# hammershock/3dgs-avatar-release

Hardware: AMD Instinct MI355X
Metric: render fps (fwd+bwd) @200k Gaussians 1024x1024 SH3 (higher is better)
Workload: dtype f32; 1 GPU; config3: 200k Gaussians, 1024x1024, SH deg 3, forward+backward; shs+scales+rotations inputs, L1 loss (L1 fused into the rasterizer: l1_target); tile_rect=1, l1=fused, long_lists=0, gaussians=200000, width=1024, height=1024, sh_degree=3, frames_per_rank=1857, total_frames=1857, ranks=1, backend=none, parallelism=frames sharded x1

## Files before the change

### 3dgs-avatar-release_amd/csrc/binning.hip

```cpp
#include "common.h"

__global__ __launch_bounds__(256) void first_pair_kernel(const uint32_t* __restrict__ tiles,
                                                         const uint32_t* __restrict__ wave_tiles, float* __restrict__ rec,
                                                         int P, unsigned long long* __restrict__ count,
                                                         unsigned long long* host_count) {
    __shared__ unsigned long long wb[4];
    const int tid = threadIdx.x, lane = tid & 63, wid = tid >> 6;
    const int w0 = 4 * (int)blockIdx.x;
    unsigned long long before = 0;
    for (int w = tid; w < w0; w += 256) before += wave_tiles[w];
#pragma unroll
    for (int d = 32; d >= 1; d >>= 1) before += __shfl_xor(before, d, 64);
    if (lane == 0) wb[wid] = before;
    const int i = blockIdx.x * 256 + tid;
    const uint32_t v = i < P ? tiles[i] : 0u;
    uint32_t x = v;
#pragma unroll
    for (int d = 1; d < 64; d <<= 1) {
        const uint32_t y = __shfl_up(x, d, 64);
        if (lane >= d) x += y;
    }
    __syncthreads();
    const unsigned long long block_base = (wb[0] + wb[1]) + (wb[2] + wb[3]);
    uint32_t woff = 0;
// ... 257 lines not shown
        }
#pragma unroll
        for (int i = 0; i < PER; i++) {
            if (i * 1024 >= ntiles) break;
            mx = max(mx, held[i]);
        }
    } else {
        for (int t = tid; t < ntiles; t += 1024) mx = max(mx, tile_work(ranges, keys, mode, t));
    }
    mx = wave_max(mx);
    if (lane == 0) wmax[wid] = mx;
    __syncthreads();
    mx = 0;
    for (int w = 0; w < 16; w++) mx = max(mx, wmax[w]);
    const float scale = mx ? 1023.0f / (float)mx : 0.f;
    auto bin_of = [&](uint32_t w) { return 1023u - min(1023u, (uint32_t)((float)w * scale)); };
    if (HELD) {
#pragma unroll
        for (int i = 0; i < PER; i++) {
            if (i * 1024 >= ntiles) break;
            if (i * 1024 + tid < ntiles) atomicAdd(&hist[bin_of(held[i])], 1u);
        }
    } else {
        for (int t = tid; t < ntiles; t += 1024) atomicAdd(&hist[bin_of(tile_work(ranges, keys, mode, t))], 1u);
    }
    __syncthreads();
    const uint32_t v = hist[tid];
    const uint32_t x = wave_scan_incl(v);
    if (lane == 63) wsum[wid] = x;
    __syncthreads();
    uint32_t woff = 0;
    for (int w = 0; w < wid; w++) woff += wsum[w];
    hist[tid] = woff + x - v;
    __syncthreads();
    uint32_t wide_from = 0xFFFFFFFFu;
    uint32_t ch = 0;
    uint32_t xmask = 0;
    if (mode == 2) {
        const unsigned long long D = *pc.dev;
        wide_from = max(FWD4_MIN_LIST, (uint32_t)min(D / (unsigned long long)ll.total_div, 0x7FFFFFFFull));
        if (ll.mark == 2 && D <= FWDC_SPARSE_PAIRS) wide_from = min(FWD4_MIN_LIST, ll.ch_min);
        if (ll.stats || ll.mark == 2) {
            uint32_t nlong = 0;
            if (HELD) {
#pragma unroll
                for (int i = 0; i < PER; i++) {
                    if (i * 1024 >= ntiles) break;
                    nlong += (i * 1024 + tid < ntiles && held[i] > wide_from) ? 1u : 0u;
                }
            } else {
                for (int t = tid; t < ntiles; t += 1024) nlong += tile_work(ranges, keys, mode, t) > wide_from ? 1u : 0u;
            }
            nlong = wave_sum(nlong);
            __syncthreads();
            if (lane == 0) wsum[wid] = nlong;
            __syncthreads();
            uint32_t tot = 0;
            for (int w = 0; w < 16; w++) tot += wsum[w];
            if (tid == 0 && ll.stats) {
                __hip_atomic_store(&ll.stats[0], (long long)tot, __ATOMIC_RELAXED, __HIP_MEMORY_SCOPE_SYSTEM);
                __hip_atomic_store(&ll.stats[1], (long long)mx, __ATOMIC_RELAXED, __HIP_MEMORY_SCOPE_SYSTEM);
            }
            xmask = (ll.mark == 2 && ll.xcc_mask) ? (*ll.xcc_mask & 0xFFu) : 0u;
            if (xmask && tot > 0 && tot <= FWDC_MAX_UNITS / 2 && D <= (unsigned long long)pc.cap) {
                ch = ll.ch_min;
                while (D / ch + tot > (unsigned long long)FWDC_MAX_UNITS && ch < 0x40000000u) ch <<= 1;
            }
            __syncthreads();
            if (tid == 0) wmax[0] = 0u;
            if (tid < 16) wsum[tid] = 0u;
            __syncthreads();
        }
        if (!ll.mark) wide_from = 0xFFFFFFFFu;
        if (ll.mark == 2 && ch == 0) wide_from = 0xFFFFFFFFu;
    }
    auto place = [&](const int t, const uint32_t wk) {
        const bool marked = wk > wide_from && (ch == 0u || wk > ch);
        order[atomicAdd(&hist[bin_of(wk)], 1u)] = (uint32_t)t | (marked ? 0x80000000u : 0u);
    };
    if (HELD) {
#pragma unroll
        for (int i = 0; i < PER; i++) {
            if (i * 1024 >= ntiles) break;
            const int t = i * 1024 + tid;
            if (t < ntiles) place(t, held[i]);
        }
    } else {
        for (int t = tid; t < ntiles; t += 1024) place(t, tile_work(ranges, keys, mode, t));
    }
    if (ch) {
        __syncthreads();
        uint32_t* __restrict__ stash = hist;
        uint32_t* __restrict__ nstash = &wmax[1];
        if (tid == 0) *nstash = 0u;
        __syncthreads();
        const uint32_t nx = (uint32_t)__popc(xmask);
        for (int pos = tid; pos < ntiles; pos += 1024) {
            const uint32_t ov = order[pos];
            if (!(ov >> 31)) continue;
            const int t = (int)(ov & 0x7FFFFFFFu);
            const uint32_t nch = (tile_work(ranges, keys, mode, t) + ch - 1u) / ch;
            const uint32_t u0 = atomicAdd(&wmax[0], nch);
            const uint32_t ph = (uint32_t)pos % (2u * nx);
            uint32_t pick = ph < nx ? ph : 2u * nx - 1u - ph, best = 0;
            for (uint32_t x = 0; x < 8; x++) {
                if ((xmask >> x) & 1u) {
                    if (pick == 0u) { best = x; break; }
                    pick--;
                }
            }
            const uint32_t i0 = atomicAdd(&wsum[8 + best], 4u * nch);
            const uint32_t k = atomicAdd(nstash, 1u);
            stash[4 * k] = (uint32_t)t;
            stash[4 * k + 1] = u0;
            stash[4 * k + 2] = i0 | (best << 28);
            stash[4 * k + 3] = nch;
        }
        __syncthreads();
        const uint32_t nk = *nstash;
        for (uint32_t k = (uint32_t)wid; k < nk; k += 16) {
            const uint32_t t = stash[4 * k], u0 = stash[4 * k + 1], ib = stash[4 * k + 2], nch = stash[4 * k + 3];
            uint32_t* __restrict__ items = ll.cw_items + (size_t)(ib >> 28) * (FWDC_MAX_UNITS * 4) + (ib & 0x0FFFFFFFu);
            for (uint32_t c = (uint32_t)lane; c < nch; c += 64) ll.cw_units[u0 + c] = make_uint2(t, c | (nch << 16));
            for (uint32_t i = (uint32_t)lane; i < 4u * nch; i += 64) items[i] = (u0 + (i >> 2)) * 4u + (i & 3u);
        }
    }
    if (ll.cw_hdr) {
        __syncthreads();
        if (tid == 0) {
            ll.cw_hdr[0] = (mode == 2 && ch) ? wmax[0] : 0u;
            ll.cw_hdr[1] = ch;
        }
        if (tid < 8) ll.cw_hdr[4 + tid] = (mode == 2 && ch) ? wsum[8 + tid] : 0u;
    }
}

template <bool HELD>
__global__ __launch_bounds__(1024) void tile_order_kernel(const uint2* __restrict__ ranges,
                                                          const uint32_t* __restrict__ keys, int mode, int ntiles,
                                                          uint32_t* __restrict__ order, const PairCount pc,
                                                          const FillJob fill, const LongLists ll) {
    if (blockIdx.x > 0) {
        if (fill.clean && *fill.clean == MARKS_CLEAN) return;
        const uint4 ones = make_uint4(0xFFFFFFFFu, 0xFFFFFFFFu, 0xFFFFFFFFu, 0xFFFFFFFFu);
        for (size_t k = (size_t)(blockIdx.x - 1) * 1024 + threadIdx.x; k < fill.quads; k += (size_t)(gridDim.x - 1) * 1024)
            if (fill.stream) store_stream(&fill.ptr[k], ones); else fill.ptr[k] = ones;
        return;
    }
    __shared__ uint32_t hist[1024];
    __shared__ uint32_t wmax[16];
    __shared__ uint32_t wsum[16];
    if (mode < 0) return;
    tile_order_body<HELD>(ranges, keys, mode, ntiles, order, pc, ll, hist, wmax, wsum);
}

#define BM_LD 33
#ifndef TW_STOP_AFTER
#define TW_STOP_AFTER 99
#endif
template <bool CW>
__global__ __launch_bounds__(TBK_THREADS) void tile_write_kernel(const uint4* __restrict__ ranklist,
                                                                 const uint32_t* __restrict__ seg_start, int P, int gx,
                                                                 int gy, int nbx, int nblocks, int nseg, int ntiles,
                                                                 const uint32_t* __restrict__ seg_cnt,
                                                                 const uint32_t* __restrict__ tile_tot,
                                                                 uint2* __restrict__ ranges, uint32_t* __restrict__ order,
                                                                 uint32_t* __restrict__ point_list, const PairCount pc,
                                                                 const LongLists ll) {
    __shared__ uint32_t m_id[TBK_BUF];
    __shared__ unsigned short m_rc[TBK_BUF];
    __shared__ uint32_t bitmap[TB_TILES * BM_LD];
    __shared__ uint32_t dst[TB_TILES];
    __shared__ uint32_t wcnt[TBK_WAVES];
    __shared__ unsigned long long sb_scratch[20];
    static_assert(TBK_THREADS == 1024 && TBK_WAVES == 16 && TB_H <= 4 && TB_TILES * BM_LD >= 1024 && TB_TILES >= 32, "the ordering job borrows bitmap / dst");
    if (blockIdx.x == 0) {
        if (CW) {
            if (ntiles <= 32 * 1024) tile_order_body<true>(nullptr, tile_tot, 2, ntiles, order, pc, ll, bitmap, dst, dst + 16);
            else tile_order_body<false>(nullptr, tile_tot, 2, ntiles, order, pc, ll, bitmap, dst, dst + 16);
        } else if (ntiles <= 32 * 1024) {
            tile_order_plain<true>(nullptr, tile_tot, 2, ntiles, order, pc, ll, bitmap, dst, dst + 16);
        } else {
            tile_order_plain<false>(nullptr, tile_tot, 2, ntiles, order, pc, ll, bitmap, dst, dst + 16);
        }
        return;
    }
    const int tid = threadIdx.x, lane = tid & 63, wid = tid >> 6;
    const int b = ((int)blockIdx.x - 1) % nblocks, sg = ((int)blockIdx.x - 1) / nblocks;
    const int r0 = min(P, (int)seg_start[sg] * 256), r1 = min(P, (int)seg_start[sg + 1] * 256);
    const int bx0 = (b % nbx) * TB_W, by0 = (b / nbx) * TB_H;
    const int bx1 = min(gx, bx0 + TB_W), by1 = min(gy, by0 + TB_H);
    const unsigned long long frame_pairs = *pc.dev;
    const bool fits = frame_pairs <= (unsigned long long)pc.cap;
    uint32_t my_dst = 0;
    {
        const int t_blk0 = by0 * gx + bx0;
        uint32_t part = 0;
        for (int t0 = 0; t0 < t_blk0; t0 += 4 * TBK_THREADS) {
            uint32_t v[4];
#pragma unroll
            for (int k = 0; k < 4; k++) v[k] = t0 + k * TBK_THREADS + tid < t_blk0 ? tile_tot[t0 + k * TBK_THREADS + tid] : 0u;
            part += (v[0] + v[1]) + (v[2] + v[3]);
        }
        const int ty = by0 + wid, tx = bx0 + lane;
        const bool row_ok = tid < TB_TILES && ty < by1;
        const int t_row0 = ty * gx + bx0, t = t_row0 + lane;
        const bool tile_ok = row_ok && tx < bx1;
        uint32_t tot = 0, pre = 0, rowsum = 0;
        if (row_ok) {
            for (int k = lane; k < gx; k += 64) rowsum += t_row0 + k < ntiles ? tile_tot[t_row0 + k] : 0u;
            if (tile_ok) {
                tot = tile_tot[t];
                for (int s0 = 0; s0 < sg; s0 += 8) {
                    uint32_t v[8];
#pragma unroll
                    for (int k = 0; k < 8; k++) v[k] = (s0 + k < sg) ? seg_cnt[(size_t)(s0 + k) * ntiles + t] : 0u;
#pragma unroll
                    for (int k = 0; k < 8; k++) pre += v[k];
                }
            }
        }
        part = wave_sum(part);
        rowsum = wave_sum(rowsum);
        uint32_t* s_part = reinterpret_cast<uint32_t*>(sb_scratch);
        if (lane == 0) {
            s_part[wid] = part;
            if (wid < TB_H) s_part[16 + wid] = rowsum;
        }
        __syncthreads();
        if (row_ok) {
            uint32_t before = 0;
            for (int w = 0; w < TBK_WAVES; w++) before += s_part[w];
            for (int r = 0; r < wid; r++) before += s_part[16 + r];
            const uint32_t x = wave_scan_incl(tot);
            const uint32_t first = before + x - tot;
            if (sg == 0 && tile_ok) ranges[t] = fits ? make_uint2(first, first + tot) : make_uint2(0u, 0u);
            my_dst = first + pre;
        }
        __syncthreads();
    }
    if (TW_STOP_AFTER <= 1) return;
    if (!fits || !point_list) return;
    for (int k = tid; k < TB_TILES * BM_LD; k += TBK_THREADS) bitmap[k] = 0u;
    uint4 e[TBK_LPL];
    auto load_trip = [&](const int rb) {
#pragma unroll
        for (int k = 0; k < TBK_LPL; k++) {
            const int r = rb + wid * (64 * TBK_LPL) + k * 64 + lane;
            e[k] = r < r1 ? ranklist[r] : make_uint4(0, 0, 0, 0);
        }
    };
    if (TW_STOP_AFTER <= 2) return;
    load_trip(r0);
    if (tid < TB_TILES) dst[tid] = my_dst;
    const unsigned long long lt_mask = (lane == 0) ? 0ull : (~0ull >> (64 - lane));
    int count = 0;
    const int grp = lane >> 4, gl = lane & 15;

    auto process_batch = [&](const int n) {
        const int nw = (n + 31) >> 5;
        for (int m0 = wid * 4; m0 < n; m0 += TBK_WAVES * 4) {
            const int m = m0 + grp;
            if (m < n) {
                const uint32_t rc = m_rc[m];
                const uint32_t lw = ((rc >> 8) & 63u) + 1u, lh = ((rc >> 14) & 3u) + 1u;
                const uint32_t area = lw * lh, lx = rc & 63u, ly = (rc >> 6) & 3u;
                for (uint32_t j = (uint32_t)gl; j < area; j += 16u) {
                    const uint32_t dy = (j >= lw ? 1u : 0u) + (j >= 2u * lw ? 1u : 0u) + (j >= 3u * lw ? 1u : 0u);
                    const uint32_t lt = (ly + dy) * TB_W + lx + (j - dy * lw);
                    atomicOr(&bitmap[lt * BM_LD + (m >> 5)], 1u << (m & 31));
                }
            }
        }
        __syncthreads();
        for (int lt0 = wid * 4; lt0 < TB_TILES; lt0 += TBK_WAVES * 4) {
            const int lt = lt0 + grp;
            uint32_t bits0 = 0, bits1 = 0;
            if (gl < nw) { bits0 = bitmap[lt * BM_LD + gl]; bitmap[lt * BM_LD + gl] = 0u; }
            if (gl + 16 < nw) { bits1 = bitmap[lt * BM_LD + gl + 16]; bitmap[lt * BM_LD + gl + 16] = 0u; }
            const uint32_t c0 = (uint32_t)__popc(bits0), c1 = (uint32_t)__popc(bits1);
            const uint32_t xs = row_scan_incl(c0 | (c1 << 16));
            const uint32_t x0 = xs & 0xFFFFu, x1 = xs >> 16;
            const uint32_t e0 = (uint32_t)__builtin_amdgcn_readlane((int)xs, 15), e1 = (uint32_t)__builtin_amdgcn_readlane((int)xs, 31);
            const uint32_t e2 = (uint32_t)__builtin_amdgcn_readlane((int)xs, 47), e3 = (uint32_t)__builtin_amdgcn_readlane((int)xs, 63);
            const uint32_t ends = grp == 0 ? e0 : (grp == 1 ? e1 : (grp == 2 ? e2 : e3));
            const uint32_t tot0 = ends & 0xFFFFu, tot1 = ends >> 16;
            const uint32_t d0 = dst[lt];
            uint32_t pos = d0 + x0 - c0;
            while (bits0) {
                const int bp = __ffs((int)bits0) - 1;
                bits0 &= bits0 - 1u;
                point_list[pos++] = m_id[(gl << 5) + bp];
            }
            pos = d0 + tot0 + x1 - c1;
            while (bits1) {
                const int bp = __ffs((int)bits1) - 1;
                bits1 &= bits1 - 1u;
                point_list[pos++] = m_id[((gl + 16) << 5) + bp];
            }
            if (gl == 0) dst[lt] = d0 + tot0 + tot1;
        }
        __syncthreads();
    };

    __syncthreads();
    for (int rb = r0; rb < r1 || count > 0;) {
        if (rb < r1) {
            uint32_t rc[TBK_LPL], id[TBK_LPL];
            unsigned long long bal[TBK_LPL];
            int c[TBK_LPL], csum = 0;
#pragma unroll
            for (int k = 0; k < TBK_LPL; k++) {
                const bool h = block_hit(e[k], bx0, by0, bx1, by1, &rc[k]);
                id[k] = e[k].x;
                bal[k] = __ballot(h);
                c[k] = __popcll(bal[k]);
                csum += c[k];
            }
            if (lane == 0) wcnt[wid] = (uint32_t)csum;
            if (rb + TBK_CHUNK < r1) load_trip(rb + TBK_CHUNK);
            __syncthreads();
            uint32_t woff = 0, tot = 0;
            for (int w = 0; w < TBK_WAVES; w++) {
                const uint32_t cw = wcnt[w];
                woff += w < wid ? cw : 0u;
                tot += cw;
            }
            int slot0 = count + (int)woff;
#pragma unroll
            for (int k = 0; k < TBK_LPL; k++) {
                if ((bal[k] >> lane) & 1ull) {
                    const int slot = slot0 + __popcll(bal[k] & lt_mask);
                    m_id[slot] = id[k];
                    m_rc[slot] = (unsigned short)rc[k];
                }
                slot0 += c[k];
            }
            count += (int)tot;
            rb += TBK_CHUNK;
            __syncthreads();
        }
        const bool last = rb >= r1;
        while (count >= TBK_BATCH || (last && count > 0)) {
            const int n = min(count, TBK_BATCH);
            if (TW_STOP_AFTER > 3) process_batch(n);
            const int rem = count - n;
            uint32_t cid[TBK_LPL];
            unsigned short crc[TBK_LPL];
#pragma unroll
            for (int k = 0; k < TBK_LPL; k++) {
                const int i = tid + k * TBK_THREADS;
                cid[k] = i < rem ? m_id[n + i] : 0u;
                crc[k] = i < rem ? m_rc[n + i] : (unsigned short)0;
            }
            __syncthreads();
#pragma unroll
            for (int k = 0; k < TBK_LPL; k++) {
                const int i = tid + k * TBK_THREADS;
                if (i < rem) { m_id[i] = cid[k]; m_rc[i] = crc[k]; }
            }
            count = rem;
            __syncthreads();
        }
    }
}

int launch_tile_order(const uint32_t* ranges, const uint32_t* keys, int mode, int ntiles, uint32_t* order, PairCount pc,
                      FillJob fill, LongLists ll, int debug, hipStream_t s) {
    const size_t pieces = (fill.quads + 1023) / 1024;
    const int side = fill.ptr ? (int)(pieces < 255 ? pieces : 255) : 0;
    if (ntiles <= 32 * 1024)
        hipLaunchKernelGGL(tile_order_kernel<true>, dim3(1 + side), dim3(1024), 0, s, reinterpret_cast<const uint2*>(ranges),
                           keys, mode, ntiles, order, pc, fill, ll);
    else
        hipLaunchKernelGGL(tile_order_kernel<false>, dim3(1 + side), dim3(1024), 0, s, reinterpret_cast<const uint2*>(ranges),
                           keys, mode, ntiles, order, pc, fill, ll);
    GS_LAUNCH_CHECK("tile_order", debug, s);
    return GS_OK;
}

int launch_tile_lists(const uint4* ranklist, const uint32_t* chunk_pairs, uint32_t* seg_start, int P, int gx, int gy, TileCounts tc, uint32_t* ranges,
                      uint32_t* order, uint32_t* point_list, PairCount pc, LongLists ll, bool totals_zeroed, int debug,
                      hipStream_t s) {
    uint32_t* seg_cnt = tc.seg_cnt;
    const BinGrid G = bin_grid(gx, gy);
    const int nseg = bin_segments(G, P);
    const int ntiles = gx * gy;
    if (!totals_zeroed) {
        const int zrc = gs_zero_async(tc.tile_tot, tc.zero_bytes, "tile_totals.zero", s);
        if (zrc != GS_OK) return zrc;
    }
    {
        int band_rows = TC_CELLS / (gx + 1) - 1;
        if (band_rows < 1) return GS_E_TOO_LARGE;
        if (band_rows > gy) band_rows = gy;
        const int nbands = (gy + band_rows - 1) / band_rows;
        StageScope sc_("tile_count", s);
        hipLaunchKernelGGL(tile_count_kernel, dim3((unsigned)(nbands * nseg)), dim3(TC_THREADS), 0, s, ranklist, chunk_pairs, seg_start, P,
                           gx, gy, band_rows, nbands, nseg, ntiles, seg_cnt, tc.tile_tot, tc.xcc_mask);
        GS_LAUNCH_CHECK("tile_count", debug, s);
    }
    {
        StageScope sc_("tile_write", s);
        if (ll.mark == 2)
            hipLaunchKernelGGL(tile_write_kernel<true>, dim3((unsigned)(1 + G.nblocks * nseg)), dim3(TBK_THREADS), 0, s, ranklist,
                               seg_start, P, gx, gy, G.nbx, G.nblocks, nseg, ntiles, seg_cnt, tc.tile_tot,
                               reinterpret_cast<uint2*>(ranges), order, pc.cap > 0 ? point_list : nullptr, pc, ll);
        else
            hipLaunchKernelGGL(tile_write_kernel<false>, dim3((unsigned)(1 + G.nblocks * nseg)), dim3(TBK_THREADS), 0, s, ranklist,
                               seg_start, P, gx, gy, G.nbx, G.nblocks, nseg, ntiles, seg_cnt, tc.tile_tot,
                               reinterpret_cast<uint2*>(ranges), order, pc.cap > 0 ? point_list : nullptr, pc, ll);
        GS_LAUNCH_CHECK("tile_write", debug, s);
    }
    return GS_OK;
}
```

### 3dgs-avatar-release_amd/csrc/capi.hip

```cpp
#include "common.h"
#include <string.h>
#include <stdlib.h>
#include <atomic>
#include <chrono>
#include <mutex>
#include <vector>

static thread_local int g_last_hip = 0;
static thread_local const char* g_last_stage = "";
void gs_set_error(int hip_err, const char* stage) {
    g_last_hip = hip_err;
    g_last_stage = stage;
}

struct TuneSwitch {
    const char* name;
    int key, def;
    const char* env;
    bool (*ok)(int);
};
static const TuneSwitch k_tune[GS_TUNE_COUNT] = {
    {"xcd_map", GS_TUNE_XCD_MAP, 1, nullptr, nullptr},
    {"depth_sort", GS_TUNE_DEPTH_SORT, 1, nullptr, nullptr},
    {"nt_stores", GS_TUNE_NT_STORES, 1, nullptr, nullptr},
    {"bwd_chunks", GS_TUNE_BWD_CHUNKS, 1, nullptr, nullptr},
    {"fwd4", GS_TUNE_FWD4, 1, "GSPLAT_FWD4", nullptr},
    {"small_tiles", GS_TUNE_SMALL_TILES, BWD_CHUNK_MAX_TILES, nullptr, nullptr},
    {"shared_qlist", GS_TUNE_SHARED_QLIST, 1, nullptr, nullptr},
    {"ones_fast", GS_TUNE_ONES_FAST, 1, nullptr, nullptr},
    {"bwd_order", GS_TUNE_BWD_ORDER, 1, nullptr, nullptr},
    {"fwd_marks", GS_TUNE_FWD_MARKS, 1, nullptr, nullptr},
    {"fwdc_ch", GS_TUNE_FWDC_CH, (int)FWDC_CH_MIN, "GSPLAT_FWDC_CH", [](int v) { return v >= 64 && (v & (v - 1)) == 0; }},
    {"fwdc_div", GS_TUNE_FWDC_DIV, (int)FWD4_TOTAL_DIV, "GSPLAT_FWDC_DIV", [](int v) { return v >= 1; }},
};
struct TuneState {
    std::atomic<int> v[GS_TUNE_COUNT];
    TuneState() {
        for (const TuneSwitch& t : k_tune) {
            int value = t.def;
            if (const char* e = t.env ? getenv(t.env) : nullptr) {
                const int x = atoi(e);
                if (!t.ok || t.ok(x)) value = x;
            }
            v[t.key].store(value);
        }
    }
};
static TuneState& tune_state() {
    static TuneState st;
    return st;
}
int gs_tune_get(int key) {
    return (key >= 0 && key < GS_TUNE_COUNT) ? tune_state().v[key].load(std::memory_order_relaxed) : 0;
}

struct ProfRec { const char* name; hipEvent_t a, b; };
struct ProfState {
    bool on = false;
    bool armed = false;
    int nested = 0;
    char filter[32] = {0};
    std::vector<ProfRec> recs;
    std::vector<hipEvent_t> pool;
    hipEvent_t get() {
        if (!pool.empty()) { hipEvent_t e = pool.back(); pool.pop_back(); return e; }
        hipEvent_t e = nullptr;
        (void)hipEventCreate(&e);
        return e;
    }
};
static ProfState g_prof;
static std::mutex g_prof_mu;
static bool profiling_on() { return g_prof.on; }
void gs_prof_begin(const char* stage, hipStream_t s) {
    if (!g_prof.on) return;
    std::lock_guard<std::mutex> lk(g_prof_mu);
    if (g_prof.armed) { g_prof.nested++; return; }
    g_prof.armed = g_prof.on && (g_prof.filter[0] == 0 || strcmp(g_prof.filter, stage) == 0);
    if (!g_prof.armed) return;
    ProfRec r{stage, g_prof.get(), g_prof.get()};
    (void)hipEventRecord(r.a, s);
    g_prof.recs.push_back(r);
}
void gs_prof_end(hipStream_t s) {
    if (!g_prof.on) return;
    std::lock_guard<std::mutex> lk(g_prof_mu);
    if (!g_prof.armed || g_prof.recs.empty()) return;
    if (g_prof.nested > 0) { g_prof.nested--; return; }
    (void)hipEventRecord(g_prof.recs.back().b, s);
    g_prof.armed = false;
}

static int validate(const GsFwdArgs* a) {
    if (!a) return GS_E_BAD_ARG;
    if (a->P < 0 || a->W <= 0 || a->H <= 0) return GS_E_BAD_ARG;
    if (!a->bg || !a->viewmatrix || !a->projmatrix || !a->campos) return GS_E_BAD_ARG;
    if (a->P > 0 && (!a->means3D || !a->opacities)) return GS_E_BAD_ARG;
    if ((a->shs != nullptr) == (a->colors_precomp != nullptr)) return GS_E_EXCLUSIVE;
    const bool sr = a->scales != nullptr && a->rotations != nullptr;
    if ((a->scales != nullptr) != (a->rotations != nullptr)) return GS_E_EXCLUSIVE;
    if (sr == (a->cov3D_precomp != nullptr)) return GS_E_EXCLUSIVE;
    if (a->shs) {
        if (a->sh_degree < 0 || a->sh_degree > 3) return GS_E_BAD_ARG;
        if (a->M < (a->sh_degree + 1) * (a->sh_degree + 1)) return GS_E_BAD_ARG;
        if (a->M > 16) return GS_E_BAD_ARG;
    }
    if (a->rotations && ((uintptr_t)a->rotations & 15u)) return GS_E_BAD_ARG;
    if ((a->W + TILE - 1) / TILE > 0xFFFF || (a->H + TILE - 1) / TILE > 0xFFFF) return GS_E_TOO_LARGE;
    return GS_OK;
}

static bool stream_is_capturing(void* stream) {
    hipStreamCaptureStatus st = hipStreamCaptureStatusNone;
    const hipError_t e = hipStreamIsCapturing((hipStream_t)stream, &st);
    if (e != hipSuccess) {
        (void)hipGetLastError();
        return e == hipErrorStreamCaptureImplicit || e == hipErrorStreamCaptureUnsupported || e == hipErrorStreamCaptureInvalidated;
    }
    return st != hipStreamCaptureStatusNone;
}
#define GS_CAPTURE_OK_IF(stream, cond)                                           \
    do {                                                                         \
        if (stream_is_capturing(stream) && (!(cond) || profiling_on())) return GS_E_CAPTURE; \
    } while (0)
#define GS_NO_CAPTURE(stream) GS_CAPTURE_OK_IF(stream, false)

__global__ void zero_words_kernel(uint32_t* __restrict__ p, size_t words) {
    for (size_t k = (size_t)blockIdx.x * blockDim.x + threadIdx.x; k < words; k += (size_t)gridDim.x * blockDim.x) p[k] = 0u;
}
int gs_zero_async(void* ptr, size_t bytes, const char* stage, hipStream_t s) {
    const size_t words = bytes / 4;
    if (words == 0) return GS_OK;
    const size_t blocks = (words + 255) / 256;
    hipLaunchKernelGGL(zero_words_kernel, dim3((unsigned)(blocks < 1024 ? blocks : 1024)), dim3(256), 0, s, (uint32_t*)ptr, words);
    const hipError_t e = hipGetLastError();
    if (e != hipSuccess) { gs_set_error((int)e, stage); return GS_E_HIP; }
    return GS_OK;
}

__global__ __launch_bounds__(256) void clock_probe_kernel(unsigned long long* __restrict__ out, int iters, float seed, float* __restrict__ sink) {
    const unsigned long long t0 = __builtin_readcyclecounter(), r0 = __builtin_amdgcn_s_memrealtime();
    float a[8];
#pragma unroll
    for (int i = 0; i < 8; i++) a[i] = seed + (float)i + (float)threadIdx.x * 1e-3f;
    for (int it = 0; it < iters; it++) {
#pragma unroll
        for (int u = 0; u < 4; u++)
#pragma unroll
            for (int i = 0; i < 8; i++) a[i] = __builtin_fmaf(a[i], 1.0001f, 0.5f);
    }
    float sum = 0.f;
#pragma unroll
    for (int i = 0; i < 8; i++) sum += a[i];
    if (sum == 12345.678f) sink[0] = sum;
    if (threadIdx.x == 0) {
        const unsigned long long t1 = __builtin_readcyclecounter(), r1 = __builtin_amdgcn_s_memrealtime();
        atomicAdd(&out[0], t1 - t0);
        atomicAdd(&out[1], r1 - r0);
    }
}

__global__ __launch_bounds__(64) void xcc_probe_kernel(uint32_t* __restrict__ out) {
    if (threadIdx.x == 0) out[blockIdx.x] = xcc_id();
}

template <class Void, class VoidBin, class G, class B, class I, class Own>
static int frame_states(const GsFwdArgs* a, Void* geom, size_t geom_bytes, VoidBin* binning, size_t binning_bytes, Void* img,
                        size_t img_bytes, int64_t D, G* g, B* b, I* im, Own own) {
    int rc = validate(a);
    if (rc != GS_OK) return rc;
    if (!geom || !img || D < 0 || (D > 0 && !binning)) return GS_E_BAD_ARG;
    if ((rc = own()) != GS_OK) return rc;
    *g = geom_state(geom, a->P);
    *im = img_state(img, a->W, a->H, a->long_lists);
    *b = bin_state(D > 0 ? binning : nullptr, D);
    if (geom_bytes < g->total || img_bytes < im->total || (D > 0 && binning_bytes < b->total)) return GS_E_WORKSPACE;
    return GS_OK;
}

template <class T> static T* writable(T* p) { return p; }
template <class T> static T* writable(const T* p) { return const_cast<T*>(p); }
template <bool RO>
static QuadLists quad_lists(const ImgViewT<RO>& im, const BinView& b, int long_lists) {
    QuadLists ql;
    ql.qlist = b.qlist;
    ql.ncon_c = writable(im.ncon_c);
    ql.qcount = writable(im.qcount);
    ql.chunks = gs_tune_get(GS_TUNE_BWD_CHUNKS) ? im.bwd_chunks : 1;
    ql.four_waves = forward_small_image(im.ntiles, long_lists) ? 1 : 0;
    ql.ckpt = ql.chunks > 1 ? writable(im.ckpt) : nullptr;
    ql.ck_start = ql.chunks > 1 ? writable(im.ck_start) : nullptr;
    return ql;
}
template <bool RO>
static void quad_lists_chunked(QuadLists& ql, const ImgView& own, const ImgViewT<RO>& list) {
    ql.chunked = 1;
    ql.cw_hdr = list.cw_hdr;
    ql.cw_units = list.cw_units;
    ql.cw_items = list.cw_items;
    ql.cw_q = own.cw_q;
    ql.cw_flag = own.cw_flag;
    ql.cw_done = own.cw_done;
    ql.cw_rec = own.cw_rec;
}
static int sync_if_debug(const GsFwdArgs* a, const char* stage, hipStream_t s) {
    if (!a->debug) return GS_OK;
    const hipError_t e = hipStreamSynchronize(s);
    if (e != hipSuccess) { gs_set_error((int)e, stage); return GS_E_HIP; }
    return GS_OK;
}

extern "C" {

int gs_xcc_probe(uint32_t* xcc, int32_t n_blocks, void* stream) {
    if (!xcc || n_blocks <= 0) return GS_E_BAD_ARG;
    hipStream_t s = (hipStream_t)stream;
    hipLaunchKernelGGL(xcc_probe_kernel, dim3((unsigned)n_blocks), dim3(64), 0, s, xcc);
    GS_LAUNCH_CHECK("xcc_probe", 0, s);
    return GS_OK;
}

int gs_clock_probe(uint64_t* ticks, int32_t iters, void* stream) {
    if (!ticks || iters <= 0) return GS_E_BAD_ARG;
    GS_NO_CAPTURE(stream);
    hipStream_t s = (hipStream_t)stream;
    int rc = gs_zero_async(ticks, 32, "clock_probe.zero", s);
    if (rc != GS_OK) return rc;
    hipLaunchKernelGGL(clock_probe_kernel, dim3(2048), dim3(256), 0, s, (unsigned long long*)ticks, iters, 1.0f, (float*)(ticks + 2));
    GS_LAUNCH_CHECK("clock_probe", 0, s);
    return GS_OK;
}

int gs_geom_bytes(int32_t P, size_t* out) {
    if (!out || P < 0) return GS_E_BAD_ARG;
    *out = geom_layout(P).total;
    return GS_OK;
}
int gs_image_bytes(int32_t W, int32_t H, size_t* out) {
    if (!out || W <= 0 || H <= 0) return GS_E_BAD_ARG;
    *out = img_layout(W, H).total;
    return GS_OK;
}
int gs_image_bytes_for(const GsFwdArgs* a, size_t* out) {
    if (!a || !out || a->W <= 0 || a->H <= 0) return GS_E_BAD_ARG;
    *out = img_layout(a->W, a->H, a->long_lists).total;
    return GS_OK;
}
int gs_binning_bytes(int64_t D, int32_t W, int32_t H, size_t* out) {
    if (!out || D < 0 || W <= 0 || H <= 0) return GS_E_BAD_ARG;
    if (D > GS_MAX_PAIRS) return GS_E_TOO_LARGE;
    *out = bin_layout(D).total;
    return GS_OK;
}
int gs_backward_scratch_bytes(int64_t D, int32_t P, int32_t W, int32_t H, size_t* out) {
    if (!out || D < 0 || P < 0 || W <= 0 || H <= 0) return GS_E_BAD_ARG;
    const ImgLayout I = img_layout(W, H);
    *out = scratch_total_bytes(D, P, I.gx * I.gy);
    return GS_OK;
}

static int forward_phase1(const GsFwdArgs* a, void* geom, size_t geom_bytes, void* img, size_t img_bytes, int32_t* radii,
                          int64_t* count_host_pinned, unsigned long long* poll, void* stream) {
    GeomView g;
    BinView none;
    ImgView im;
    int rc = frame_states(a, geom, geom_bytes, (void*)nullptr, 0, img, img_bytes, 0, &g, &none, &im,
                          [&]() -> int { return (a->P > 0 && !radii) ? GS_E_BAD_ARG : GS_OK; });
    if (rc != GS_OK) return rc;
    hipStream_t s = (hipStream_t)stream;
    if (a->P == 0) {
        rc = gs_zero_async(g.count, COUNT_ZERO_BYTES, "count.zero", s);
        if (rc != GS_OK) return rc;
    } else {
        ZeroJob zt;
        sort_totals_region(g.hist, a->P, 32, &zt.ptr, &zt.words);
        const ZeroJob zi{im.tile_tot, (int)(im.tile_zero_bytes / 4)};
        { StageScope sc_("preprocess", s);
        rc = launch_preprocess(*a, g.rec, g.depths, g.tiles, g.clamped, g.key0, g.val0, radii, g.wsum, g.wkmin, g.wkmax, zt, zi, s); }
        if (rc != GS_OK) return rc;
        if (gs_tune_get(GS_TUNE_DEPTH_SORT)) {
            StageScope sc_("depth_sort", s);
            const DepthSortState ds{g.ds_tmp, g.ds_tmp2, g.ds_cnt, g.ds_pre, g.ds_tot, g.ds_loc, g.ds_grp, g.ds_range, g.ds_nb, g.ds_blocks};
            const PairNumbering pn{g.tiles, g.wsum, g.rec, g.count, poll, g.chunk_pairs, (a->P + 255) / 256};
            const RankOut ro{g.rec, g.tiles, g.val0, g.ranklist, g.chunk_pairs};
            rc = launch_depth_sort(g.key0, g.wkmin, g.wkmax, g.nwaves, a->P, ds, pn, ro, a->debug, s);
            if (rc != GS_OK) return rc;
        } else {
            { StageScope sc_("pair_scan", s);
            rc = launch_first_pair(g.tiles, g.wsum, g.rec, g.count, poll, a->P, a->debug, s); }
            if (rc != GS_OK) return rc;
            { StageScope sc_("depth_sort", s);
            rc = launch_sort_pairs(g.key0, g.val0, g.key1, g.val1, g.hist, a->P, 32, true, a->debug, s); }
            if (rc != GS_OK) return rc;
            { StageScope sc_("rank_list", s);
            rc = launch_rank_list(g.val0, g.rec, g.tiles, g.ranklist, g.chunk_pairs, a->P, a->debug, s); }
            if (rc != GS_OK) return rc;
        }
    }
    if (count_host_pinned && (!poll || a->P == 0)) {
        hipError_t e = hipMemcpyAsync(count_host_pinned, g.count, 8, hipMemcpyDeviceToHost, s);
        if (e != hipSuccess) { gs_set_error((int)e, "count.copy"); return GS_E_HIP; }
    }
    return GS_OK;
}

int gs_forward_preprocess(const GsFwdArgs* a, void* geom, size_t geom_bytes, void* img, size_t img_bytes,
                          int32_t* radii, int64_t* count_host_pinned, void* stream) {
    GS_CAPTURE_OK_IF(stream, a && !a->debug && count_host_pinned == nullptr);
    return forward_phase1(a, geom, geom_bytes, img, img_bytes, radii, count_host_pinned, nullptr, stream);
}

static int forward_phase2(const GsFwdArgs* a, void* geom, size_t geom_bytes, void* binning, size_t binning_bytes, void* img,
                          size_t img_bytes, int64_t cap, float* out_color, void* stream, bool totals_zeroed) {
    GeomView g;
    BinView b;
    ImgView im;
    int rc = frame_states(a, geom, geom_bytes, binning, binning_bytes, img, img_bytes, cap, &g, &b, &im, [&]() -> int {
        if (!out_color) return GS_E_BAD_ARG;
        if (a->l1_target && !a->l1_loss) return GS_E_BAD_ARG;
        return cap > GS_MAX_PAIRS ? GS_E_TOO_LARGE : GS_OK;
    });
    if (rc != GS_OK) return rc;
    hipStream_t s = (hipStream_t)stream;
    const PairCount pc{g.count + COUNT_PAIRS, (uint32_t)cap};
    const bool chunked = forward_chunked(im.ntiles, a->long_lists);
    if (a->P > 0) {
        rc = launch_tile_lists(g.ranklist, g.chunk_pairs, g.seg_start, a->P, im.gx, im.gy,
                               TileCounts{im.seg_cnt, im.tile_tot, im.tile_zero_bytes, im.cw_xcc_mask}, im.ranges, im.order,
                               b.point_list, pc,
                               LongLists{chunked ? 2 : (forward_small_image(im.ntiles, a->long_lists) ? 1 : 0), (long long*)a->frame_stats,
                                         im.cw_hdr, im.cw_units, (uint32_t)gs_tune_get(GS_TUNE_FWDC_CH), im.cw_items, im.cw_xcc_mask,
                                         chunked ? (uint32_t)gs_tune_get(GS_TUNE_FWDC_DIV) : (uint32_t)FWD4_TOTAL_DIV},
                               totals_zeroed, a->debug, s);
        if (rc != GS_OK) return rc;
    } else {
        rc = gs_zero_async(im.ranges, (size_t)im.ntiles * 8, "ranges.zero", s);
        if (rc != GS_OK) return rc;
        StageScope sc_("ranges_order", s);
        rc = launch_tile_order(im.ranges, nullptr, 0, im.ntiles, im.order, pc, FillJob{nullptr, 0},
                               LongLists{0, nullptr, im.cw_hdr, nullptr}, a->debug, s);
        if (rc != GS_OK) return rc;
    }
    QuadLists ql = quad_lists(im, b, a->long_lists);
    if (chunked) quad_lists_chunked(ql, im, im);
    if (cap > 0) {
        ql.marks = (gs_tune_get(GS_TUNE_FWD_MARKS) && !a->forward_only) ? b.marks : nullptr;
        ql.mark_quads = (size_t)cap;
        ql.marks_flag = b.marks_flag;
    }
    ql.l1_target = a->l1_target;
    ql.l1_part = im.l1_part;
    ql.l1_loss = a->l1_loss;
    { StageScope sc_("render_fwd", s);
    rc = launch_render_forward(g.rec, a->P > 0 ? b.point_list : nullptr, im.ranges, im.order, a->bg, a->W, a->H, out_color,
                               im.final_T, im.n_contrib, ql, s); }
    if (rc != GS_OK) return rc;
    return sync_if_debug(a, "render_forward", s);
}

int gs_forward_render(const GsFwdArgs* a, void* geom, size_t geom_bytes, void* binning, size_t binning_bytes,
                      void* img, size_t img_bytes, int64_t D, float* out_color, void* stream) {
    GS_CAPTURE_OK_IF(stream, a && !a->debug && a->frame_stats == nullptr);
    return forward_phase2(a, geom, geom_bytes, binning, binning_bytes, img, img_bytes, D, out_color, stream, false);
}

int gs_forward(const GsFwdArgs* a, void* geom, size_t geom_bytes, void* binning, size_t binning_bytes, int64_t capacity,
               void* img, size_t img_bytes, int32_t* radii, int64_t* count_host_pinned, float* out_color,
               int64_t* num_rendered, void* stream) {
    if (!count_host_pinned || !num_rendered || capacity < 0) return GS_E_BAD_ARG;
    GS_NO_CAPTURE(stream);
    volatile int64_t* word = count_host_pinned;
    const int64_t pending = -1;
    static std::atomic<bool> poll_works{true};
    const bool poll = a && a->P > 0 && poll_works.load(std::memory_order_relaxed);
    if (poll) *word = pending;
    int rc = forward_phase1(a, geom, geom_bytes, img, img_bytes, radii, count_host_pinned,
                            poll ? (unsigned long long*)count_host_pinned : nullptr, stream);
    if (rc != GS_OK) return rc;
    const bool speculate = capacity > 0 && binning && binning_bytes >= bin_layout(capacity).total && capacity <= GS_MAX_PAIRS;
    if (speculate) {
        rc = forward_phase2(a, geom, geom_bytes, binning, binning_bytes, img, img_bytes, capacity, out_color, stream, true);
        if (rc != GS_OK) return rc;
    }
    bool have = false;
    if (poll) {
        const auto t0 = std::chrono::steady_clock::now();
        for (long spin = 0;; spin++) {
            if (*word != pending) { have = true; break; }
            if ((spin & 1023) == 1023 && std::chrono::steady_clock::now() - t0 > std::chrono::milliseconds(200)) break;
        }
    }
    if (!have) {
        hipError_t e = hipStreamSynchronize((hipStream_t)stream);
        if (e != hipSuccess) { gs_set_error((int)e, "count.sync"); return GS_E_HIP; }
        if (poll && *word == pending) {
            poll_works.store(false, std::memory_order_relaxed);
            int64_t c = 0;
            e = hipMemcpy(&c, geom_state(geom, a->P).count + COUNT_PAIRS, 8, hipMemcpyDeviceToHost);
            if (e != hipSuccess) { gs_set_error((int)e, "count.copy"); return GS_E_HIP; }
            *word = c;
        }
    }
    const int64_t D = *word;
    *num_rendered = D;
    if (D > (int64_t)GS_MAX_PAIRS) return GS_E_TOO_LARGE;
    if (!speculate || D > capacity) return GS_E_WORKSPACE;
    return GS_OK;
}

int gs_forward_shared(const GsFwdArgs* a, const void* geom_src, const void* img_src, void* geom, size_t geom_bytes,
                      void* binning, size_t binning_bytes, void* img, size_t img_bytes, int64_t D, float* out_color,
                      void* stream) {
    GS_CAPTURE_OK_IF(stream, a && !a->debug && a->P > 0);
    GeomView g;
    BinView b;
    ImgView im;
    int rc = frame_states(a, geom, geom_bytes, binning, binning_bytes, img, img_bytes, D, &g, &b, &im,
                          [&]() -> int { return (!geom_src || !img_src || !out_color) ? GS_E_BAD_ARG : GS_OK; });
    if (rc != GS_OK) return rc;
    const GeomViewRO first_g = geom_state(geom_src, a->P);
    const ImgViewRO first_im = img_state(img_src, a->W, a->H, a->long_lists);
    hipStream_t s = (hipStream_t)stream;
    const bool chunked = forward_chunked(im.ntiles, a->long_lists);
    QuadLists ql = quad_lists(im, b, a->long_lists);
    unsigned long long* not_ones = nullptr;
    if (a->P > 0) {
        StageScope sc_("recolor", s);
        if (gs_tune_get(GS_TUNE_ONES_FAST) && gs_tune_get(GS_TUNE_SHARED_QLIST) && a->colors_precomp && D > 0)
            not_ones = not_ones_word(first_g);
        const SecondOnes so{first_im.final_T, first_im.n_contrib, first_im.ncon_c, first_im.qcount, first_im.ckpt, first_im.ck_start,
                            out_color, im.final_T, im.n_contrib, im.ncon_c, im.qcount, ql.ckpt, ql.ck_start, a->bg, a->W, a->H,
                            im.gx, im.ntiles, ql.chunks};
        rc = launch_recolor(*a, first_g.rec, first_g.tiles, g.rec, g.tiles, g.clamped, not_ones,
                            CopyJob{first_im.ranges, im.ranges, im.ntiles * 2}, CopyJob{first_im.order, im.order, im.ntiles},
                            ZeroJob{im.cw_flag, im.cw_clear_words}, not_ones ? &so : nullptr, s);
        if (rc != GS_OK) return rc;
    } else {
        hipError_t e = hipMemcpyAsync(im.ranges, first_im.ranges, (size_t)im.ntiles * 8, hipMemcpyDeviceToDevice, s);
        if (e == hipSuccess) e = hipMemcpyAsync(im.order, first_im.order, (size_t)im.ntiles * 4, hipMemcpyDeviceToDevice, s);
        if (e != hipSuccess) { gs_set_error((int)e, "shared.copy"); return GS_E_HIP; }
    }
    if (gs_tune_get(GS_TUNE_SHARED_QLIST)) {
        ql.src_qcount = first_im.qcount;
        ql.src_n_contrib = first_im.n_contrib;
        ql.not_ones = not_ones;
    }
    if (chunked && a->P > 0) {
        quad_lists_chunked(ql, im, first_im);
        if (ql.src_qcount) {
            ql.src_cw_flag = first_im.cw_flag;
            ql.src_cw_rec = first_im.cw_rec;
            ql.src_final_T = first_im.final_T;
        }
    }
    ql.all_ones = im.all_ones;
    { StageScope sc_("render_fwd", s);
    rc = launch_render_forward(g.rec, b.point_list, im.ranges, im.order, a->bg, a->W, a->H, out_color, im.final_T, im.n_contrib, ql, s); }
    if (rc != GS_OK) return rc;
    return sync_if_debug(a, "render_forward", s);
}

int gs_opacity_image(const GsFwdArgs* a, const void* img, size_t img_bytes, float* opacity, void* stream) {
    GS_CAPTURE_OK_IF(stream, true);
    int rc = validate(a);
    if (rc != GS_OK) return rc;
    if (!img || !opacity) return GS_E_BAD_ARG;
    const ImgViewRO im = img_state(img, a->W, a->H, a->long_lists);
    if (img_bytes < im.total) return GS_E_WORKSPACE;
    return launch_opacity_image(im.final_T, a->bg, a->W, a->H, opacity, (hipStream_t)stream);
}

static int backward_impl(const GsFwdArgs* a, const int32_t* radii, const void* geom, size_t geom_bytes, void* binning,
                         size_t binning_bytes, const void* img, size_t img_bytes, int64_t D, const float* out_color,
                         const float* dL_dpix, const float* dL_dopacity_img, void* scratch, size_t scratch_bytes,
                         const GsGrads* gr, void* stream, const GsSecondImage* second = nullptr) {
    GS_CAPTURE_OK_IF(stream, a && !a->debug);
    GeomViewRO g;
    BinView b;
    ImgViewRO im;
    int rc = frame_states(a, geom, geom_bytes, binning, binning_bytes, img, img_bytes, D, &g, &b, &im, [&]() -> int {
        if (!out_color || (!dL_dpix && !a->l1_target) || !gr || (a->P > 0 && !scratch)) return GS_E_BAD_ARG;
        if (a->P > 0 && (!radii || !gr->dL_dmeans3D || !gr->dL_dmeans2D || !gr->dL_dcolors || !gr->dL_dopacity || !gr->dL_dcov3D))
            return GS_E_BAD_ARG;
        if (a->P > 0 && a->shs && !gr->dL_dsh) return GS_E_BAD_ARG;
        if (a->P > 0 && a->scales && (!gr->dL_dscales || !gr->dL_drotations)) return GS_E_BAD_ARG;
        if (gr->dL_drotations && ((uintptr_t)gr->dL_drotations & 15u)) return GS_E_BAD_ARG;
        return GS_OK;
    });
    if (rc != GS_OK) return rc;
    if (a->P > 0 && scratch_bytes < scratch_total_bytes(D, a->P, im.ntiles)) return GS_E_WORKSPACE;
    if (a->P == 0) return GS_OK;
    hipStream_t s = (hipStream_t)stream;
    float* const sums = (float*)((char*)scratch + scratch_rows_bytes(D));
    if (D > 0) {
        const QuadLists ql = quad_lists(im, b, a->long_lists);
        SecondImage si{nullptr, nullptr, nullptr, nullptr, nullptr};
        if (second) {
            const ImgViewRO im2 = img_state(second->img, a->W, a->H, second->long_lists);
            if (second->img_bytes < im2.total || im2.bwd_chunks != im.bwd_chunks) return GS_E_BAD_ARG;
            si = SecondImage{second->colors, second->out_color, second->dL_dpix, ql.chunks > 1 ? im2.ckpt : nullptr, im2.all_ones};
        }
        uint32_t* const q8 = reinterpret_cast<uint32_t*>(b.marks);
        uint32_t* const own_order = (uint32_t*)((char*)sums + scratch_sums_bytes(a->P));
        const bool order_here = gs_tune_get(GS_TUNE_BWD_ORDER) != 0;
        { StageScope sc_("tile_order", s);
        rc = launch_tile_order(im.ranges, ql.qcount, order_here ? 1 : -1, im.ntiles, own_order, PairCount{nullptr, 0},
                               FillJob{b.marks, (size_t)D, gs_tune_get(GS_TUNE_NT_STORES) & 1, b.marks_flag},
                               LongLists{0, nullptr}, a->debug, s); }
        if (rc != GS_OK) return rc;
        { StageScope sc_("render_bwd", s);
        rc = launch_render_backward(g.rec, im.ranges, order_here ? own_order : im.order, a->W, a->H, ql, out_color, dL_dpix,
                                    dL_dopacity_img, im.final_T, a->bg, (float*)scratch, q8, second ? &si : nullptr,
                                    L1Grad{a->l1_target, a->l1_grad}, s); }
        if (rc != GS_OK) return rc;
        rc = sync_if_debug(a, "render_backward", s);
        if (rc != GS_OK) return rc;
    }
    StageScope sc_("gaussian_bwd", s);
    return launch_gaussian_backward(*a, radii, g.rec, g.tiles, g.clamped, reinterpret_cast<const uint32_t*>(b.marks),
                                    (const float*)scratch, sums, b.marks_flag, *gr, s);
}

int gs_backward(const GsFwdArgs* a, const int32_t* radii, const void* geom, size_t geom_bytes, void* binning,
                size_t binning_bytes, const void* img, size_t img_bytes, int64_t D, const float* out_color,
                const float* dL_dpix, void* scratch, size_t scratch_bytes, const GsGrads* gr, void* stream) {
    return backward_impl(a, radii, geom, geom_bytes, binning, binning_bytes, img, img_bytes, D, out_color, dL_dpix, nullptr,
                         scratch, scratch_bytes, gr, stream);
}

int gs_backward_with_opacity(const GsFwdArgs* a, const int32_t* radii, const void* geom, size_t geom_bytes,
                             void* binning, size_t binning_bytes, const void* img, size_t img_bytes, int64_t D,
                             const float* out_color, const float* dL_dpix, const float* dL_dopacity_img, void* scratch,
                             size_t scratch_bytes, const GsGrads* gr, void* stream) {
    if (!dL_dopacity_img) return GS_E_BAD_ARG;
    return backward_impl(a, radii, geom, geom_bytes, binning, binning_bytes, img, img_bytes, D, out_color, dL_dpix,
                         dL_dopacity_img, scratch, scratch_bytes, gr, stream);
}

int gs_backward_with_second(const GsFwdArgs* a, const int32_t* radii, const void* geom, size_t geom_bytes,
                            void* binning, size_t binning_bytes, const void* img, size_t img_bytes, int64_t D,
                            const float* out_color, const float* dL_dpix, const GsSecondImage* second, void* scratch,
                            size_t scratch_bytes, const GsGrads* grads, void* stream) {
    if (!second || !second->colors || !second->out_color || !second->dL_dpix || !second->img) return GS_E_BAD_ARG;
    return backward_impl(a, radii, geom, geom_bytes, binning, binning_bytes, img, img_bytes, D, out_color, dL_dpix, nullptr,
                         scratch, scratch_bytes, grads, stream, second);
}

int gs_mark_visible(int32_t P, const float* means3D, const float* viewmatrix, const float* projmatrix,
                    uint8_t* present, void* stream) {
    GS_CAPTURE_OK_IF(stream, true);
    (void)projmatrix;
    if (P < 0 || !viewmatrix || (P > 0 && (!means3D || !present))) return GS_E_BAD_ARG;
    if (P == 0) return GS_OK;
    return launch_mark_visible(P, means3D, viewmatrix, present, (hipStream_t)stream);
}

int knn_workspace_bytes(int32_t P, size_t* out) {
    if (!out || P < 0) return GS_E_BAD_ARG;
    *out = knn_ws_bytes(P);
    return GS_OK;
}
int knn_dist2(int32_t P, const float* points, float* mean_d2, void* workspace, size_t workspace_bytes, void* stream) {
    GS_NO_CAPTURE(stream);
    if (P < 0 || (P > 0 && (!points || !mean_d2 || !workspace))) return GS_E_BAD_ARG;
    if (P == 0) return GS_OK;
    return launch_knn(P, points, mean_d2, workspace, workspace_bytes, (hipStream_t)stream);
}

int gs_build_covariance(int32_t N, const float* scaling, float scaling_modifier, const float* rotation, int32_t rotation_is_matrix,
                        float* cov6, void* stream) {
    GS_CAPTURE_OK_IF(stream, true);
    if (N < 0 || (N > 0 && (!scaling || !rotation || !cov6))) return GS_E_BAD_ARG;
    if (!rotation_is_matrix && ((uintptr_t)rotation & 15u)) return GS_E_BAD_ARG;
    if (N == 0) return GS_OK;
    return launch_build_cov(N, scaling, scaling_modifier, rotation, rotation_is_matrix ? 1 : 0, cov6, (hipStream_t)stream);
}
int gs_build_covariance_backward(int32_t N, const float* scaling, float scaling_modifier, const float* rotation,
                                 int32_t rotation_is_matrix, const float* dL_dcov6, float* dL_dscaling, float* dL_drotation,
                                 void* stream) {
    GS_CAPTURE_OK_IF(stream, true);
    if (N < 0 || (N > 0 && (!scaling || !rotation || !dL_dcov6 || !dL_dscaling || !dL_drotation))) return GS_E_BAD_ARG;
    if (!rotation_is_matrix && (((uintptr_t)rotation | (uintptr_t)dL_drotation) & 15u)) return GS_E_BAD_ARG;
    if (N == 0) return GS_OK;
    return launch_build_cov_bwd(N, scaling, scaling_modifier, rotation, rotation_is_matrix ? 1 : 0, dL_dcov6, dL_dscaling,
                                dL_drotation, (hipStream_t)stream);
}
int gs_sh2rgb(int32_t N, int32_t sh_degree, int32_t M, const float* shs, const float* xyz, const float* campos,
              const float* fwd_rotation, const float* view_noise_host, float* colors, uint8_t* clamped, void* stream) {
    GS_CAPTURE_OK_IF(stream, view_noise_host == nullptr);
    if (N < 0 || sh_degree < 0 || sh_degree > 3 || M < (sh_degree + 1) * (sh_degree + 1) || M > 16) return GS_E_BAD_ARG;
    if (N > 0 && (!shs || !xyz || !campos || !colors || !clamped)) return GS_E_BAD_ARG;
    if (N == 0) return GS_OK;
    return launch_sh2rgb(N, sh_degree, M, shs, xyz, campos, fwd_rotation, view_noise_host, colors, clamped, (hipStream_t)stream);
}
int gs_sh2rgb_backward(int32_t N, int32_t sh_degree, int32_t M, const float* shs, const float* xyz, const float* campos,
                       const float* fwd_rotation, const float* view_noise_host, const uint8_t* clamped,
                       const float* dL_dcolors, float* dL_dshs, float* dL_dxyz, void* stream) {
    GS_CAPTURE_OK_IF(stream, view_noise_host == nullptr);
    if (N < 0 || sh_degree < 0 || sh_degree > 3 || M < (sh_degree + 1) * (sh_degree + 1) || M > 16) return GS_E_BAD_ARG;
    if (N > 0 && (!shs || !xyz || !campos || !clamped || !dL_dcolors || !dL_dshs || !dL_dxyz)) return GS_E_BAD_ARG;
    if (N == 0) return GS_OK;
    return launch_sh2rgb_bwd(N, sh_degree, M, shs, xyz, campos, fwd_rotation, view_noise_host, clamped, dL_dcolors, dL_dshs,
                             dL_dxyz, (hipStream_t)stream);
}

int gs_l1_loss_workspace_bytes(int64_t n, size_t* out) {
    if (!out || n < 0) return GS_E_BAD_ARG;
    *out = l1_ws_bytes(n);
    return GS_OK;
}
int gs_l1_loss(int64_t n, const float* x, const float* y, float* loss, float* dL_dx, void* workspace, size_t workspace_bytes,
               void* stream) {
    GS_CAPTURE_OK_IF(stream, true);
    if (n <= 0 || !x || !y || !loss || !dL_dx || !workspace) return GS_E_BAD_ARG;
    if (((uintptr_t)x | (uintptr_t)y | (uintptr_t)dL_dx) & 15u) return GS_E_BAD_ARG;
    if (workspace_bytes < l1_ws_bytes(n)) return GS_E_WORKSPACE;
    return launch_l1_loss(x, y, n, loss, dL_dx, (float*)workspace, (hipStream_t)stream);
}

int gs_bce_loss(int64_t n, const float* x, const float* y, float* loss, float* dL_dx, void* workspace, size_t workspace_bytes,
                void* stream) {
    GS_CAPTURE_OK_IF(stream, true);
    if (n <= 0 || !x || !y || !loss || !dL_dx || !workspace) return GS_E_BAD_ARG;
    if (workspace_bytes < l1_ws_bytes(n)) return GS_E_WORKSPACE;
    return launch_bce_loss(x, y, n, loss, dL_dx, (float*)workspace, (hipStream_t)stream);
}

int gs_ssim_workspace_bytes(int32_t C, int32_t H, int32_t W, size_t* out) {
    if (!out || C <= 0 || H <= 0 || W <= 0) return GS_E_BAD_ARG;
    *out = ssim_ws_bytes(C, H, W);
    return GS_OK;
}
int gs_ssim_forward(int32_t C, int32_t H, int32_t W, const float* img1, const float* img2, float* ssim_out, float* dm_dmu1,
                    float* dm_dsigma1_sq, float* dm_dsigma12, void* workspace, size_t workspace_bytes, void* stream) {
    GS_CAPTURE_OK_IF(stream, true);
    if (C <= 0 || H <= 0 || W <= 0 || !img1 || !img2 || !ssim_out || !workspace) return GS_E_BAD_ARG;
    if ((dm_dmu1 != nullptr) != (dm_dsigma1_sq != nullptr) || (dm_dmu1 != nullptr) != (dm_dsigma12 != nullptr)) return GS_E_BAD_ARG;
    if (workspace_bytes < ssim_ws_bytes(C, H, W)) return GS_E_WORKSPACE;
    return launch_ssim_forward(C, H, W, img1, img2, ssim_out, dm_dmu1, dm_dsigma1_sq, dm_dsigma12, (float*)workspace,
                               (hipStream_t)stream);
}
int gs_ssim_backward(int32_t C, int32_t H, int32_t W, const float* img1, const float* img2, const float* dm_dmu1,
                     const float* dm_dsigma1_sq, const float* dm_dsigma12, const float* dL_dssim, float* dL_dimg1,
                     void* stream) {
    GS_CAPTURE_OK_IF(stream, true);
    if (C <= 0 || H <= 0 || W <= 0 || !img1 || !img2 || !dm_dmu1 || !dm_dsigma1_sq || !dm_dsigma12 || !dL_dssim || !dL_dimg1)
        return GS_E_BAD_ARG;
    return launch_ssim_backward(C, H, W, img1, img2, dm_dmu1, dm_dsigma1_sq, dm_dsigma12, dL_dssim, dL_dimg1,
                                (hipStream_t)stream);
}

int gs_densify_stats(int32_t N, const int32_t* radii, const float* viewspace_grad, float* max_radii2D,
                     float* xyz_gradient_accum, float* denom, void* stream) {
    GS_CAPTURE_OK_IF(stream, true);
    if (N < 0 || (N > 0 && (!radii || !viewspace_grad || !max_radii2D || !xyz_gradient_accum || !denom))) return GS_E_BAD_ARG;
    if (N == 0) return GS_OK;
    return launch_densify_stats(N, radii, viewspace_grad, max_radii2D, xyz_gradient_accum, denom, (hipStream_t)stream);
}
int gs_adam_step(int32_t n_tensors, const GsAdamTensor* tensors, double beta1, double beta2, double eps, int64_t step,
                 void* stream) {
    GS_NO_CAPTURE(stream);
    if (n_tensors < 0 || n_tensors > GS_ADAM_MAX_TENSORS || (n_tensors > 0 && !tensors) || step < 1) return GS_E_BAD_ARG;
    for (int k = 0; k < n_tensors; k++) {
        const GsAdamTensor& t = tensors[k];
// ... 658 lines not shown
```

### 3dgs-avatar-release_amd/csrc/common.h

```cpp
#pragma once
#include <hip/hip_runtime.h>
#include <stdint.h>
#include <stddef.h>
#include <type_traits>
#include "../../include/gsplat_mi355.h"

#define TILE 16
#define WAVE 64
#define REC_F 12
#define GS_MAX_PAIRS 0x3FFFFFFFll

static inline size_t align_up(size_t x, size_t a) { return (x + a - 1) / a * a; }

#define SORT_ITEMS 4096
#define SORT_SMALL_N (1 << 20)
#define SORT_TOTALS_REPL 16
static inline size_t sort_table_words(size_t n) {
    const size_t items = n <= (size_t)SORT_SMALL_N ? 1024 : SORT_ITEMS;
    return (size_t)256 * ((n + items - 1) / items + 4 * SORT_TOTALS_REPL);
}
#define SCAN_ITEMS 2048

#ifndef DS_ITEMS
#define DS_ITEMS 2048
#endif
#ifndef DS_PER_BUCKET
#define DS_PER_BUCKET 64
#endif
static inline int ds_buckets(int P) {
    int nb = (P / DS_PER_BUCKET + 63) / 64 * 64;
    return nb < 256 ? 256 : (nb > 4096 ? 4096 : nb);
}

#define TB_MAX_SEG 64
enum { COUNT_PAIRS = 0, COUNT_NOT_ONES = 2, COUNT_ZERO_BYTES = 24 };
struct GeomLayout {
    size_t rec, depths, tiles, clamped, key0, key1, val0, val1, ranklist, chunk_pairs, wsum, wkmin, wkmax, hist, count,
        ds_tmp, ds_tmp2, ds_cnt, ds_pre, ds_tot, ds_loc, ds_grp, ds_range, seg_start, total;
    int nblk_sort, nwaves, ds_nb, ds_blocks;
};
static inline GeomLayout geom_layout(int P) {
    GeomLayout L;
    size_t o = 0;
    size_t n = (size_t)(P > 0 ? P : 1);
    auto take = [&](size_t bytes) { size_t at = o; o = align_up(o + bytes, 256); return at; };
    L.nblk_sort = (int)((n + SORT_ITEMS - 1) / SORT_ITEMS);
    L.nwaves = (int)((n + 255) / 256) * 4;
    L.rec = take(n * REC_F * 4);
    L.depths = take(n * 4);
    L.tiles = take(n * 4);
    L.clamped = take(n * 4);
    L.key0 = take(n * 4);
    L.key1 = take(n * 4);
    L.val0 = take(n * 4);
    L.val1 = take(n * 4);
    L.ranklist = take(n * 16);
    L.chunk_pairs = take(((n + 255) / 256) * 4);
    L.wsum = take((size_t)L.nwaves * 4);
    L.wkmin = take((size_t)L.nwaves * 4);
    L.wkmax = take((size_t)L.nwaves * 4);
    L.hist = take(sort_table_words(n) * 4);
    L.count = take(64);
    L.ds_nb = ds_buckets(P);
    L.ds_blocks = (int)((n + DS_ITEMS - 1) / DS_ITEMS);
    L.ds_tmp = take(n * 8);
    L.ds_tmp2 = take(n * 8);
    L.ds_cnt = take((size_t)L.ds_blocks * (L.ds_nb + 1) * 4);
    L.ds_pre = take((size_t)L.ds_blocks * (L.ds_nb + 1) * 4);
    L.ds_tot = take((size_t)(L.ds_nb + 1) * 4);
    L.ds_loc = take((size_t)(L.ds_nb + 1) * 4);
    L.ds_grp = take((size_t)((L.ds_nb + 1 + 63) / 64) * 4);
    L.ds_range = take(16);
    L.seg_start = take((size_t)(TB_MAX_SEG + 2) * 4);
    L.total = o;
    return L;
}

struct BinLayout {
    size_t point_list, qlist, marks, marks_flag, total;
};
static inline BinLayout bin_layout(int64_t D) {
    BinLayout L;
    size_t o = 0;
    size_t n = (size_t)(D > 0 ? D : 1);
    auto take = [&](size_t bytes) { size_t at = o; o = align_up(o + bytes, 256); return at; };
    L.point_list = take(n * 4);
    L.qlist = take(n * 16);
    L.marks = take(n * 16);
    L.marks_flag = take(4);
    L.total = o;
    return L;
}

#define TB_W 64
#ifndef TB_H
#define TB_H 4
#endif
#define TB_TILES (TB_W * TB_H)
struct BinGrid { int nbx, nby, nblocks, nseg_max; };
static inline BinGrid bin_grid(int gx, int gy) {
    BinGrid G;
    G.nbx = (gx + TB_W - 1) / TB_W;
    G.nby = (gy + TB_H - 1) / TB_H;
    G.nblocks = G.nbx * G.nby;
#ifndef TB_TARGET_WGS
#define TB_TARGET_WGS 512
#endif
    int s = (TB_TARGET_WGS + G.nblocks - 1) / G.nblocks;
    G.nseg_max = s < 1 ? 1 : (s > TB_MAX_SEG ? TB_MAX_SEG : s);
    return G;
}
static inline int bin_segments(const BinGrid& G, int P) {
    int s = (P + 1023) / 1024;
    if (s < 1) s = 1;
    return s < G.nseg_max ? s : G.nseg_max;
}

enum { GS_TUNE_XCD_MAP = 0, GS_TUNE_DEPTH_SORT = 1, GS_TUNE_NT_STORES = 2, GS_TUNE_BWD_CHUNKS = 3, GS_TUNE_FWD4 = 4, GS_TUNE_SMALL_TILES = 5, GS_TUNE_SHARED_QLIST = 6, GS_TUNE_ONES_FAST = 7, GS_TUNE_BWD_ORDER = 8, GS_TUNE_FWD_MARKS = 9, GS_TUNE_FWDC_CH = 10, GS_TUNE_FWDC_DIV = 11, GS_TUNE_COUNT = 12 };
int gs_tune_get(int key);

#define BWD_CH 128
#define BWD_KMAX 16
#define BWD_CHUNK_MAX_TILES 2048
#define FWD4_MAX_TILES 2048
#define FWD4_MIN_LIST 512u
#ifndef FWD4_TOTAL_DIV
#define FWD4_TOTAL_DIV 320ull
#endif

#define FWDC_CH_MIN 256u
#define FWDC_SPARSE_PAIRS 524288ull
#define FWDC_MAX_UNITS 4096
#define FWDC_MAX_TILES (FWDC_MAX_UNITS / 2)
#define FWDC_Q_WORDS (8 * FWDC_MAX_UNITS * 4)
#define FWDC_Q_BYTES ((size_t)FWDC_Q_WORDS * 4 + 64)
#ifdef FWDC_PROF
#define FWDC_SLOTS 9
#else
#define FWDC_SLOTS 8
#endif
#define FWDC_DEAD 0x80000000u
#define FWDC_SPIN_MAX (1 << 16)
struct ImgLayout {
    size_t ranges, n_contrib, final_T, ncon_c, tile_nmax, order, seg_cnt, tile_tot, all_ones, cw_flag, cw_done, cw_q, tile_zero_bytes, l1_part, ckpt, ck_start, cw_hdr, cw_units, cw_items, cw_rec, total;
    int gx, gy, bwd_chunks;
};
static inline bool few_long_lists_mode(int ntiles, int long_lists) {
    return ntiles <= gs_tune_get(GS_TUNE_SMALL_TILES) || long_lists != 0;
}
static inline ImgLayout img_layout(int W, int H, int long_lists = 0) {
    ImgLayout L;
    size_t o = 0;
    auto take = [&](size_t bytes) { size_t at = o; o = align_up(o + bytes, 256); return at; };
    L.gx = (W + TILE - 1) / TILE;
    L.gy = (H + TILE - 1) / TILE;
    const size_t nt = (size_t)L.gx * L.gy;
    L.ranges = take(nt * 8);
    L.n_contrib = take((size_t)W * H * 4);
    L.final_T = take((size_t)W * H * 4);
    L.ncon_c = take((size_t)W * H * 4);
    L.tile_nmax = take(nt * 16);
    L.order = take(nt * 4);
    L.seg_cnt = take(nt * 4 * (size_t)bin_grid(L.gx, L.gy).nseg_max);
    L.tile_tot = take(nt * 4);
    L.all_ones = take(4);
    L.tile_zero_bytes = L.all_ones + 4 - L.tile_tot;
    const bool fl = few_long_lists_mode((int)nt, long_lists);
    const bool cw = fl && gs_tune_get(GS_TUNE_FWD4) == 2;
    L.cw_flag = L.cw_done = L.cw_q = 0;
    if (cw) {
        L.cw_flag = take((size_t)FWDC_MAX_UNITS * 4 * 4);
        L.cw_done = take(nt * 16);
        L.cw_q = take(FWDC_Q_BYTES);
        L.tile_zero_bytes = L.cw_q + FWDC_Q_BYTES - L.tile_tot;
    }
    L.l1_part = take(nt * 16);
    L.bwd_chunks = fl ? BWD_KMAX : 1;
    L.ckpt = take(nt * 4 * (size_t)(L.bwd_chunks - 1) * 64 * 16);
    L.ck_start = take(nt * 4 * (size_t)L.bwd_chunks * 4);
    L.cw_hdr = L.cw_units = L.cw_items = L.cw_rec = 0;
    if (cw) {
        L.cw_hdr = take(64);
        L.cw_units = take((size_t)FWDC_MAX_UNITS * 8);
        L.cw_items = take((size_t)FWDC_Q_WORDS * 4);
        L.cw_rec = take((size_t)FWDC_MAX_UNITS * 4 * FWDC_SLOTS * 64 * 4);
    }
    L.total = o;
    return L;
}

template <bool RO>
struct StateCarve {
    typename std::conditional<RO, const char, char>::type* base;
    StateCarve(typename std::conditional<RO, const void, void>::type* state) : base(static_cast<decltype(base)>(state)) {}
    template <class T>
    void operator()(T*& field, size_t offset, bool present = true) const {
        field = (base && present) ? reinterpret_cast<T*>(base + offset) : nullptr;
    }
};
template <bool RO>
struct GeomViewT {
    template <class T> using ptr = typename std::conditional<RO, const T, T>::type*;
    ptr<float> rec, depths;
    ptr<uint32_t> tiles, clamped, key0, key1, val0, val1;
    ptr<uint4> ranklist;
    ptr<uint32_t> chunk_pairs, wsum, wkmin, wkmax, hist;
    ptr<unsigned long long> count;
    ptr<unsigned long long> ds_tmp, ds_tmp2;
    ptr<uint32_t> ds_cnt, ds_pre, ds_tot, ds_loc, ds_grp, ds_range, seg_start;
    size_t total;
    int nwaves, ds_nb, ds_blocks;
};
template <bool RO>
struct BinViewT {
    template <class T> using ptr = typename std::conditional<RO, const T, T>::type*;
    ptr<uint32_t> point_list, qlist;
    ptr<uint4> marks;
    ptr<uint32_t> marks_flag;
    size_t total;
};
template <bool RO>
struct ImgViewT {
    template <class T> using ptr = typename std::conditional<RO, const T, T>::type*;
    ptr<uint32_t> ranges, n_contrib;
    ptr<float> final_T;
    ptr<uint32_t> ncon_c, qcount , order, seg_cnt, tile_tot, all_ones;
    ptr<uint32_t> cw_flag, cw_done, cw_q, cw_xcc_mask ;
    ptr<float> l1_part;
    ptr<float4> ckpt;
    ptr<uint32_t> ck_start, cw_hdr;
    ptr<uint2> cw_units;
    ptr<uint32_t> cw_items;
    ptr<float> cw_rec;
    size_t tile_zero_bytes;
    int cw_clear_words;
    size_t total;
    int gx, gy, ntiles, bwd_chunks;
};
typedef GeomViewT<false> GeomView;
typedef GeomViewT<true> GeomViewRO;
typedef BinViewT<false> BinView;
typedef BinViewT<true> BinViewRO;
typedef ImgViewT<false> ImgView;
typedef ImgViewT<true> ImgViewRO;

template <class Void >
static inline GeomViewT<std::is_const<Void>::value> geom_state(Void* base, int P) {
    constexpr bool RO = std::is_const<Void>::value;
    const GeomLayout L = geom_layout(P);
    const StateCarve<RO> at{base};
    GeomViewT<RO> v;
    at(v.rec, L.rec); at(v.depths, L.depths); at(v.tiles, L.tiles); at(v.clamped, L.clamped);
    at(v.key0, L.key0); at(v.key1, L.key1); at(v.val0, L.val0); at(v.val1, L.val1);
    at(v.ranklist, L.ranklist); at(v.chunk_pairs, L.chunk_pairs);
    at(v.wsum, L.wsum); at(v.wkmin, L.wkmin); at(v.wkmax, L.wkmax); at(v.hist, L.hist); at(v.count, L.count);
    at(v.ds_tmp, L.ds_tmp); at(v.ds_tmp2, L.ds_tmp2); at(v.ds_cnt, L.ds_cnt); at(v.ds_pre, L.ds_pre);
    at(v.ds_tot, L.ds_tot); at(v.ds_loc, L.ds_loc); at(v.ds_grp, L.ds_grp); at(v.ds_range, L.ds_range);
    at(v.seg_start, L.seg_start);
    v.total = L.total; v.nwaves = L.nwaves; v.ds_nb = L.ds_nb; v.ds_blocks = L.ds_blocks;
    return v;
}
template <class Void >
static inline BinViewT<std::is_const<Void>::value> bin_state(Void* base, int64_t D) {
    constexpr bool RO = std::is_const<Void>::value;
    const BinLayout L = bin_layout(D);
    const StateCarve<RO> at{base};
    BinViewT<RO> v;
    at(v.point_list, L.point_list); at(v.qlist, L.qlist); at(v.marks, L.marks); at(v.marks_flag, L.marks_flag);
    v.total = L.total;
    return v;
}
template <class Void >
static inline ImgViewT<std::is_const<Void>::value> img_state(Void* base, int W, int H, int long_lists) {
    constexpr bool RO = std::is_const<Void>::value;
    const ImgLayout L = img_layout(W, H, long_lists);
    const StateCarve<RO> at{base};
    const bool cw = L.cw_rec != 0;
    ImgViewT<RO> v;
    at(v.ranges, L.ranges); at(v.n_contrib, L.n_contrib); at(v.final_T, L.final_T); at(v.ncon_c, L.ncon_c);
    at(v.qcount, L.tile_nmax); at(v.order, L.order); at(v.seg_cnt, L.seg_cnt); at(v.tile_tot, L.tile_tot);
    at(v.all_ones, L.all_ones);
    at(v.cw_flag, L.cw_flag, cw); at(v.cw_done, L.cw_done, cw); at(v.cw_q, L.cw_q, cw);
    at(v.cw_xcc_mask, L.cw_q + (size_t)FWDC_Q_WORDS * 4, cw);
    at(v.l1_part, L.l1_part); at(v.ckpt, L.ckpt); at(v.ck_start, L.ck_start);
    at(v.cw_hdr, L.cw_hdr, cw); at(v.cw_units, L.cw_units, cw); at(v.cw_items, L.cw_items, cw); at(v.cw_rec, L.cw_rec, cw);
    v.tile_zero_bytes = L.tile_zero_bytes;
    v.cw_clear_words = cw ? (int)((L.cw_q + FWDC_Q_BYTES - L.cw_flag) / 4) : 0;
    v.total = L.total; v.gx = L.gx; v.gy = L.gy; v.ntiles = L.gx * L.gy; v.bwd_chunks = L.bwd_chunks;
    return v;
}
static inline unsigned long long* not_ones_word(const GeomViewRO& first) {
    return const_cast<unsigned long long*>(first.count) + COUNT_NOT_ONES;
}

static inline int radix_passes(int bits) { return (bits + 7) / 8; }

void gs_set_error(int hip_err, const char* stage);
#define GS_LAUNCH_CHECK(stage, dbg, stream)                                            \
    do {                                                                               \
        hipError_t e__ = hipGetLastError();                                            \
        if (e__ == hipSuccess && (dbg)) e__ = hipStreamSynchronize((hipStream_t)(stream)); \
        if (e__ != hipSuccess) { gs_set_error((int)e__, stage); return GS_E_HIP; }     \
    } while (0)

int gs_zero_async(void* ptr, size_t bytes, const char* stage, hipStream_t s);
void gs_prof_begin(const char* stage, hipStream_t s);
void gs_prof_end(hipStream_t s);
struct ZeroJob { uint32_t* ptr; int words; };
template <int CTRL, int ROW_MASK>
__device__ __forceinline__ uint32_t dpp_or_zero(uint32_t v) {
    return (uint32_t)__builtin_amdgcn_update_dpp(0, (int)v, CTRL, ROW_MASK, 0xF, false);
}
__device__ __forceinline__ uint32_t wave_scan_incl(uint32_t x) {
    x += dpp_or_zero<0x111, 0xF>(x);
    x += dpp_or_zero<0x112, 0xF>(x);
    x += dpp_or_zero<0x114, 0xF>(x);
    x += dpp_or_zero<0x118, 0xF>(x);
    x += dpp_or_zero<0x142, 0xA>(x);
    x += dpp_or_zero<0x143, 0xC>(x);
    return x;
}
__device__ __forceinline__ uint32_t row_scan_incl(uint32_t x) {
    x += dpp_or_zero<0x111, 0xF>(x);
    x += dpp_or_zero<0x112, 0xF>(x);
    x += dpp_or_zero<0x114, 0xF>(x);
    x += dpp_or_zero<0x118, 0xF>(x);
    return x;
}
__device__ __forceinline__ unsigned long long wave_scan_incl(unsigned long long x) {
#define GS_SCAN64_STEP(CTRL, MASK)                                                                           \
    x += (unsigned long long)dpp_or_zero<CTRL, MASK>((uint32_t)x) |                                          \
         ((unsigned long long)dpp_or_zero<CTRL, MASK>((uint32_t)(x >> 32)) << 32);
    GS_SCAN64_STEP(0x111, 0xF) GS_SCAN64_STEP(0x112, 0xF) GS_SCAN64_STEP(0x114, 0xF) GS_SCAN64_STEP(0x118, 0xF)
    GS_SCAN64_STEP(0x142, 0xA) GS_SCAN64_STEP(0x143, 0xC)
#undef GS_SCAN64_STEP
    return x;
}

__device__ __forceinline__ uint32_t wave_sum(uint32_t x) { return (uint32_t)__builtin_amdgcn_readlane((int)wave_scan_incl(x), 63); }
__device__ __forceinline__ unsigned long long wave_sum(unsigned long long x) {
    x = wave_scan_incl(x);
    return (unsigned long long)(uint32_t)__builtin_amdgcn_readlane((int)(uint32_t)x, 63) |
           ((unsigned long long)(uint32_t)__builtin_amdgcn_readlane((int)(uint32_t)(x >> 32), 63) << 32);
}
__device__ __forceinline__ uint32_t wave_max(uint32_t x) {
    x = max(x, dpp_or_zero<0x111, 0xF>(x));
    x = max(x, dpp_or_zero<0x112, 0xF>(x));
    x = max(x, dpp_or_zero<0x114, 0xF>(x));
    x = max(x, dpp_or_zero<0x118, 0xF>(x));
    x = max(x, dpp_or_zero<0x142, 0xA>(x));
    x = max(x, dpp_or_zero<0x143, 0xC>(x));
    return (uint32_t)__builtin_amdgcn_readlane((int)x, 63);
}
__device__ __forceinline__ uint32_t wave_min(uint32_t x) { return ~wave_max(~x); }
__device__ __forceinline__ float wave_sum(float x) {
#define GS_FSUM_STEP(CTRL, MASK) x += __builtin_bit_cast(float, __builtin_amdgcn_update_dpp(0, __builtin_bit_cast(int, x), CTRL, MASK, 0xF, false));
    GS_FSUM_STEP(0x111, 0xF) GS_FSUM_STEP(0x112, 0xF) GS_FSUM_STEP(0x114, 0xF) GS_FSUM_STEP(0x118, 0xF)
    GS_FSUM_STEP(0x142, 0xA) GS_FSUM_STEP(0x143, 0xC)
#undef GS_FSUM_STEP
    return __builtin_bit_cast(float, __builtin_amdgcn_readlane(__builtin_bit_cast(int, x), 63));
}

#ifndef SEG_RANK_W
#define SEG_RANK_W 4096u
#endif
__device__ __forceinline__ int segment_of(unsigned long long before, unsigned long long scale, int nseg) {
    const unsigned long long hi = __umul64hi(before, scale), lo = before * scale;
    return (int)min((unsigned long long)(nseg - 1), (hi << 32) | (lo >> 32));
}
__device__ __forceinline__ void segment_starts(const uint32_t* __restrict__ chunk_pairs, int P, int nseg, uint32_t* seg_start ,
                                               unsigned long long* scratch ) {
    const int tid = threadIdx.x, lane = tid & 63, wid = tid >> 6;
    const int nthreads = (int)blockDim.x, nwaves = nthreads >> 6;
    const int nchunks = (P + 255) / 256;
    const int per = (nchunks + nthreads - 1) / nthreads;
    const int c0 = tid * per;
    auto work = [&](int c) { return chunk_pairs[c] + SEG_RANK_W; };
    uint32_t w[4] = {0u, 0u, 0u, 0u};
    const uint32_t w_prev = (c0 > 0 && c0 < nchunks) ? work(c0 - 1) : 0u;
    unsigned long long mine = 0;
    for (int k0 = 0; k0 < per; k0 += 4) {
#pragma unroll
        for (int k = 0; k < 4; k++) w[k] = (k0 + k < per && c0 + k0 + k < nchunks) ? work(c0 + k0 + k) : 0u;
#pragma unroll
        for (int k = 0; k < 4; k++) mine += w[k];
    }
    const unsigned long long x = wave_scan_incl(mine);
    __syncthreads();
    if (lane == 63) scratch[wid] = x;
    __syncthreads();
    unsigned long long woff = 0, total = 0;
    for (int wv = 0; wv < nwaves; wv++) {
        const unsigned long long c = scratch[wv];
        woff += wv < wid ? c : 0ull;
        total += c;
    }
    const unsigned long long scale = (unsigned long long)((double)nseg * 4294967296.0 / (double)total);
    unsigned long long before = woff + x - mine;
    int prev_seg = -1;
    if (c0 > 0 && c0 < nchunks) prev_seg = segment_of(before - w_prev, scale, nseg);
    for (int k0 = 0; k0 < per; k0 += 4) {
        if (per > 4) {
#pragma unroll
            for (int k = 0; k < 4; k++) w[k] = (k0 + k < per && c0 + k0 + k < nchunks) ? work(c0 + k0 + k) : 0u;
        }
#pragma unroll
        for (int k = 0; k < 4; k++) {
            const int c = c0 + k0 + k;
            if (k0 + k < per && c < nchunks) {
                const int sgc = segment_of(before, scale, nseg);
                for (int sg = prev_seg + 1; sg <= sgc; sg++) seg_start[sg] = (uint32_t)c;
                prev_seg = sgc;
                before += w[k];
                if (c == nchunks - 1)
                    for (int sg = prev_seg + 1; sg <= nseg; sg++) seg_start[sg] = (uint32_t)nchunks;
            }
        }
    }
}

__device__ __forceinline__ uint32_t xcc_id() {
    uint32_t v;
    asm volatile("s_getreg_b32 %0, hwreg(HW_REG_XCC_ID, 0, 4)" : "=s"(v));
    return v & 7u;
}
__device__ __forceinline__ void zero_job(const ZeroJob z) {
    for (int k = blockIdx.x * blockDim.x + threadIdx.x; k < z.words; k += gridDim.x * blockDim.x) z.ptr[k] = 0u;
}

struct PairCount { const unsigned long long* dev; uint32_t cap; };
__device__ __forceinline__ uint32_t pair_count(const PairCount pc) {
    const unsigned long long d = *pc.dev;
    return d <= (unsigned long long)pc.cap ? (uint32_t)d : 0u;
}

__device__ __forceinline__ void render_block_map(int b, int xmap, int* slot, int* q) {
    if (xmap) {
        *slot = ((b >> 5) << 3) + (b & 7);
// ... 21 lines not shown
struct RankOut { const float* rec; const uint32_t* tiles; uint32_t* sorted_idx; uint4* ranklist; uint32_t* chunk_pairs; };
int launch_depth_sort(const uint32_t* keys, const uint32_t* wave_kmin, const uint32_t* wave_kmax, int nwaves, int P,
                      DepthSortState st, PairNumbering pn, RankOut ro, int debug, hipStream_t s);
struct CopyJob { const uint32_t* src; uint32_t* dst; int words; };
struct SecondOnes {
    const float* src_final_T; const uint32_t* src_n_contrib; const uint32_t* src_ncon_c; const uint32_t* src_qcount;
    const float4* src_ckpt; const uint32_t* src_ck_start;
    float* out_color; float* final_T; uint32_t* n_contrib; uint32_t* ncon_c; uint32_t* qcount; float4* ckpt; uint32_t* ck_start;
    const float* bg; int W, H, gx, ntiles, chunks;
};
__device__ __forceinline__ void second_ones_body(const SecondOnes& A, const int block, const int pixel_blocks) {
    if (block < pixel_blocks) {
        const size_t HW = (size_t)A.H * A.W, pid = (size_t)block * 256 + threadIdx.x;
        if (pid < HW) {
            const float Tf = A.src_final_T[pid];
            A.final_T[pid] = Tf;
            A.n_contrib[pid] = A.src_n_contrib[pid];
            A.ncon_c[pid] = A.src_ncon_c[pid];
            A.out_color[pid] = (1.0f - Tf) + Tf * A.bg[0];
            A.out_color[HW + pid] = (1.0f - Tf) + Tf * A.bg[1];
            A.out_color[2 * HW + pid] = (1.0f - Tf) + Tf * A.bg[2];
        }
        return;
    }
    const int quad = (block - pixel_blocks) * 4 + ((int)threadIdx.x >> 6), tile = quad >> 2, lane = threadIdx.x & 63;
    if (tile >= A.ntiles) return;
    if (lane == 0) A.qcount[quad] = A.src_qcount[quad];
    if (A.chunks > 1) {
        if (lane < A.chunks) A.ck_start[(size_t)quad * A.chunks + lane] = A.src_ck_start[(size_t)quad * A.chunks + lane];
        for (int c = 1; c < A.chunks; c++) {
            if (A.src_ck_start[(size_t)quad * A.chunks + c] == 0xFFFFFFFFu) break;
            const size_t ci = ((size_t)quad * (size_t)(A.chunks - 1) + (size_t)(c - 1)) * 64 + lane;
            const float Tc = A.src_ckpt[ci].x;
            A.ckpt[ci] = make_float4(Tc, 1.0f - Tc, 1.0f - Tc, 1.0f - Tc);
        }
    }
}
int launch_recolor(const GsFwdArgs& a, const float* rec_src, const uint32_t* tiles_src, float* rec_dst,
                   uint32_t* tiles_dst, uint32_t* clamped_dst, unsigned long long* not_ones, CopyJob c0, CopyJob c1,
                   ZeroJob z0, const SecondOnes* ones, hipStream_t s);
int launch_mark_visible(int P, const float* means3D, const float* view, uint8_t* present, hipStream_t s);

int launch_sort_pairs(uint32_t* k0, uint32_t* v0, uint32_t* k1, uint32_t* v1, uint32_t* hist, int64_t n, int bits,
                      bool totals_zeroed, int debug, hipStream_t s, const unsigned long long* n_dev = nullptr);
static inline void sort_totals_region(uint32_t* hist, int64_t n, int bits, uint32_t** ptr, int* words) {
    const size_t nn = (size_t)(n > 0 ? n : 1);
    const size_t items = nn <= (size_t)SORT_SMALL_N ? 1024 : SORT_ITEMS;
    *ptr = hist + (size_t)256 * ((nn + items - 1) / items);
    *words = ((bits + 7) / 8) * SORT_TOTALS_REPL * 256;
}


int launch_first_pair(const uint32_t* tiles, const uint32_t* wave_tiles, float* rec, unsigned long long* count,
                      unsigned long long* host_count, int P, int debug, hipStream_t s);
int launch_rank_list(const uint32_t* sorted_idx, const float* rec, const uint32_t* tiles, uint4* ranklist,
                     uint32_t* chunk_pairs, int P, int debug, hipStream_t s);
struct TileCounts { uint32_t *seg_cnt, *tile_tot; size_t zero_bytes; uint32_t* xcc_mask = nullptr; };
struct LongLists { int mark; long long* stats; uint32_t* cw_hdr = nullptr; uint2* cw_units = nullptr; uint32_t ch_min = FWDC_CH_MIN;
                   uint32_t* cw_items = nullptr; const uint32_t* xcc_mask = nullptr;
                   uint32_t total_div = (uint32_t)FWD4_TOTAL_DIV; };
int launch_tile_lists(const uint4* ranklist, const uint32_t* chunk_pairs, uint32_t* seg_start, int P, int gx, int gy, TileCounts tc, uint32_t* ranges,
                      uint32_t* order, uint32_t* point_list, PairCount pc, LongLists ll, bool totals_zeroed, int debug,
                      hipStream_t s);

int launch_densify_stats(int N, const int32_t* radii, const float* viewspace_grad, float* max_radii2D,
                         float* xyz_gradient_accum, float* denom, hipStream_t s);
int launch_adam(int n, const GsAdamTensor* tensors, double beta1, double beta2, double eps, int64_t step, hipStream_t s);
size_t grad_norm_workspace_bytes(int n, const GsGradTensor* tensors);
int launch_grad_norm(int n, const GsGradTensor* tensors, float max_norm, float* out, float* workspace, hipStream_t s);
int launch_grad_scale(int n, const GsGradTensor* tensors, const float* clip_coef, hipStream_t s);
int launch_adam_ex(int n, const GsAdamTensorEx* tensors, double beta1, double beta2, double eps, int64_t step,
                   const float* clip_coef, hipStream_t s);
size_t densify_workspace_bytes(int N);
int launch_densify_plan(const GsDensifyPlan& p, void* workspace, int32_t* count_host, hipStream_t s);
int launch_densify_apply(int N, int N_new, const void* workspace, int n, const GsDensifyTensor* tensors,
                         const float* scaling, const float* rotation, const float* noise, hipStream_t s);
int launch_reset_opacity(int N, const float* in, float* out, float* exp_avg, float* exp_avg_sq, hipStream_t s);
size_t aiap_workspace_bytes(int N, int K);
int launch_aiap_forward(int N, int K, const long long* idx, int n_sets, const GsAiapSet* sets, void* workspace, hipStream_t s);
int launch_aiap_backward(int N, int K, const long long* idx, int n_sets, const GsAiapSet* sets, const void* workspace,
                         hipStream_t s);

struct HgTable {
    int L, F;
    float scale[GS_HASHGRID_MAX_LEVELS];
    uint32_t res[GS_HASHGRID_MAX_LEVELS], size[GS_HASHGRID_MAX_LEVELS], off[GS_HASHGRID_MAX_LEVELS + 1];
};
int hashgrid_table(const GsHashGrid* g, HgTable* t);
size_t hashgrid_workspace_bytes(const HgTable& t, int N);
int launch_hashgrid_forward(const HgTable& t, int N, const float* x, const float* params, float* out, hipStream_t s);
int launch_hashgrid_backward(const HgTable& t, int N, const float* x, const float* params, const float* dL_dout,
                             float* dL_dx, float* dL_dparams, void* workspace, hipStream_t s);
size_t skinning_workspace_bytes(int N);
int launch_skin_weights_forward(int N, int kind, const float* logits, float* weights, hipStream_t s);
int launch_skin_weights_backward(int N, int kind, const float* logits, const float* dL_dweights, float* dL_dlogits,
                                 hipStream_t s);
int launch_skinning_forward(int N, int kind, const float* w, const float* tfs, const float* xyz, const float* rot,
                            float* xyz_out, float* rot_out, float* T_fwd, hipStream_t s);
int launch_skinning_backward(int N, int kind, const float* w, const float* tfs, const float* xyz, const float* rot,
                             const float* dxyz_out, const float* drot_out, float* dw, float* dtfs, float* dxyz, float* drot,
                             void* workspace, hipStream_t s);
size_t skin_loss_workspace_bytes(int n);
int launch_mesh_sample(int n, int V, int F, const float* verts, const int* faces, const float* cdf, const float* vweights,
                       const float* aabb_min, const float* aabb_inv_extent, const float* draws, float* p_norm, float* target,
                       int* face, float* bary, float* points, hipStream_t s);
int launch_skin_loss_forward(int n, int kind, const float* logits, const float* target, float* loss, void* workspace,
                             hipStream_t s);
int launch_skin_loss_backward(int n, int kind, const float* logits, const float* target, const float* dL_dloss,
                              float* dL_dlogits, hipStream_t s);
size_t pose_workspace_bytes(int V);
int launch_pose_forward(const GsPoseArgs* a, float* rots, float* Jtrs, float* bone, float* loss, float* state, void* workspace,
                        hipStream_t s);
int launch_pose_backward(const GsPoseArgs* a, const float* state, const float* g_rots, const float* g_Jtrs, const float* g_bone,
                         const float* g_loss, float* dbetas, float* droot, float* dbody, float* dhand, float* dtrans,
                         hipStream_t s);
size_t pose_encoder_grad_floats(int d);
int launch_pose_encoder_forward(const GsPoseEncArgs* a, float* out, float* state, hipStream_t s);
int launch_pose_encoder_backward(const GsPoseEncArgs* a, const float* state, const float* g_out, float* dparams, float* drots,
                                 float* dJtrs, hipStream_t s);
size_t nonrigid_workspace_bytes(int N, int D);
int launch_nonrigid_apply_forward(int N, int D, int smode, int rmode, const float* deltas, const float* xyz, const float* scaling,
                                  const float* rot, float* xyz_o, float* scal_o, float* rot_o, float* feat, float* losses,
                                  void* workspace, hipStream_t s);
int launch_nonrigid_apply_backward(int N, int D, int smode, int rmode, const float* deltas, const float* scaling, const float* rot,
                                   const float* g_xyz, const float* g_scal, const float* g_rot, const float* g_feat,
                                   const float* g_nrx, const float* g_nrs, const float* g_nrr, float* ddeltas, float* dscal,
                                   float* drot, hipStream_t s);
struct TxGrads {
    float* before[GS_TEXTURE_MAX_BEFORE];
    float* after[GS_TEXTURE_MAX_AFTER];
};
size_t texture_workspace_bytes(int N, int D, int latent_dim);
int launch_texture_input_forward(const GsTextureArgs* a, float* inp, hipStream_t s);
int launch_texture_input_backward(const GsTextureArgs* a, const float* g, const TxGrads& grads, float* dxyz, float* dlatent,
                                  void* workspace, hipStream_t s);
size_t mlp_workspace_bytes(const GsMlpArgs* a, int backward);
int launch_mlp_forward(const GsMlpArgs* a, float* y, float* acts, void* workspace, hipStream_t s);
int launch_mlp_backward(const GsMlpArgs* a, const float* acts, const float* g, void* workspace, hipStream_t s);
int launch_knn_points(int Nq, const float* queries, int Nr, const float* ref, int K, float* out_d, long long* out_i,
                      void* ws, size_t ws_bytes, hipStream_t s);

int launch_build_cov(int N, const float* scales, float mod, const float* rot, int is_matrix, float* cov6, hipStream_t s);
int launch_build_cov_bwd(int N, const float* scales, float mod, const float* rot, int is_matrix, const float* dL_dcov6,
                         float* dL_dscales, float* dL_drot, hipStream_t s);
int launch_sh2rgb(int N, int deg, int M, const float* shs, const float* xyz, const float* campos, const float* R_fwd,
                  const float* noise_host, float* colors, uint8_t* clamped, hipStream_t s);
int launch_sh2rgb_bwd(int N, int deg, int M, const float* shs, const float* xyz, const float* campos, const float* R_fwd,
                      const float* noise_host, const uint8_t* clamped, const float* dL_dcolors, float* dL_dshs, float* dL_dxyz,
                      hipStream_t s);

size_t l1_ws_bytes(int64_t n);
int launch_l1_loss(const float* x, const float* y, int64_t n, float* loss, float* grad, float* partial, hipStream_t s);
int launch_loss_final(const float* partial, int nparts, float inv_n, float* loss, hipStream_t s);
int launch_bce_loss(const float* x, const float* y, int64_t n, float* loss, float* grad, float* partial, hipStream_t s);
size_t ssim_ws_bytes(int C, int H, int W);
int launch_ssim_forward(int C, int H, int W, const float* img1, const float* img2, float* ssim_out, float* dm_dmu1,
                        float* dm_ds1, float* dm_ds12, float* partial, hipStream_t s);
int launch_ssim_backward(int C, int H, int W, const float* img1, const float* img2, const float* dm_dmu1,
                         const float* dm_ds1, const float* dm_ds12, const float* dL_dssim, float* dL_dimg1,
                         hipStream_t s);

#define MARKS_CLEAN 0x600DF111u
struct FillJob { uint4* ptr; size_t quads; int stream = 0; const uint32_t* clean = nullptr;  };

typedef uint32_t gs_u32x4 __attribute__((ext_vector_type(4)));
__device__ __forceinline__ void store_stream(uint4* p, uint4 v) {
    gs_u32x4 x = {v.x, v.y, v.z, v.w};
    __builtin_nontemporal_store(x, reinterpret_cast<gs_u32x4*>(p));
}
int launch_tile_order(const uint32_t* ranges, const uint32_t* keys, int mode, int ntiles, uint32_t* order, PairCount pc,
                      FillJob fill, LongLists ll, int debug, hipStream_t s);
struct QuadLists {
    uint32_t* qlist;
    uint32_t* ncon_c;
    uint32_t* qcount;
    int four_waves = 0;
    int chunked = 0;
    const uint32_t* cw_hdr = nullptr;
    const uint2* cw_units = nullptr;
    const uint32_t* cw_items = nullptr;
    uint32_t* cw_q = nullptr;
    uint32_t* cw_flag = nullptr;
    uint32_t* cw_done = nullptr;
    float* cw_rec = nullptr;
    const uint32_t* src_cw_flag = nullptr;
    const float* src_cw_rec = nullptr;
    const float* src_final_T = nullptr;
    const uint32_t* src_qcount = nullptr;
    const uint32_t* src_n_contrib = nullptr;
    const unsigned long long* not_ones = nullptr;
    float4* ckpt = nullptr;
    uint32_t* ck_start = nullptr;
    int chunks = 1;
    uint4* marks = nullptr;
    size_t mark_quads = 0;
    uint32_t* marks_flag = nullptr;
    uint32_t* all_ones = nullptr;
    const float* l1_target = nullptr;
    float* l1_part = nullptr;
    float* l1_loss = nullptr;
};
int launch_render_forward(const float* rec, const uint32_t* point_list, const uint32_t* ranges, const uint32_t* order,
                          const float* bg, int W, int H, float* out_color, float* final_T, uint32_t* n_contrib,
                          const QuadLists& ql, hipStream_t s);
struct SecondImage {
    const float* colors;
    const float* out_color;
    const float* dL_dpix;
    const float4* ckpt;
    const uint32_t* all_ones;
};
struct L1Grad { const float* target; const float* grad; };
int launch_render_backward(const float* rec, const uint32_t* ranges, const uint32_t* order, int W, int H,
                           const QuadLists& ql, const float* out_color, const float* dL_dpix, const float* dL_dopa,
                           const float* final_T, const float* bg, float* qrows, uint32_t* q8, const SecondImage* second,
                           L1Grad l1, hipStream_t s);
int launch_opacity_image(const float* final_T, const float* bg, int W, int H, float* out, hipStream_t s);
int launch_gaussian_backward(const GsFwdArgs& a, const int32_t* radii, const float* rec, const uint32_t* tiles,
                             const uint32_t* clamped, const uint32_t* q8, const float* qrows, float* sums,
                             uint32_t* marks_flag, const GsGrads& g, hipStream_t s);
#define ROW_UNWRITTEN 0xFFFFFFFFu
__host__ __device__ __forceinline__ uint32_t gradient_row(uint32_t first_pair, uint32_t w, uint32_t tx, uint32_t ty, uint32_t q) {
    return first_pair * 4u + (2u * ty + (q >> 1)) * (2u * w) + 2u * tx + (q & 1u);
}
static inline size_t scratch_rows_bytes(int64_t D) { return align_up((size_t)(D > 0 ? D : 1) * 4 * 32, 256); }
static inline size_t scratch_sums_bytes(int P) { return align_up((size_t)(P > 0 ? P : 1) * REC_F * 4, 256); }
static inline size_t scratch_total_bytes(int64_t D, int P, int ntiles) {
    return scratch_rows_bytes(D) + scratch_sums_bytes(P) + align_up((size_t)ntiles * 4, 256);
}

int launch_pair_stats(const float* rec, const uint32_t* point_list, const uint32_t* ranges, const uint32_t* n_contrib, int W, int H,
                      unsigned long long* out, hipStream_t s);
int launch_knn(int P, const float* points, float* out, void* ws, size_t ws_bytes, hipStream_t s);
size_t knn_ws_bytes(int P);
```

### 3dgs-avatar-release_amd/csrc/loss.hip

```cpp
#include "common.h"
#include <math.h>

#define L1_THREADS 256
#define L1_MAX_BLOCKS 1024

__device__ __forceinline__ float sgn_over_n(float d, float inv_n) { return d > 0.f ? inv_n : (d < 0.f ? -inv_n : 0.f); }

__global__ __launch_bounds__(L1_THREADS) void l1_partial_kernel(const float* __restrict__ x, const float* __restrict__ y,
                                                                int64_t n, float inv_n, float* __restrict__ grad,
                                                                float* __restrict__ partial) {
    __shared__ float ws[L1_THREADS / 64];
    const int tid = threadIdx.x, lane = tid & 63, wid = tid >> 6;
    float acc = 0.f;
    const int64_t n4 = n >> 2;
    const float4* x4 = reinterpret_cast<const float4*>(x);
    const float4* y4 = reinterpret_cast<const float4*>(y);
    float4* g4 = reinterpret_cast<float4*>(grad);
    const int64_t stride = (int64_t)gridDim.x * L1_THREADS;
    for (int64_t i = (int64_t)blockIdx.x * L1_THREADS + tid; i < n4; i += stride) {
        const float4 a = x4[i], b = y4[i];
        const float d0 = a.x - b.x, d1 = a.y - b.y, d2 = a.z - b.z, d3 = a.w - b.w;
        acc += (fabsf(d0) + fabsf(d1)) + (fabsf(d2) + fabsf(d3));
        g4[i] = make_float4(sgn_over_n(d0, inv_n), sgn_over_n(d1, inv_n), sgn_over_n(d2, inv_n), sgn_over_n(d3, inv_n));
    }
    if (blockIdx.x == 0 && tid < (int)(n & 3)) {
        const int64_t i = (n4 << 2) + tid;
        const float d = x[i] - y[i];
        acc += fabsf(d);
        grad[i] = sgn_over_n(d, inv_n);
    }
    acc = wave_sum(acc);
    if (lane == 0) ws[wid] = acc;
    __syncthreads();
    if (tid == 0) partial[blockIdx.x] = (ws[0] + ws[1]) + (ws[2] + ws[3]);
}

__global__ __launch_bounds__(L1_THREADS) void l1_final_kernel(const float* __restrict__ partial, int nparts, float inv_n,
                                                              float* __restrict__ loss) {
    __shared__ float ws[L1_THREADS / 64];
    const int tid = threadIdx.x, lane = tid & 63, wid = tid >> 6;
    float acc = 0.f;
    for (int i = tid; i < nparts; i += L1_THREADS) acc += partial[i];
    acc = wave_sum(acc);
    if (lane == 0) ws[wid] = acc;
    __syncthreads();
    if (tid == 0) loss[0] = ((ws[0] + ws[1]) + (ws[2] + ws[3])) * inv_n;
}

__global__ __launch_bounds__(L1_THREADS) void bce_partial_kernel(const float* __restrict__ x, const float* __restrict__ y,
                                                                 int64_t n, float inv_n, float* __restrict__ grad,
                                                                 float* __restrict__ partial) {
    __shared__ float ws[L1_THREADS / 64];
    const int tid = threadIdx.x, lane = tid & 63, wid = tid >> 6;
    float acc = 0.f;
    const int64_t stride = (int64_t)gridDim.x * L1_THREADS;
    for (int64_t i = (int64_t)blockIdx.x * L1_THREADS + tid; i < n; i += stride) {
        const float xv = x[i], t = y[i];
        const float p = fminf(fmaxf(xv, 1.0e-3f), 1.0f - 1.0e-3f);
        acc -= t * logf(p) + (1.0f - t) * logf(1.0f - p);
        const bool inside = xv >= 1.0e-3f && xv <= 1.0f - 1.0e-3f;
        grad[i] = inside ? (p - t) / (p * (1.0f - p)) * inv_n : 0.f;
    }
    acc = wave_sum(acc);
    if (lane == 0) ws[wid] = acc;
    __syncthreads();
    if (tid == 0) partial[blockIdx.x] = (ws[0] + ws[1]) + (ws[2] + ws[3]);
}

static int l1_blocks(int64_t n) {
    const int64_t want = ((n >> 2) + L1_THREADS - 1) / L1_THREADS;
    return (int)(want < 1 ? 1 : (want > L1_MAX_BLOCKS ? L1_MAX_BLOCKS : want));
}

size_t l1_ws_bytes(int64_t n) { return (size_t)l1_blocks(n) * sizeof(float); }

int launch_bce_loss(const float* x, const float* y, int64_t n, float* loss, float* grad, float* partial, hipStream_t s) {
    const int blocks = l1_blocks(n);
    const float inv_n = 1.0f / (float)n;
    StageScope st("bce_loss", s);
    hipLaunchKernelGGL(bce_partial_kernel, dim3(blocks), dim3(L1_THREADS), 0, s, x, y, n, inv_n, grad, partial);
    GS_LAUNCH_CHECK("bce_loss.partial", 0, s);
    hipLaunchKernelGGL(l1_final_kernel, dim3(1), dim3(L1_THREADS), 0, s, partial, blocks, inv_n, loss);
    GS_LAUNCH_CHECK("bce_loss.final", 0, s);
    return GS_OK;
}

__global__ __launch_bounds__(1024) void loss_final_wide_kernel(const float* __restrict__ partial, int nparts, float inv_n,
                                                               float* __restrict__ loss) {
    __shared__ float ws[16];
    const int tid = threadIdx.x, lane = tid & 63, wid = tid >> 6;
    float acc = 0.f;
    for (int i0 = tid; i0 < nparts; i0 += 8 * 1024) {
        float v[8];
#pragma unroll
        for (int u = 0; u < 8; u++) v[u] = (i0 + u * 1024 < nparts) ? partial[i0 + u * 1024] : 0.f;
#pragma unroll
        for (int u = 0; u < 8; u++) acc += v[u];
    }
    acc = wave_sum(acc);
    if (lane == 0) ws[wid] = acc;
    __syncthreads();
    if (tid == 0) {
        float t = 0.f;
        for (int w = 0; w < 16; w++) t += ws[w];
        loss[0] = t * inv_n;
    }
}

int launch_loss_final(const float* partial, int nparts, float inv_n, float* loss, hipStream_t s) {
    hipLaunchKernelGGL(loss_final_wide_kernel, dim3(1), dim3(1024), 0, s, partial, nparts, inv_n, loss);
    GS_LAUNCH_CHECK("loss_final", 0, s);
    return GS_OK;
}

int launch_l1_loss(const float* x, const float* y, int64_t n, float* loss, float* grad, float* partial, hipStream_t s) {
    const int blocks = l1_blocks(n);
    const float inv_n = 1.0f / (float)n;
    StageScope st("l1_loss", s);
    hipLaunchKernelGGL(l1_partial_kernel, dim3(blocks), dim3(L1_THREADS), 0, s, x, y, n, inv_n, grad, partial);
    GS_LAUNCH_CHECK("l1_loss.partial", 0, s);
    hipLaunchKernelGGL(l1_final_kernel, dim3(1), dim3(L1_THREADS), 0, s, partial, blocks, inv_n, loss);
    GS_LAUNCH_CHECK("l1_loss.final", 0, s);
    return GS_OK;
}

#define SS_T 32
#define SS_NT 256
#define SS_R 5
#define SS_H (SS_T + 2 * SS_R)
#define SS_C1 0.0001f
#define SS_C2 0.0009f

struct SsimWindow { float w[11]; };

__global__ __launch_bounds__(SS_NT) void ssim_fwd_kernel(int H, int W, const float* __restrict__ img1,
                                                         const float* __restrict__ img2, SsimWindow win,
                                                         float* __restrict__ dm_dmu1, float* __restrict__ dm_ds1,
                                                         float* __restrict__ dm_ds12, float* __restrict__ partial) {
    __shared__ float hx[5][SS_H][SS_T + 1];
    float (*t1)[SS_H + 1] = reinterpret_cast<float (*)[SS_H + 1]>(&hx[0][0][0]);
    float (*t2)[SS_H + 1] = reinterpret_cast<float (*)[SS_H + 1]>(&hx[0][0][0] + SS_H * (SS_H + 1));
    static_assert(2 * SS_H * (SS_H + 1) <= 5 * SS_H * (SS_T + 1), "halo tiles fit in hx");
    __shared__ float ws[SS_NT / 64];
    const int tid = threadIdx.x, tx = tid % SS_T, ty = tid / SS_T;
    const int x0 = blockIdx.x * SS_T, y0 = blockIdx.y * SS_T;
    const size_t plane = (size_t)blockIdx.z * H * W;
    {
        constexpr int TRIPS = (SS_H + SS_NT / 64 - 1) / (SS_NT / 64);
        const int c = tid & 63;
        float v1[TRIPS], v2[TRIPS];
#pragma unroll
        for (int u = 0; u < TRIPS; u++) {
            const int r = (tid >> 6) + u * (SS_NT / 64);
            const int y = y0 + r - SS_R, x = x0 + c - SS_R;
            const bool in = r < SS_H && c < SS_H && y >= 0 && y < H && x >= 0 && x < W;
            v1[u] = in ? img1[plane + (size_t)y * W + x] : 0.f;
            v2[u] = in ? img2[plane + (size_t)y * W + x] : 0.f;
        }
#pragma unroll
        for (int u = 0; u < TRIPS; u++) {
            const int r = (tid >> 6) + u * (SS_NT / 64);
            if (r < SS_H && c < SS_H) { t1[r][c] = v1[u]; t2[r][c] = v2[u]; }
        }
    }
    __syncthreads();
    {
        const int r = tid >> 2, c0 = (tid & 3) * 8;
        float a[18], b[18], aa[18], bb[18], ab[18];
        if (r < SS_H) {
#pragma unroll
            for (int j = 0; j < 18; j++) {
                a[j] = t1[r][c0 + j];
                b[j] = t2[r][c0 + j];
                aa[j] = a[j] * a[j];
                bb[j] = b[j] * b[j];
                ab[j] = a[j] * b[j];
            }
        }
        __syncthreads();
        if (r < SS_H) {
#pragma unroll
            for (int o = 0; o < 8; o++) {
                float m1 = 0.f, m2 = 0.f, e11 = 0.f, e22 = 0.f, e12 = 0.f;
#pragma unroll
                for (int k = 0; k < 11; k++) {
                    const float w = win.w[k];
                    m1 += w * a[o + k];
                    m2 += w * b[o + k];
                    e11 += w * aa[o + k];
                    e22 += w * bb[o + k];
                    e12 += w * ab[o + k];
                }
                hx[0][r][c0 + o] = m1; hx[1][r][c0 + o] = m2; hx[2][r][c0 + o] = e11; hx[3][r][c0 + o] = e22;
                hx[4][r][c0 + o] = e12;
            }
        }
    }
    __syncthreads();
    float val = 0.f;
    {
        const int oy0 = ty * 4;
        float acc[5][4];
#pragma unroll
        for (int m = 0; m < 5; m++) {
            float v[14];
#pragma unroll
            for (int j = 0; j < 14; j++) v[j] = hx[m][oy0 + j][tx];
#pragma unroll
            for (int o = 0; o < 4; o++) {
                float sum = 0.f;
#pragma unroll
                for (int k = 0; k < 11; k++) sum += win.w[k] * v[o + k];
                acc[m][o] = sum;
            }
        }
#pragma unroll
        for (int o = 0; o < 4; o++) {
            const float mu1 = acc[0][o], mu2 = acc[1][o], e11 = acc[2][o], e22 = acc[3][o], e12 = acc[4][o];
            const int x = x0 + tx, y = y0 + oy0 + o;
            if (x < W && y < H) {
                const float mu1_sq = mu1 * mu1, mu2_sq = mu2 * mu2, mu12 = mu1 * mu2;
                const float s1 = e11 - mu1_sq, s2 = e22 - mu2_sq, s12 = e12 - mu12;
                const float A = 2.f * mu12 + SS_C1, B = 2.f * s12 + SS_C2;
                const float C = mu1_sq + mu2_sq + SS_C1, D = s1 + s2 + SS_C2;
                const float inv_cd = 1.0f / (C * D);
                const float v = A * B * inv_cd;
                val += v;
                if (dm_dmu1) {
                    const float d_s1 = -v / D;
                    const float d_s12 = 2.f * A * inv_cd;
                    const float d_mu1 = 2.f * mu2 * B * inv_cd - 2.f * mu1 * v / C - 2.f * mu1 * d_s1 - mu2 * d_s12;
                    const size_t oo = plane + (size_t)y * W + x;
                    dm_dmu1[oo] = d_mu1;
                    dm_ds1[oo] = d_s1;
                    dm_ds12[oo] = d_s12;
                }
            }
        }
    }
    val = wave_sum(val);
    if ((tid & 63) == 0) ws[tid >> 6] = val;
    __syncthreads();
    if (tid == 0) partial[((size_t)blockIdx.z * gridDim.y + blockIdx.y) * gridDim.x + blockIdx.x] = (ws[0] + ws[1]) + (ws[2] + ws[3]);
}

__global__ __launch_bounds__(256) void ssim_final_kernel(const float* __restrict__ partial, int nparts, float inv_n,
                                                         float* __restrict__ out) {
    __shared__ float ws[4];
    const int tid = threadIdx.x, lane = tid & 63, wid = tid >> 6;
    float acc = 0.f;
    for (int i = tid; i < nparts; i += 256) acc += partial[i];
    acc = wave_sum(acc);
    if (lane == 0) ws[wid] = acc;
    __syncthreads();
    if (tid == 0) out[0] = ((ws[0] + ws[1]) + (ws[2] + ws[3])) * inv_n;
}

__global__ __launch_bounds__(SS_NT) void ssim_bwd_kernel(int H, int W, const float* __restrict__ img1,
                                                         const float* __restrict__ img2, SsimWindow win,
// ... 122 lines not shown
```

### 3dgs-avatar-release_amd/csrc/render_fwd.hip

```cpp
#include "common.h"
#include "blend.h"
#include <type_traits>

struct FwdArgs {
    const float4* __restrict__ rec;
    const uint32_t* __restrict__ point_list;
    const uint2* __restrict__ ranges;
    const uint32_t* __restrict__ order;
    const float* __restrict__ bg;
    int W, H, gx, ntiles, xmap;
    float* __restrict__ out_color;
    float* __restrict__ final_T;
    uint32_t* __restrict__ n_contrib;
    uint32_t* __restrict__ qlist;
    uint32_t* __restrict__ ncon_c;
    uint32_t* __restrict__ qcount;
    float4* __restrict__ ckpt;
    uint32_t* __restrict__ ck_start;
    int chunks;
    const uint32_t* __restrict__ src_qcount;
    const uint32_t* __restrict__ src_n_contrib;
    const unsigned long long* __restrict__ not_ones;
    uint4* __restrict__ marks;
    size_t mark_quads;
// ... 737 lines not shown
#ifdef FWD4_PROF
        pf_batches++;
        pf_steps += (lead + (uint32_t)cnt + 3u) / 4u;
#endif
        const char* sp = reinterpret_cast<const char*>(srec) + e * 48;
        const uint32_t kstep0 = kbase - lead;
        const int nstaged = (int)lead + cnt;
        uint32_t idx1 = kstep0 + (uint32_t)e + 1u;
        auto step = [&](const float4 a, const float2 b, const float4 c) {
            const float dx = a.x - pxf, dy = a.y - pyf;
            const float power2 = __builtin_fmaf(a.z * dx, dx, __builtin_fmaf(a.w, dx, b.x * dy) * dy);
            const float G = __builtin_amdgcn_exp2f(power2);
            const float al = fminf(0.99f, b.y * G);
            const float a2 = (power2 <= 0.0f && al >= (1.0f / 255.0f)) ? al : 0.f;
            const float x = 1.f - a2;
            const float xs = __uint_as_float((__float_as_uint(qperm<QP_PREV>(x)) & ~e0_mask) | (0x3F800000u & e0_mask));
            float tb = Tc;
#pragma unroll
            for (int r = 0; r < 3; r++) tb = mul_qprev(tb, xs);
            const float ta = tb * x;
            const bool pass = ta >= 0.0001f;
            const float w = pass ? a2 * tb : 0.f;
            C0 += c.x * w;
            C1 += c.y * w;
            C2 += c.z * w;
            last_k = (w > 0.f) ? idx1 : last_k;
            idx1 += 4u;
            uint32_t cand = pass ? __float_as_uint(ta) : 0x7F800000u;
            cand = min(cand, qperm<QP_X1>(cand));
            cand = min(cand, qperm<QP_X2>(cand));
            Tf = cand != 0x7F800000u ? __uint_as_float(cand) : Tf;
            Tc = qperm<QP_LAST>(ta);
        };
        auto ld_a = [&](int o) { return *reinterpret_cast<const float4*>(sp + o); };
        auto ld_b = [&](int o) { return *reinterpret_cast<const float2*>(sp + o + 16); };
        auto ld_c = [&](int o) {
            const float4 c = *reinterpret_cast<const float4*>(sp + o + 32);
            asm volatile("" ::"v"(c.w));
            return c;
        };
        float4 a0 = ld_a(0), c0 = ld_c(0);
        float2 b0 = ld_b(0);
        int j = 0;
        for (; j + 4 < nstaged; j += 8) {
            if (ck_due(kstep0 + (uint32_t)j)) checkpoint(kstep0 + (uint32_t)j);
            const float4 a1 = ld_a(192), c1 = ld_c(192);
            const float2 b1 = ld_b(192);
            step(a0, b0, c0);
            if (ck_due(kstep0 + (uint32_t)j + 4u)) checkpoint(kstep0 + (uint32_t)j + 4u);
            a0 = ld_a(384); c0 = ld_c(384); b0 = ld_b(384);
            sp += 384;
            step(a1, b1, c1);
        }
        if (j < nstaged) {
            if (ck_due(kstep0 + (uint32_t)j)) checkpoint(kstep0 + (uint32_t)j);
            step(a0, b0, c0);
        }
        PF_ADD(pf_loop);
        {
            uint32_t lk = max(last_k, qperm<QP_X1>(last_k));
            lk = max(lk, qperm<QP_X2>(lk));
            last_k = lk;
            if (lk > kbase) last = __float_as_uint(srec[(lk - 1u - kstep0) * 3 + 2].w);
        }
        const bool alive = __ballot(Tc >= 0.0001f) != 0ull;
        if (lane == 0) s_flag[wv] = alive ? 1u : 0u;
        lds_barrier();
        live = (s_flag[0] | s_flag[1] | s_flag[2] | s_flag[3]) != 0u;
        PF_ADD(pf_tail);
    }
#ifdef FWD4_PROF
    if (tid == 0 && blockIdx.x < 8)
        printf("fwd4prof block %d tile %d q %d: list %d batches %u steps %u | cycles total %llu stage %llu loop %llu tail %llu\n", (int)blockIdx.x, tile, q, n,
               pf_batches, pf_steps, (unsigned long long)(__builtin_readcyclecounter() - pf_t0), pf_stage, pf_loop, pf_tail);
#endif
    {
        const uint32_t wm = wave_max_u32(last_k);
        if (lane == 0) s_lastk[wv] = wm;
        lds_barrier();
        if (tid == 0) qcount[quad] = max(max(s_lastk[0], s_lastk[1]), max(s_lastk[2], s_lastk[3]));
        if (chunks > 1 && tid > nck && tid < chunks) ck_start[quad * (size_t)chunks + tid] = 0xFFFFFFFFu;
    }
    float s0 = C0 + qperm<QP_X1>(C0), s1 = C1 + qperm<QP_X1>(C1), s2 = C2 + qperm<QP_X1>(C2);
    s0 += qperm<QP_X2>(s0);
    s1 += qperm<QP_X2>(s1);
    s2 += qperm<QP_X2>(s2);
    float l1 = 0.f;
    if (inside && e0) {
        const size_t HW = (size_t)H * W;
        const size_t pid = (size_t)py * W + px;
        final_T[pid] = Tf;
        n_contrib[pid] = FQ ? A.src_n_contrib[pid] : last;
        ncon_c[pid] = last_k;
        const float o0 = s0 + Tf * bg[0], o1 = s1 + Tf * bg[1], o2 = s2 + Tf * bg[2];
        out_color[pid] = o0;
        out_color[HW + pid] = o1;
        out_color[2 * HW + pid] = o2;
        l1 = (fabsf(o0 - gt0) + fabsf(o1 - gt1)) + fabsf(o2 - gt2);
    }
    if (A.l1_target) {
        l1 = wave_sum(l1);
        lds_barrier();
        if (lane == 0) s_lastk[wv] = __float_as_uint(l1);
        lds_barrier();
        if (tid == 0)
            A.l1_part[quad] = (__uint_as_float(s_lastk[0]) + __uint_as_float(s_lastk[1])) + (__uint_as_float(s_lastk[2]) + __uint_as_float(s_lastk[3]));
    }
}

template <bool FQ>
__global__ __launch_bounds__(FWD4_BATCH) void render_fwd_small_kernel(const FwdArgs A) {
    __shared__ float4 srec[(FWD4_BATCH + 12) * 3];
    __shared__ uint32_t s_cnt[4], s_flag[4], s_lastk[4];
    int slot, q;
    if (blockIdx.x == 0 && threadIdx.x == 0 && A.all_ones) *A.all_ones = (A.not_ones && *A.not_ones == 0ull) ? 1u : 0u;
    render_block_map((int)blockIdx.x, A.xmap, &slot, &q);
    if (slot < A.ntiles && !(FQ && A.not_ones && *A.not_ones == 0ull)) {
        const uint32_t ov = A.order[slot];
        if (ov >> 31) {
            render_quadrant_4<FQ>(A, (int)(ov & 0x7FFFFFFFu), q, srec, s_cnt, s_flag, s_lastk);
        } else if (threadIdx.x < 64) {
            render_quadrant_1<FQ>(A, (int)ov, q, srec);
        }
    }
    forward_side_fill(A);
}

int launch_render_forward(const float* rec, const uint32_t* point_list, const uint32_t* ranges, const uint32_t* order,
                          const float* bg, int W, int H, float* out_color, float* final_T, uint32_t* n_contrib,
                          const QuadLists& ql, hipStream_t s) {
    const int gx = (W + TILE - 1) / TILE, gy = (H + TILE - 1) / TILE;
    const int xmap = gs_tune_get(GS_TUNE_XCD_MAP);
    const FwdArgs A{reinterpret_cast<const float4*>(rec), point_list, reinterpret_cast<const uint2*>(ranges), order, bg, W, H, gx,
                    gx * gy, xmap, out_color, final_T, n_contrib, ql.qlist, ql.ncon_c, ql.qcount, ql.ckpt, ql.ck_start,
                    ql.ckpt ? ql.chunks : 1, ql.src_qcount, ql.src_n_contrib, ql.not_ones, ql.marks, ql.mark_quads, ql.marks_flag, ql.all_ones,
                    ql.l1_target, ql.l1_part,
                    ql.chunked ? FWDC_MAX_UNITS * 4 : 0, ql.cw_hdr, ql.cw_units, ql.cw_items, ql.cw_q, ql.cw_flag, ql.cw_done, ql.cw_rec, ql.src_cw_flag,
                    ql.src_cw_rec, ql.src_final_T};
    const dim3 grid(render_grid_blocks(gx * gy, xmap) + A.cw_blocks);
    const bool fq = ql.src_qcount != nullptr;
    if (ql.four_waves) {
        if (fq) hipLaunchKernelGGL(render_fwd_small_kernel<true>, grid, dim3(FWD4_BATCH), 0, s, A);
        else hipLaunchKernelGGL(render_fwd_small_kernel<false>, grid, dim3(FWD4_BATCH), 0, s, A);
    } else {
        if (A.cw_blocks) {
            if (fq) hipLaunchKernelGGL(render_fwd_cw_kernel<true>, grid, dim3(64), 0, s, A);
            else hipLaunchKernelGGL(render_fwd_cw_kernel<false>, grid, dim3(64), 0, s, A);
        } else {
            if (fq) hipLaunchKernelGGL(render_fwd_kernel<true>, grid, dim3(64), 0, s, A);
            else hipLaunchKernelGGL(render_fwd_kernel<false>, grid, dim3(64), 0, s, A);
        }
    }
    GS_LAUNCH_CHECK("render_forward", 0, s);
    if (ql.l1_target)
        return launch_loss_final(ql.l1_part, gx * gy * 4, 1.0f / (3.0f * (float)W * (float)H), ql.l1_loss, s);
    return GS_OK;
}

__global__ __launch_bounds__(256) void opacity_image_kernel(const float* __restrict__ final_T, const float* __restrict__ bg,
                                                            int n, float* __restrict__ out) {
    const int i = blockIdx.x * blockDim.x + threadIdx.x;
    if (i >= n) return;
    const float Tf = final_T[i];
    out[i] = (1.0f - Tf) + Tf * bg[0];
}

int launch_opacity_image(const float* final_T, const float* bg, int W, int H, float* out, hipStream_t s) {
    const int n = W * H;
    hipLaunchKernelGGL(opacity_image_kernel, dim3((n + 255) / 256), dim3(256), 0, s, final_T, bg, n, out);
    GS_LAUNCH_CHECK("opacity_image", 0, s);
    return GS_OK;
}
```

### 3dgs-avatar-release_amd/diff_gaussian_rasterization/__init__.py

```python
import ctypes
import os
import threading
import weakref
from typing import NamedTuple

import torch
import torch.nn as nn

from gsplat_mi355 import _lib

__all__ = ["GaussianRasterizationSettings", "GaussianRasterizer", "rasterize_gaussians"]


class GaussianRasterizationSettings(NamedTuple):
    image_height: int
    image_width: int
    tanfovx: float
    tanfovy: float
    bg: torch.Tensor
    scale_modifier: float
    viewmatrix: torch.Tensor
    projmatrix: torch.Tensor
    sh_degree: int
    campos: torch.Tensor
    prefiltered: bool
    debug: bool


_tls = threading.local()
_SHARE = os.environ.get("GSPLAT_SHARE_GEOMETRY", "1") != "0"
_SPECULATE = os.environ.get("GSPLAT_SPECULATE", "1") != "0"


class _GeomEntry(object):
    __slots__ = ("key", "geom", "binning", "img", "num_rendered", "capacity", "radii", "color_ref", "means2D_id",
                 "allow_second", "second", "long_lists", "__weakref__")

    def __init__(self, key, geom, binning, img, num_rendered, capacity, radii):
        self.key, self.geom, self.binning, self.img, self.radii = key, geom, binning, img, radii
        self.num_rendered, self.capacity = num_rendered, capacity
        self.color_ref, self.means2D_id, self.allow_second, self.second, self.long_lists = None, None, False, None, 0

    def release(self):
        self.key = self.geom = self.binning = self.img = self.radii = None


class _GeomCache(object):

    def __init__(self):
        self.offer = {}
        self.hits = 0

    @staticmethod
    def _sig(t):
        if t is None or t.numel() == 0:
            return None
        return (id(t), t.data_ptr(), t._version, tuple(t.shape), tuple(t.stride()))

    def key(self, settings, means3D, opacities, scales, rotations, cov3D, stream_handle=None, capturing=False):
        tensors = (means3D, opacities, scales, rotations, cov3D, settings.viewmatrix, settings.projmatrix, settings.campos)
        return dict(scalars=(int(settings.image_height), int(settings.image_width), float(settings.tanfovx),
                             float(settings.tanfovy), float(settings.scale_modifier), int(means3D.shape[0]), _TILE_RECT,
                             _lib.stream_handle(means3D.device) if stream_handle is None
                             else int(stream_handle),
                             bool(capturing)),
                    sigs=[self._sig(t) for t in tensors],
                    objs=[t for t in tensors if t is not None and t.numel() > 0])

    def take(self, dev, key):
        ref = self.offer.pop(dev.index, None)
        e = ref() if ref is not None else None
        if e is None or e.key is None:
            return None
        if e.key["scalars"] != key["scalars"] or e.key["sigs"] != key["sigs"]:
            return None
        self.hits += 1
        return e

    def put(self, dev, entry):
        self.offer[dev.index] = weakref.ref(entry)

    def clear(self):
        self.offer.clear()


_geom_cache = _GeomCache()


def release_shared_geometry():
    _geom_cache.clear()


_sizes = {}
_lib.tuning_listeners.append(_sizes.clear)


def _size(fn_name, *args):
    k = (fn_name,) + args
    v = _sizes.get(k)
    if v is None:
        if len(_sizes) > 4096:
            _sizes.clear()
        v = _sizes[k] = _lib.nbytes(getattr(_lib.load(), fn_name), *args)
    return v


_last_count = {}


def _capacity_for(count):
    want = count + count // 8
    step = 1 << max(want.bit_length() - 5, 0)
    return (want + step - 1) // step * step


_is_capturing = None


def _stream_capturing():
    global _is_capturing
    if _is_capturing is None:
        _is_capturing = getattr(torch._C, "_cuda_isCurrentStreamCapturing", None) or torch.cuda.is_current_stream_capturing
    return bool(_is_capturing())


_captured = []


def captured_forwards(clear=False):
    out = list(_captured)
    if clear:
        del _captured[:]
    return out


_CAPTURE_SLACK = float(os.environ.get("GSPLAT_CAPTURE_SLACK", "0.25"))


def _pinned_count(device):
    cache = getattr(_tls, "pinned", None)
    if cache is None:
        cache = _tls.pinned = {}
    key = device.index
    if key not in cache:
        cache[key] = torch.zeros(1, dtype=torch.int64).pin_memory()
    return cache[key]


def _f32c(t, name):
    if t is None or t.numel() == 0:
        return None
    if not t.is_cuda:
        raise RuntimeError("diff_gaussian_rasterization: `%s` must be a GPU tensor (this build has no CPU path)" % name)
    if t.dtype != torch.float32:
        raise RuntimeError("diff_gaussian_rasterization: `%s` must be float32" % name)
    return t.contiguous()


_TILE_RECT = int(os.environ.get("GSPLAT_TILE_RECT", "1"))


_LONG_LISTS = os.environ.get("GSPLAT_LONG_LISTS", "0")
_frame_stats = {}


def _stats_words(key):
    st = _frame_stats.get(key)
    if st is None:
        st = _frame_stats[key] = torch.zeros(2, dtype=torch.int64).pin_memory()
    return st


def _make_args(settings, means3D, sh, colors_precomp, opacities, scales, rotations, cov3Ds_precomp, keep, long_lists=None):
    a = _lib.GsFwdArgs()
    P = int(means3D.shape[0])
    a.P = P
    a.sh_degree = int(settings.sh_degree)
    a.M = int(sh.shape[1]) if sh is not None else 0
    a.W, a.H = int(settings.image_width), int(settings.image_height)
    dev = means3D.device
    bg = _f32c(settings.bg.to(dev), "bg")
    view = _f32c(settings.viewmatrix.to(dev), "viewmatrix")
    proj = _f32c(settings.projmatrix.to(dev), "projmatrix")
    campos = _f32c(settings.campos.to(dev), "campos")
    keep.extend([bg, view, proj, campos])
    a.bg, a.viewmatrix, a.projmatrix, a.campos = bg.data_ptr(), view.data_ptr(), proj.data_ptr(), campos.data_ptr()
    a.means3D = _lib.ptr(means3D)
    a.shs = _lib.ptr(sh)
    a.colors_precomp = _lib.ptr(colors_precomp)
    a.opacities = _lib.ptr(opacities)
    a.scales = _lib.ptr(scales)
    a.rotations = _lib.ptr(rotations)
    a.cov3D_precomp = _lib.ptr(cov3Ds_precomp)
    a.scale_modifier = float(settings.scale_modifier)
    a.tanfovx, a.tanfovy = float(settings.tanfovx), float(settings.tanfovy)
    a.prefiltered = int(bool(settings.prefiltered))
    a.debug = int(bool(settings.debug))
    a.tile_rect = _TILE_RECT
    st = _stats_words((dev.index, a.W, a.H))
    if long_lists is None:
        long_lists = 1 if (_LONG_LISTS == "1" or (_LONG_LISTS == "auto" and int(st[0]) > 0)) else 0
        a.frame_stats = st.data_ptr()
    a.long_lists = int(long_lists)
    return a


def _dump_snapshot(path, raster_settings, tensors):
    try:
        cpu = [t.detach().cpu().clone() if isinstance(t, torch.Tensor) else t for t in tensors]
        settings = {k: (v.detach().cpu() if isinstance(v, torch.Tensor) else v) for k, v in raster_settings._asdict().items()}
        torch.save({"settings": settings, "tensors": cpu}, path)
    except Exception:
        pass


def rasterize_gaussians(means3D, means2D, sh, colors_precomp, opacities, scales, rotations, cov3Ds_precomp,
                        raster_settings, with_opacity=False, l1_target=None):
    if l1_target is not None:
        l1_target = _f32c(l1_target, "l1_target")
        if tuple(l1_target.shape) != (3, int(raster_settings.image_height), int(raster_settings.image_width)):
            raise ValueError("diff_gaussian_rasterization: l1_target must be a (3, H, W) image")
    dep = None
    if (_FUSE_SECOND and _SHARE and not with_opacity and torch.is_grad_enabled() and colors_precomp is not None
            and colors_precomp.numel() and not colors_precomp.requires_grad and (sh is None or sh.numel() == 0)):
        dep = _second_render_dependency(means3D, means2D, opacities, scales, rotations, cov3Ds_precomp, raster_settings)
    if not torch.is_grad_enabled():
        color, radii, opacity, l1 = _RasterizeGaussians.forward(_InferenceCtx(), means3D, means2D, sh, colors_precomp, opacities,
                                                                scales, rotations, cov3Ds_precomp, raster_settings,
                                                                bool(with_opacity), None, l1_target)
    else:
        color, radii, opacity, l1 = _RasterizeGaussians.apply(means3D, means2D, sh, colors_precomp, opacities, scales,
                                                               rotations, cov3Ds_precomp, raster_settings, bool(with_opacity),
                                                               dep, l1_target)
    out = (color, radii, opacity) if with_opacity else (color, radii)
    return out + (l1,) if l1_target is not None else out


_FUSE_SECOND = os.environ.get("GSPLAT_FUSE_SECOND_BACKWARD", "1") != "0"


def _second_render_dependency(means3D, means2D, opacities, scales, rotations, cov3Ds_precomp, settings):
    if not means3D.is_cuda:
        return None
    ref = _geom_cache.offer.get(means3D.device.index)
    e = ref() if ref is not None else None
    if e is None or e.key is None or not e.allow_second or e.color_ref is None or e.means2D_id != id(means2D):
        return None
    img1 = e.color_ref()
    if img1 is None or not img1.requires_grad:
        return None
    def c(t):
        return t if (t is None or t.numel() == 0 or (t.dtype == torch.float32 and t.is_contiguous())) else None
    if any(c(t) is None and t is not None and t.numel() for t in (means3D, opacities, scales, rotations, cov3Ds_precomp)):
        return None
    key = _geom_cache.key(settings, means3D, opacities, scales, rotations, cov3Ds_precomp)
    if e.key["scalars"] != key["scalars"] or e.key["sigs"] != key["sigs"]:
        return None
    return img1


class _InferenceCtx(object):
    needs_input_grad = (False,) * 12

    def set_materialize_grads(self, value):
        pass

    def save_for_backward(self, *tensors):
        pass

    def mark_non_differentiable(self, *tensors):
        pass


class _RasterizeGaussians(torch.autograd.Function):
    @staticmethod
    def forward(ctx, means3D, means2D, sh, colors_precomp, opacities, scales, rotations, cov3Ds_precomp,
                raster_settings, with_opacity=False, dep=None, l1_target=None):
        if not raster_settings.debug:
            return _RasterizeGaussians._forward(ctx, means3D, means2D, sh, colors_precomp, opacities, scales, rotations,
                                                cov3Ds_precomp, raster_settings, with_opacity, dep, l1_target)
        args = (means3D, means2D, sh, colors_precomp, opacities, scales, rotations, cov3Ds_precomp)
        try:
            return _RasterizeGaussians._forward(ctx, means3D, means2D, sh, colors_precomp, opacities, scales, rotations,
                                                cov3Ds_precomp, raster_settings, with_opacity, dep, l1_target)
        except Exception:
            _dump_snapshot("snapshot_fw.dump", raster_settings, args)
            print("\nAn error occured in forward. Please forward snapshot_fw.dump for debugging.")
            raise

    @staticmethod
    def _forward(ctx, means3D, means2D, sh, colors_precomp, opacities, scales, rotations, cov3Ds_precomp,
                 raster_settings, with_opacity=False, dep=None, l1_target=None):
        ctx.with_opacity = bool(with_opacity)
        ctx.l1_target = None
        l1 = None
        ctx.defer_to = None
        means2D_in = means2D
        ctx.set_materialize_grads(False)
        L = _lib.load()
        means3D = _f32c(means3D, "means3D")
        if means3D is None:
            raise RuntimeError("diff_gaussian_rasterization: means3D is empty")
        sh = _f32c(sh, "shs")
        colors_precomp = _f32c(colors_precomp, "colors_precomp")
        opacities = _f32c(opacities, "opacities")
        scales = _f32c(scales, "scales")
        rotations = _f32c(rotations, "rotations")
        if rotations is not None:
            rotations = _lib.contiguous_aligned(rotations)
        cov3Ds_precomp = _f32c(cov3Ds_precomp, "cov3D_precomp")
        dev = means3D.device
        P = int(means3D.shape[0])
        W, H = int(raster_settings.image_width), int(raster_settings.image_height)
        keep = []
        with _lib.on_device(dev):
            a = _make_args(raster_settings, means3D, sh, colors_precomp, opacities, scales, rotations, cov3Ds_precomp,
                           keep)
            stream_h = _lib.stream_handle(dev)
            sptr = ctypes.c_void_p(stream_h)
            capturing = _stream_capturing()
            if capturing:
                a.frame_stats = None
            if l1_target is not None:
                ctx.l1_target = l1_target
                l1 = torch.empty((), dtype=torch.float32, device=dev)
                a.l1_target, a.l1_loss = l1_target.data_ptr(), l1.data_ptr()
            inference = isinstance(ctx, _InferenceCtx)
            if inference:
                a.forward_only = 1
            share = _SHARE and not inference and any(ctx.needs_input_grad)
            gkey = (_geom_cache.key(raster_settings, means3D, opacities, scales, rotations, cov3Ds_precomp, stream_h,
                                    capturing)
                    if share else None)
            hit = _geom_cache.take(dev, gkey) if (share and l1_target is None) else None
            if not share or l1_target is not None:
                _geom_cache.offer.pop(dev.index, None)
            ctx.geom_entry = None
            if hit is not None:
                a.long_lists = int(hit.long_lists)
            geom_bytes = _size("gs_geom_bytes", P)
            ik = ("img", W, H, int(a.long_lists))
            img_bytes = _sizes.get(ik)
            if img_bytes is None:
                img_bytes = _sizes[ik] = _lib.nbytes(L.gs_image_bytes_for, ctypes.byref(a))
            geom = torch.empty(geom_bytes, dtype=torch.uint8, device=dev)
            img = torch.empty(img_bytes, dtype=torch.uint8, device=dev)
            radii = torch.empty(P, dtype=torch.int32, device=dev)
            if hit is not None:
                num_rendered, capacity = hit.num_rendered, hit.capacity
                binning = hit.binning
                if (dep is not None and hit.allow_second and hit.color_ref is not None and hit.color_ref() is dep
                        and hit.long_lists == int(a.long_lists)):
                    ctx.defer_to = hit
                bin_bytes = binning.numel()
                radii.copy_(hit.radii)
                color = torch.empty(3, H, W, dtype=torch.float32, device=dev)
                check_qlist = binning.clone() if (raster_settings.debug and bin_bytes) else None
                _lib.check(L.gs_forward_shared(ctypes.byref(a), hit.geom.data_ptr(), hit.img.data_ptr(),
                                               geom.data_ptr(), geom_bytes, binning.data_ptr(), bin_bytes, img.data_ptr(),
                                               img_bytes, capacity, color.data_ptr(), sptr))
                if check_qlist is not None and not torch.equal(check_qlist, binning):
                    raise RuntimeError("diff_gaussian_rasterization: the shared-geometry render changed the binning "
                                       "state it shares with the previous call")
                return _RasterizeGaussians._finish(ctx, raster_settings, num_rendered, capacity, means3D, sh, colors_precomp,
                                                   opacities, scales, rotations, cov3Ds_precomp, radii, geom, binning,
                                                   img, color, dev, a, sptr, keep)
            color = torch.empty(3, H, W, dtype=torch.float32, device=dev)
            if capturing:
                ck = (dev.index, P, W, H)
                if ck not in _last_count:
                    raise RuntimeError("diff_gaussian_rasterization: run one eager frame of this shape (P=%d, %dx%d) before "
                                       "capturing it into a graph: the binning state of a captured frame has a fixed "
                                       "capacity, sized from the last eager frame's pair count" % (P, W, H))
                guess = _last_count[ck]
                capacity = _capacity_for(max(int(guess * (1.0 + _CAPTURE_SLACK)), 1024))
                bin_bytes = _size("gs_binning_bytes", capacity, W, H)
                binning = torch.empty(bin_bytes, dtype=torch.uint8, device=dev)
                _lib.check(L.gs_forward_preprocess(ctypes.byref(a), geom.data_ptr(), geom_bytes, img.data_ptr(), img_bytes,
                                                   radii.data_ptr(), None, sptr))
                _lib.check(L.gs_forward_render(ctypes.byref(a), geom.data_ptr(), geom_bytes, binning.data_ptr(), bin_bytes,
                                               img.data_ptr(), img_bytes, capacity, color.data_ptr(), sptr))
                cptr = ctypes.c_void_p()
                _lib.check(L.gs_geom_field(geom.data_ptr(), P, _lib.GS_GEOM_COUNT, ctypes.byref(cptr)))
                off = int(cptr.value) - geom.data_ptr()
                _captured.append((geom[off:off + 8].view(torch.int64), capacity))
                num_rendered = capacity
                if share:
                    ctx.geom_entry = _GeomEntry(gkey, geom, binning, img, num_rendered, capacity, radii)
                    ctx.geom_entry.color_ref = weakref.ref(color)
                    ctx.geom_entry.means2D_id = id(means2D_in)
                    ctx.geom_entry.allow_second = not ctx.with_opacity
                    ctx.geom_entry.long_lists = int(a.long_lists)
                    _geom_cache.put(dev, ctx.geom_entry)
                return _RasterizeGaussians._finish(ctx, raster_settings, num_rendered, capacity, means3D, sh, colors_precomp,
                                                   opacities, scales, rotations, cov3Ds_precomp, radii, geom, binning, img,
                                                   color, dev, a, sptr, keep, l1)
            count = _pinned_count(dev)
            guess = _last_count.get((dev.index, P, W, H), 0)
            capacity = _capacity_for(guess) if (guess and _SPECULATE) else 0
            bin_bytes = _size("gs_binning_bytes", capacity, W, H) if capacity else 0
            binning = torch.empty(bin_bytes, dtype=torch.uint8, device=dev) if capacity else None
            nr = ctypes.c_int64(0)
            rc = L.gs_forward(ctypes.byref(a), geom.data_ptr(), geom_bytes, _lib.ptr(binning), bin_bytes, capacity,
                              img.data_ptr(), img_bytes, radii.data_ptr(), count.data_ptr(), color.data_ptr(),
                              ctypes.byref(nr), sptr)
            num_rendered = int(nr.value)
            if rc == _lib.GS_E_WORKSPACE:
                capacity = num_rendered
                bin_bytes = _size("gs_binning_bytes", capacity, W, H)
                binning = torch.empty(bin_bytes, dtype=torch.uint8, device=dev)
                rc = L.gs_forward_render(ctypes.byref(a), geom.data_ptr(), geom_bytes, binning.data_ptr(), bin_bytes,
                                         img.data_ptr(), img_bytes, capacity, color.data_ptr(), sptr)
            _lib.check(rc)
            if len(_last_count) > 256:
                _last_count.clear()
            _last_count[(dev.index, P, W, H)] = num_rendered
            if share:
                ctx.geom_entry = _GeomEntry(gkey, geom, binning, img, num_rendered, capacity, radii)
                ctx.geom_entry.color_ref = weakref.ref(color)
                ctx.geom_entry.means2D_id = id(means2D_in)
                ctx.geom_entry.allow_second = not ctx.with_opacity
                ctx.geom_entry.long_lists = int(a.long_lists)
                _geom_cache.put(dev, ctx.geom_entry)
            return _RasterizeGaussians._finish(ctx, raster_settings, num_rendered, capacity, means3D, sh, colors_precomp,
                                               opacities, scales, rotations, cov3Ds_precomp, radii, geom, binning, img, color,
                                               dev, a, sptr, keep, l1)

    @staticmethod
    def _finish(ctx, raster_settings, num_rendered, capacity, means3D, sh, colors_precomp, opacities, scales, rotations,
                cov3Ds_precomp, radii, geom, binning, img, color, dev, a, sptr, keep=None, l1=None):
        opacity = None
        if ctx.with_opacity:
            L = _lib.load()
            H, W = int(raster_settings.image_height), int(raster_settings.image_width)
            opacity = torch.empty(1, H, W, dtype=torch.float32, device=dev)
            _lib.check(L.gs_opacity_image(ctypes.byref(a), img.data_ptr(), img.numel(), opacity.data_ptr(), sptr))
        ctx.raster_settings = raster_settings
        ctx.long_lists = int(a.long_lists)
        ctx.fwd_args = (a, keep)
        ctx.num_rendered = num_rendered
        ctx.capacity = capacity
        ctx.present = (sh is not None, colors_precomp is not None, scales is not None, cov3Ds_precomp is not None)
        empty = torch.empty(0, device=dev)
        ctx.save_for_backward(means3D, sh if sh is not None else empty,
                              colors_precomp if colors_precomp is not None else empty, opacities,
                              scales if scales is not None else empty, rotations if rotations is not None else empty,
                              cov3Ds_precomp if cov3Ds_precomp is not None else empty, radii, geom, binning, img, color)
        ctx.mark_non_differentiable(radii)
        return color, radii, opacity, l1

    @staticmethod
    def backward(ctx, grad_out_color, _grad_radii, grad_out_opacity=None, grad_l1=None):
        if not ctx.raster_settings.debug:
            return _RasterizeGaussians._backward(ctx, grad_out_color, _grad_radii, grad_out_opacity, grad_l1)
        try:
            return _RasterizeGaussians._backward(ctx, grad_out_color, _grad_radii, grad_out_opacity, grad_l1)
        except Exception:
            _dump_snapshot("snapshot_bw.dump", ctx.raster_settings, tuple(ctx.saved_tensors[:8]) + (grad_out_color,))
            print("\nAn error occured in backward. Writing snapshot_bw.dump for debugging.\n")
            raise

    @staticmethod
    def _backward(ctx, grad_out_color, _grad_radii, grad_out_opacity=None, grad_l1=None):
        L = _lib.load()
        tgt = getattr(ctx, "defer_to", None)
        if tgt is not None and tgt.geom is not None and grad_out_color is not None:
            saved = ctx.saved_tensors
            tgt.second = dict(colors=saved[2], out_color=saved[11], grad=_f32c(grad_out_color, "grad_out_color"), img=saved[10],
                              long_lists=ctx.long_lists)
            return (None,) * 12
        entry = getattr(ctx, "geom_entry", None)
        second = None
        if entry is not None:
            second, entry.second = entry.second, None
            entry.release()
            ctx.geom_entry = None
        (means3D, sh, colors_precomp, opacities, scales, rotations, cov3Ds_precomp, radii, geom, binning, img,
         color) = ctx.saved_tensors
        has_sh, has_col, has_sr, has_cov = ctx.present
        settings = ctx.raster_settings
        dev = means3D.device
        P = int(means3D.shape[0])
        W, H = int(settings.image_width), int(settings.image_height)
        D = ctx.capacity
        use_l1 = ctx.l1_target is not None and grad_l1 is not None
        if grad_out_color is None and not use_l1:
            grad_out_color = torch.zeros(3, H, W, dtype=torch.float32, device=dev)
        g = _f32c(grad_out_color, "grad_out_color") if grad_out_color is not None else None
        g_l1 = _f32c(grad_l1, "grad_l1") if use_l1 else None
        g_op = _f32c(grad_out_opacity, "grad_out_opacity") if (ctx.with_opacity and grad_out_opacity is not None) else None
        with _lib.on_device(dev):
            a, _keep = ctx.fwd_args
            if (a.means3D != means3D.data_ptr() or a.opacities != opacities.data_ptr()
                    or (has_sh and a.shs != sh.data_ptr()) or (has_sr and a.scales != scales.data_ptr())):
                _keep = []
                a = _make_args(settings, means3D, sh if has_sh else None, colors_precomp if has_col else None, opacities,
                               scales if has_sr else None, rotations if has_sr else None,
                               cov3Ds_precomp if has_cov else None, _keep, long_lists=ctx.long_lists)
            a.l1_target = ctx.l1_target.data_ptr() if use_l1 else None
            a.l1_loss = None
            a.l1_grad = g_l1.data_ptr() if use_l1 else None
            gp = g.data_ptr() if g is not None else None
            sptr = _lib.stream_ptr(dev)
            scratch_bytes = _size("gs_backward_scratch_bytes", D, P, W, H)
            scratch = torch.empty(scratch_bytes, dtype=torch.uint8, device=dev)
            M = int(sh.shape[1]) if has_sh else 0
            f = dict(dtype=torch.float32, device=dev)
            d_means3D = torch.empty(P, 3, **f)
            d_means2D = torch.empty(P, 3, **f)
            d_colors = torch.empty(P, 3, **f)
            d_opacity = torch.empty(P, 1, **f)
            d_cov3D = torch.empty(P, 6, **f)
            d_sh = torch.empty(P, M, 3, **f) if has_sh else None
            d_scales = torch.empty(P, 3, **f) if has_sr else None
            d_rot = torch.empty(P, 4, **f) if has_sr else None
            gr = _lib.GsGrads(_lib.ptr(d_means3D), _lib.ptr(d_means2D), _lib.ptr(d_sh), _lib.ptr(d_colors),
                              _lib.ptr(d_opacity), _lib.ptr(d_scales), _lib.ptr(d_rot), _lib.ptr(d_cov3D))
            if second is not None and g_op is None:
                si = _lib.GsSecondImage(second["colors"].data_ptr(), second["out_color"].data_ptr(), second["grad"].data_ptr(),
                                        second["img"].data_ptr(), second["img"].numel(), int(second["long_lists"]))
                _lib.check(L.gs_backward_with_second(ctypes.byref(a), radii.data_ptr(), geom.data_ptr(), geom.numel(),
                                                     binning.data_ptr(), binning.numel(), img.data_ptr(), img.numel(), D,
                                                     color.data_ptr(), gp, ctypes.byref(si), scratch.data_ptr(),
                                                     scratch_bytes, ctypes.byref(gr), sptr))
            elif g_op is None:
                _lib.check(L.gs_backward(ctypes.byref(a), radii.data_ptr(), geom.data_ptr(), geom.numel(),
                                         binning.data_ptr(), binning.numel(), img.data_ptr(), img.numel(), D,
                                         color.data_ptr(), gp, scratch.data_ptr(), scratch_bytes,
                                         ctypes.byref(gr), sptr))
            else:
                _lib.check(L.gs_backward_with_opacity(ctypes.byref(a), radii.data_ptr(), geom.data_ptr(), geom.numel(),
                                                      binning.data_ptr(), binning.numel(), img.data_ptr(), img.numel(), D,
                                                      color.data_ptr(), gp, g_op.data_ptr(), scratch.data_ptr(),
                                                      scratch_bytes, ctypes.byref(gr), sptr))
        return (d_means3D, d_means2D, d_sh, d_colors if has_col else None, d_opacity, d_scales, d_rot,
                d_cov3D if has_cov else None, None, None, None, None)


class GaussianRasterizer(nn.Module):
    def __init__(self, raster_settings):
        super().__init__()
        self.raster_settings = raster_settings

    def markVisible(self, positions):
        L = _lib.load()
        rs = self.raster_settings
        with torch.no_grad():
            pos = _f32c(positions, "positions")
            P = int(pos.shape[0])
            out = torch.zeros(P, dtype=torch.uint8, device=pos.device)
            view = _f32c(rs.viewmatrix.to(pos.device), "viewmatrix")
            proj = _f32c(rs.projmatrix.to(pos.device), "projmatrix")
            with _lib.on_device(pos.device):
                sptr = _lib.stream_ptr(pos.device)
                _lib.check(L.gs_mark_visible(P, pos.data_ptr(), view.data_ptr(), proj.data_ptr(), _lib.ptr(out), sptr))
        return out.bool()

    def forward(self, means3D, means2D, opacities, shs=None, colors_precomp=None, scales=None, rotations=None,
                cov3D_precomp=None, with_opacity=False, l1_target=None):
        raster_settings = self.raster_settings
        if (shs is None and colors_precomp is None) or (shs is not None and colors_precomp is not None):
            raise Exception('Please provide excatly one of either SHs or precomputed colors!')
        if ((scales is None or rotations is None) and cov3D_precomp is None) or \
                ((scales is not None or rotations is not None) and cov3D_precomp is not None):
            raise Exception('Please provide exactly one of either scale/rotation pair or precomputed 3D covariance!')
        if shs is None:
            shs = torch.Tensor([])
        if colors_precomp is None:
            colors_precomp = torch.Tensor([])
        if scales is None:
            scales = torch.Tensor([])
        if rotations is None:
            rotations = torch.Tensor([])
        if cov3D_precomp is None:
            cov3D_precomp = torch.Tensor([])
        return rasterize_gaussians(means3D, means2D, shs, colors_precomp, opacities, scales, rotations, cov3D_precomp,
                                   raster_settings, with_opacity=with_opacity, l1_target=l1_target)
```

### 3dgs-avatar-release_amd/gsplat_mi355/_lib.py

```python
import ctypes
import os
import threading
from ctypes import POINTER, c_char_p, c_double, c_float, c_int, c_int32, c_int64, c_size_t, c_uint8, c_void_p

_HERE = os.path.dirname(os.path.abspath(__file__))
LIB_PATH = os.environ.get("GSPLAT_LIB_PATH") or os.path.join(os.path.dirname(_HERE), "lib", "libgsplat_mi355.so")


class GsFwdArgs(ctypes.Structure):
    _fields_ = [
        ("P", c_int32), ("sh_degree", c_int32), ("M", c_int32), ("W", c_int32), ("H", c_int32),
        ("bg", c_void_p), ("means3D", c_void_p), ("shs", c_void_p), ("colors_precomp", c_void_p),
        ("opacities", c_void_p), ("scales", c_void_p), ("rotations", c_void_p), ("cov3D_precomp", c_void_p),
        ("viewmatrix", c_void_p), ("projmatrix", c_void_p), ("campos", c_void_p),
        ("scale_modifier", c_float), ("tanfovx", c_float), ("tanfovy", c_float),
        ("prefiltered", c_int32), ("debug", c_int32), ("tile_rect", c_int32), ("long_lists", c_int32),
        ("frame_stats", c_void_p), ("l1_target", c_void_p), ("l1_loss", c_void_p), ("l1_grad", c_void_p),
        ("forward_only", c_int32),
    ]


class GsSecondImage(ctypes.Structure):
    _fields_ = [("colors", c_void_p), ("out_color", c_void_p), ("dL_dpix", c_void_p), ("img", c_void_p),
                ("img_bytes", c_size_t), ("long_lists", c_int32)]


class GsGrads(ctypes.Structure):
    _fields_ = [(n, c_void_p) for n in ("dL_dmeans3D", "dL_dmeans2D", "dL_dsh", "dL_dcolors", "dL_dopacity",
                                        "dL_dscales", "dL_drotations", "dL_dcov3D")]


EXPORTS = ["gs_geom_bytes", "gs_image_bytes", "gs_binning_bytes", "gs_backward_scratch_bytes",
           "gs_forward_preprocess", "gs_forward_render", "gs_forward", "gs_forward_shared", "gs_backward", "gs_mark_visible", "knn_workspace_bytes",
           "knn_dist2", "gs_geom_field", "gs_binning_field", "gs_image_field", "gs_status_string",
           "gs_last_hip_error", "gs_last_stage", "gs_build_info", "gs_profile_enable", "gs_profile_filter", "gs_profile_collect",
           "gs_l1_loss_workspace_bytes", "gs_l1_loss", "gs_bce_loss", "gs_ssim_workspace_bytes", "gs_ssim_forward", "gs_ssim_backward",
           "gs_build_covariance", "gs_build_covariance_backward", "gs_sh2rgb", "gs_sh2rgb_backward", "knn_points", "gs_densify_stats", "gs_adam_step",
           "gs_opacity_image", "gs_backward_with_opacity", "gs_tuning", "gs_profile_reserve", "gs_image_bytes_for", "gs_backward_with_second", "gs_clock_probe", "gs_pair_stats", "gs_xcc_probe",
           "gs_densify_workspace_bytes", "gs_densify_plan", "gs_densify_apply", "gs_reset_opacity",
           "gs_aiap_workspace_bytes", "gs_aiap_forward", "gs_aiap_backward",
           "gs_hashgrid_levels", "gs_hashgrid_workspace_bytes", "gs_hashgrid_forward", "gs_hashgrid_backward",
           "gs_skin_weights_forward", "gs_skin_weights_backward", "gs_skinning_workspace_bytes", "gs_skinning_forward",
           "gs_skinning_backward",
           "gs_mesh_sample", "gs_skin_loss_workspace_bytes", "gs_skin_loss_forward", "gs_skin_loss_backward",
           "gs_pose_workspace_bytes", "gs_pose_forward", "gs_pose_backward",
           "gs_pose_encoder_grad_floats", "gs_pose_encoder_forward", "gs_pose_encoder_backward",
           "gs_nonrigid_workspace_bytes", "gs_nonrigid_apply_forward", "gs_nonrigid_apply_backward",
           "gs_texture_workspace_bytes", "gs_texture_input_forward", "gs_texture_input_backward",
           "gs_mlp_workspace_bytes", "gs_mlp_forward", "gs_mlp_backward",
           "gs_grad_norm_workspace_bytes", "gs_grad_norm", "gs_grad_scale", "gs_adam_step_ex"]

GS_E_WORKSPACE = -5
GS_E_CAPTURE = -6
GS_ADAM_MAX_TENSORS = 16
GS_GEOM_DEPTHS, GS_GEOM_TILES, GS_GEOM_REC, GS_GEOM_CLAMPED, GS_GEOM_SORTED_IDX, GS_GEOM_COUNT, GS_GEOM_FIELDS = range(7)
GS_BIN_POINT_LIST, GS_BIN_QLIST, GS_BIN_FIELDS = range(3)
(GS_IMG_RANGES, GS_IMG_N_CONTRIB, GS_IMG_FINAL_T, GS_IMG_QCOUNT, GS_IMG_NCON_C, GS_IMG_ORDER, GS_IMG_CW_HDR, GS_IMG_CW_UNITS,
 GS_IMG_CW_FLAG, GS_IMG_CW_REC, GS_IMG_FIELDS) = range(11)


class GsAdamTensor(ctypes.Structure):
    _fields_ = [("param", c_void_p), ("grad", c_void_p), ("exp_avg", c_void_p), ("exp_avg_sq", c_void_p),
                ("n", c_int64), ("lr", c_float)]


GS_OPTIM_MAX_TENSORS, GS_GRAD_NORM_BATCH, GS_ADAM_EX_BATCH, GS_ADAM_STEP_BATCH = 4096, 192, 48, 384


class GsGradTensor(ctypes.Structure):
    _fields_ = [("grad", c_void_p), ("n", c_int64)]


class GsAdamTensorEx(ctypes.Structure):
    _fields_ = [("param", c_void_p), ("grad", c_void_p), ("exp_avg", c_void_p), ("exp_avg_sq", c_void_p),
                ("n", c_int64), ("lr", c_float), ("weight_decay", c_float), ("step", c_void_p), ("lr_dev", c_void_p)]


GS_DENSIFY_MAX_TENSORS = 24
GS_DENSIFY_COPY, GS_DENSIFY_ZERO_IF_NEW, GS_DENSIFY_ZERO, GS_DENSIFY_CHILD_POSITION, GS_DENSIFY_CHILD_SCALING = 0, 1, 2, 3, 4
GS_DENSIFY_F_KEEP, GS_DENSIFY_F_CLONE, GS_DENSIFY_F_SPLIT, GS_DENSIFY_F_PRUNE = 1, 2, 4, 8
GS_DENSIFY_F_CHILD_PRUNE, GS_DENSIFY_F_CLONE_KEPT, GS_DENSIFY_F_CHILDREN_KEPT = 16, 32, 64


class GsDensifyPlan(ctypes.Structure):
    _fields_ = [("N", c_int32), ("scaling", c_void_p), ("opacity", c_void_p), ("grad_accum", c_void_p), ("denom", c_void_p),
                ("prune_mask", c_void_p), ("grad_threshold", c_float), ("split_scale", c_float), ("min_opacity", c_float),
                ("max_world_scale", c_float), ("max_screen_size", c_float), ("prune_size", c_int32)]


class GsDensifyTensor(ctypes.Structure):
    _fields_ = [("src", c_void_p), ("dst", c_void_p), ("width", c_int32), ("kind", c_int32)]


class GsAiapSet(ctypes.Structure):
    _fields_ = [("xc", c_void_p), ("xd", c_void_p), ("D", c_int32), ("loss", c_void_p), ("dL_dloss", c_void_p),
                ("dL_dxc", c_void_p), ("dL_dxd", c_void_p)]


GS_HASHGRID_MAX_LEVELS = 32


GS_SKIN_BONES = 24
GS_SKIN_HIERARCHICAL, GS_SKIN_SOFTMAX, GS_SKIN_WEIGHTS = 0, 1, 2


GS_POSE_BONES, GS_POSE_MAX_BETAS, GS_POSE_STATE_FLOATS = 24, 16, 512


class GsPoseArgs(ctypes.Structure):
    _fields_ = [("V", c_int32), ("NB", c_int32), ("parents", c_int32 * GS_POSE_BONES)] + [
        (n, c_void_p) for n in ("v_template", "shapedirs", "J_template", "J_shapedirs", "betas", "root_orient", "pose_body",
                                "pose_hand", "trans", "rots_gt")]


GS_POSE_ENC_JOINTS, GS_POSE_ENC_MAX_DIM, GS_POSE_ENC_STATE_FLOATS = 24, 16, 1392
GS_NONRIGID_MAX_D = 2048
GS_NR_SCALE_LOGIT, GS_NR_SCALE_EXP, GS_NR_SCALE_ZERO = 0, 1, 2
GS_NR_ROT_ADD, GS_NR_ROT_MULT = 0, 1


class GsPoseEncArgs(ctypes.Structure):
    _fields_ = [("d", c_int32), ("parents", c_int32 * GS_POSE_ENC_JOINTS)] + [
        (n, c_void_p) for n in ("rots", "Jtrs", "W0", "b0")] + [
        (n, c_void_p * GS_POSE_ENC_JOINTS) for n in ("W1", "b1", "W2", "b2")]


GS_TEXTURE_MAX_D, GS_TEXTURE_MAX_BEFORE, GS_TEXTURE_MAX_AFTER = 512, 6, 2


class GsTextureArgs(ctypes.Structure):
    _fields_ = [("N", c_int32), ("D", c_int32), ("sh_degree", c_int32), ("n_before", c_int32), ("n_after", c_int32),
                ("before_w", c_int32 * GS_TEXTURE_MAX_BEFORE), ("after_w", c_int32 * GS_TEXTURE_MAX_AFTER),
                ("latent_dim", c_int32), ("rot_stride", c_int32), ("rot_row", c_int32), ("use_noise", c_int32),
                ("noise", c_float * 9), ("before", c_void_p * GS_TEXTURE_MAX_BEFORE), ("after", c_void_p * GS_TEXTURE_MAX_AFTER),
                ("xyz", c_void_p), ("campos", c_void_p), ("fwd_transform", c_void_p), ("latent", c_void_p)]


GS_MLP_MAX_WIDTH, GS_MLP_MAX_HIDDEN, GS_MLP_MAX_LAYERS, GS_MLP_MAX_IN, GS_MLP_MAX_COND, GS_MLP_MAX_OUT = 128, 6, 7, 512, 512, 64
GS_MLP_TILE_ROWS, GS_MLP_PARTIAL_MIN_ROWS, GS_MLP_MAX_PARTIALS = 128, 256, 128


class GsMlpArgs(ctypes.Structure):
    _fields_ = [(n, c_int32) for n in ("N", "dim_in", "dim_cond", "width", "n_hidden", "dim_out")] + [
        ("slope", c_float), ("x", c_void_p), ("cond", c_void_p)] + [
        (n, c_void_p * GS_MLP_MAX_LAYERS) for n in ("W", "b", "dW", "db")] + [("dx", c_void_p), ("dcond", c_void_p)]


class GsHashGrid(ctypes.Structure):
    _fields_ = [("n_levels", c_int32), ("n_features_per_level", c_int32), ("log2_hashmap_size", c_int32),
                ("base_resolution", c_int32), ("per_level_scale", c_float)]


_lock = threading.Lock()
_lib = None


def load():
    global _lib
    if _lib is not None:
        return _lib
    with _lock:
        if _lib is not None:
            return _lib
        import torch
        if not os.path.exists(LIB_PATH):
            raise RuntimeError("libgsplat_mi355.so not found at %s: build it with "
                               "`python 3dgs-avatar-release_amd/build.py` (there is no CPU fallback)" % LIB_PATH)
        L = ctypes.CDLL(LIB_PATH)
        L.gs_geom_bytes.argtypes = [c_int32, POINTER(c_size_t)]
        L.gs_image_bytes.argtypes = [c_int32, c_int32, POINTER(c_size_t)]
        L.gs_image_bytes_for.argtypes = [POINTER(GsFwdArgs), POINTER(c_size_t)]
# ... 227 lines not shown
```

### include/gsplat_mi355.h

```cpp
#ifndef GSPLAT_MI355_H
#define GSPLAT_MI355_H

#include <stddef.h>
#include <stdint.h>

#ifdef __cplusplus
extern "C" {
#endif

#define GS_OK 0
#define GS_E_BAD_ARG (-1)
#define GS_E_EXCLUSIVE (-2)
#define GS_E_TOO_LARGE (-3)
#define GS_E_HIP (-4)
#define GS_E_WORKSPACE (-5)
#define GS_E_CAPTURE (-6)


typedef struct GsFwdArgs {
    int32_t P;
    int32_t sh_degree;
    int32_t M;
    int32_t W, H;
    const float* bg;
    const float* means3D;
    const float* shs;
    const float* colors_precomp;
    const float* opacities;
    const float* scales;
    const float* rotations;
    const float* cov3D_precomp;
    const float* viewmatrix;
    const float* projmatrix;
    const float* campos;
    float scale_modifier, tanfovx, tanfovy;
    int32_t prefiltered;
    int32_t debug;
    int32_t tile_rect;
    int32_t long_lists;
    int64_t* frame_stats;
    const float* l1_target;
    float* l1_loss;
    const float* l1_grad;
    int32_t forward_only;
} GsFwdArgs;

typedef struct GsGrads {
    float* dL_dmeans3D;
    float* dL_dmeans2D;
    float* dL_dsh;
    float* dL_dcolors;
    float* dL_dopacity;
    float* dL_dscales;
    float* dL_drotations;
    float* dL_dcov3D;
} GsGrads;

int gs_geom_bytes(int32_t P, size_t* out);
int gs_image_bytes(int32_t W, int32_t H, size_t* out);
int gs_binning_bytes(int64_t num_rendered, int32_t W, int32_t H, size_t* out);
int gs_backward_scratch_bytes(int64_t num_rendered, int32_t P, int32_t W, int32_t H, size_t* out);

int gs_forward_preprocess(const GsFwdArgs* a, void* geom, size_t geom_bytes, void* img, size_t img_bytes,
                          int32_t* radii, int64_t* count_host_pinned, void* stream);

int gs_forward_render(const GsFwdArgs* a, void* geom, size_t geom_bytes, void* binning, size_t binning_bytes,
                      void* img, size_t img_bytes, int64_t num_rendered, float* out_color, void* stream);

int gs_forward(const GsFwdArgs* a, void* geom, size_t geom_bytes, void* binning, size_t binning_bytes, int64_t capacity,
               void* img, size_t img_bytes, int32_t* radii, int64_t* count_host_pinned, float* out_color,
               int64_t* num_rendered, void* stream);

int gs_forward_shared(const GsFwdArgs* a, const void* geom_src, const void* img_src, void* geom, size_t geom_bytes,
                      void* binning, size_t binning_bytes, void* img, size_t img_bytes, int64_t num_rendered,
                      float* out_color, void* stream);

int gs_backward(const GsFwdArgs* a, const int32_t* radii, const void* geom, size_t geom_bytes, void* binning,
                size_t binning_bytes, const void* img, size_t img_bytes, int64_t num_rendered,
                const float* out_color, const float* dL_dpix, void* scratch, size_t scratch_bytes,
                const GsGrads* grads, void* stream);

int gs_opacity_image(const GsFwdArgs* a, const void* img, size_t img_bytes, float* opacity, void* stream);
int gs_backward_with_opacity(const GsFwdArgs* a, const int32_t* radii, const void* geom, size_t geom_bytes,
                             void* binning, size_t binning_bytes, const void* img, size_t img_bytes,
                             int64_t num_rendered, const float* out_color, const float* dL_dpix,
                             const float* dL_dopacity_img, void* scratch, size_t scratch_bytes, const GsGrads* grads,
                             void* stream);

typedef struct GsSecondImage {
    const float* colors;
    const float* out_color;
    const float* dL_dpix;
    const void* img;
    size_t img_bytes;
    int32_t long_lists;
} GsSecondImage;
int gs_backward_with_second(const GsFwdArgs* a, const int32_t* radii, const void* geom, size_t geom_bytes,
                            void* binning, size_t binning_bytes, const void* img, size_t img_bytes, int64_t D,
                            const float* out_color, const float* dL_dpix, const GsSecondImage* second, void* scratch,
                            size_t scratch_bytes, const GsGrads* grads, void* stream);

int gs_mark_visible(int32_t P, const float* means3D, const float* viewmatrix, const float* projmatrix,
                    uint8_t* present, void* stream);

int knn_workspace_bytes(int32_t P, size_t* out);
int knn_dist2(int32_t P, const float* points, float* mean_d2, void* workspace, size_t workspace_bytes, void* stream);

int gs_build_covariance(int32_t N, const float* scaling, float scaling_modifier, const float* rotation,
                        int32_t rotation_is_matrix, float* cov6, void* stream);
int gs_build_covariance_backward(int32_t N, const float* scaling, float scaling_modifier, const float* rotation,
                                 int32_t rotation_is_matrix, const float* dL_dcov6, float* dL_dscaling,
                                 float* dL_drotation, void* stream);
int gs_sh2rgb(int32_t N, int32_t sh_degree, int32_t M, const float* shs, const float* xyz, const float* campos,
              const float* fwd_rotation, const float* view_noise_host, float* colors, uint8_t* clamped, void* stream);
int gs_sh2rgb_backward(int32_t N, int32_t sh_degree, int32_t M, const float* shs, const float* xyz, const float* campos,
                       const float* fwd_rotation, const float* view_noise_host, const uint8_t* clamped,
                       const float* dL_dcolors, float* dL_dshs, float* dL_dxyz, void* stream);

int gs_l1_loss_workspace_bytes(int64_t n, size_t* out);
int gs_l1_loss(int64_t n, const float* x, const float* y, float* loss, float* dL_dx, void* workspace,
               size_t workspace_bytes, void* stream);

int gs_bce_loss(int64_t n, const float* x, const float* y, float* loss, float* dL_dx, void* workspace,
                size_t workspace_bytes, void* stream);

int gs_ssim_workspace_bytes(int32_t C, int32_t H, int32_t W, size_t* out);
int gs_ssim_forward(int32_t C, int32_t H, int32_t W, const float* img1, const float* img2, float* ssim_out,
                    float* dm_dmu1, float* dm_dsigma1_sq, float* dm_dsigma12, void* workspace, size_t workspace_bytes,
                    void* stream);
int gs_ssim_backward(int32_t C, int32_t H, int32_t W, const float* img1, const float* img2, const float* dm_dmu1,
                     const float* dm_dsigma1_sq, const float* dm_dsigma12, const float* dL_dssim, float* dL_dimg1,
                     void* stream);

int knn_points(int32_t Nq, const float* queries, int32_t Nr, const float* ref, int32_t K, float* dists, int64_t* idx,
               void* workspace, size_t workspace_bytes, void* stream);

#define GS_ADAM_MAX_TENSORS 16
typedef struct GsAdamTensor {
    float* param;
    const float* grad;
    float* exp_avg;
    float* exp_avg_sq;
    int64_t n;
    float lr;
} GsAdamTensor;
int gs_densify_stats(int32_t N, const int32_t* radii, const float* viewspace_grad, float* max_radii2D,
                     float* xyz_gradient_accum, float* denom, void* stream);
int gs_adam_step(int32_t n_tensors, const GsAdamTensor* tensors, double beta1, double beta2, double eps, int64_t step,
                 void* stream);

#define GS_OPTIM_MAX_TENSORS 4096
#define GS_GRAD_NORM_BATCH 192
#define GS_ADAM_EX_BATCH 48
#define GS_ADAM_STEP_BATCH 384
typedef struct GsGradTensor {
    float* grad;
    int64_t n;
} GsGradTensor;
typedef struct GsAdamTensorEx {
    float* param;
    const float* grad;
    float* exp_avg;
    float* exp_avg_sq;
    int64_t n;
    float lr;
    float weight_decay;
    float* step;
    const float* lr_dev;
} GsAdamTensorEx;
int gs_grad_norm_workspace_bytes(int32_t n_tensors, const GsGradTensor* tensors, size_t* out);
int gs_grad_norm(int32_t n_tensors, const GsGradTensor* tensors, float max_norm, float* out, void* workspace,
                 size_t workspace_bytes, void* stream);
int gs_grad_scale(int32_t n_tensors, const GsGradTensor* tensors, const float* clip_coef, void* stream);
int gs_adam_step_ex(int32_t n_tensors, const GsAdamTensorEx* tensors, double beta1, double beta2, double eps, int64_t step,
                    const float* clip_coef, void* stream);

#define GS_DENSIFY_MAX_TENSORS 24
#define GS_DENSIFY_COPY 0
#define GS_DENSIFY_ZERO_IF_NEW 1
#define GS_DENSIFY_ZERO 2
#define GS_DENSIFY_CHILD_POSITION 3
#define GS_DENSIFY_CHILD_SCALING 4
#define GS_DENSIFY_F_KEEP 1
#define GS_DENSIFY_F_CLONE 2
#define GS_DENSIFY_F_SPLIT 4
#define GS_DENSIFY_F_PRUNE 8
#define GS_DENSIFY_F_CHILD_PRUNE 16
#define GS_DENSIFY_F_CLONE_KEPT 32
#define GS_DENSIFY_F_CHILDREN_KEPT 64
typedef struct GsDensifyPlan {
    int32_t N;
    const float* scaling;
    const float* opacity;
    const float* grad_accum;
    const float* denom;
    const uint8_t* prune_mask;
    float grad_threshold;
// ... 223 lines not shown
```

Before: 1780 frames/s.

## Compute backward tile order in a fused post-render kernel with the L1 loss finalization

Adds a post_render kernel launched right after the forward render. One workgroup finalizes the L1 loss and another computes the backward tile order from the quad counts into a new bwd_order image buffer. The backward pass can then skip its own tile_order launch when the order was produced in forward and the marks are clean. This saves one kernel launch and its serial single-block work on the backward critical path, at the cost of new ABI plumbing (a fwd_order flag) and state tracking in the Python autograd wrapper.

```diff
diff --git a/3dgs-avatar-release_amd/csrc/binning.hip b/3dgs-avatar-release_amd/csrc/binning.hip
--- a/3dgs-avatar-release_amd/csrc/binning.hip
+++ b/3dgs-avatar-release_amd/csrc/binning.hip
@@ -433,6 +433,20 @@
     __shared__ uint32_t wsum[16];
     if (mode < 0) return;
     tile_order_body<HELD>(ranges, keys, mode, ntiles, order, pc, ll, hist, wmax, wsum);
+}
+
+template <bool HELD>
+__global__ __launch_bounds__(1024) void post_render_kernel(const float* __restrict__ l1_part, int nparts, float inv_n,
+                                                           float* __restrict__ l1_loss, const uint32_t* __restrict__ qcount,
+                                                           int ntiles, uint32_t* __restrict__ bwd_order) {
+    __shared__ uint32_t hist[1024];
+    __shared__ uint32_t wmax[16];
+    __shared__ uint32_t wsum[16];
+    if (l1_loss && blockIdx.x == 0) {
+        loss_final_wide_body(l1_part, nparts, inv_n, l1_loss, reinterpret_cast<float*>(wmax));
+        return;
+    }
+    tile_order_plain<HELD>(nullptr, qcount, 1, ntiles, bwd_order, PairCount{nullptr, 0}, LongLists{0, nullptr}, hist, wmax, wsum);
 }
 
 #define BM_LD 33
@@ -660,6 +674,18 @@
     return GS_OK;
 }
 
+int launch_post_render(const float* l1_part, int nparts, float inv_n, float* l1_loss, const uint32_t* qcount, int ntiles,
+                       uint32_t* bwd_order, int debug, hipStream_t s) {
+    const unsigned wgs = (l1_loss ? 1u : 0u) + (bwd_order ? 1u : 0u);
+    if (!wgs) return GS_OK;
+    if (ntiles <= 32 * 1024)
+        hipLaunchKernelGGL(post_render_kernel<true>, dim3(wgs), dim3(1024), 0, s, l1_part, nparts, inv_n, l1_loss, qcount, ntiles, bwd_order);
+    else
+        hipLaunchKernelGGL(post_render_kernel<false>, dim3(wgs), dim3(1024), 0, s, l1_part, nparts, inv_n, l1_loss, qcount, ntiles, bwd_order);
+    GS_LAUNCH_CHECK("post_render", debug, s);
+    return GS_OK;
+}
+
 int launch_tile_lists(const uint4* ranklist, const uint32_t* chunk_pairs, uint32_t* seg_start, int P, int gx, int gy, TileCounts tc, uint32_t* ranges,
                       uint32_t* order, uint32_t* point_list, PairCount pc, LongLists ll, bool totals_zeroed, int debug,
                       hipStream_t s) {
diff --git a/3dgs-avatar-release_amd/csrc/capi.hip b/3dgs-avatar-release_amd/csrc/capi.hip
--- a/3dgs-avatar-release_amd/csrc/capi.hip
+++ b/3dgs-avatar-release_amd/csrc/capi.hip
@@ -32,6 +32,7 @@
     {"fwd_marks", GS_TUNE_FWD_MARKS, 1, nullptr, nullptr},
     {"fwdc_ch", GS_TUNE_FWDC_CH, (int)FWDC_CH_MIN, "GSPLAT_FWDC_CH", [](int v) { return v >= 64 && (v & (v - 1)) == 0; }},
     {"fwdc_div", GS_TUNE_FWDC_DIV, (int)FWD4_TOTAL_DIV, "GSPLAT_FWDC_DIV", [](int v) { return v >= 1; }},
+    {"post_render", GS_TUNE_POST_RENDER, 1, "GSPLAT_POST_RENDER", nullptr},
 };
 struct TuneState {
     std::atomic<int> v[GS_TUNE_COUNT];
@@ -91,6 +92,7 @@
     g_prof.armed = false;
 }
 
+static_assert(sizeof(GsFwdArgs) == 184, "GsFwdArgs.fwd_order sits in what was the struct's tail padding: the size is ABI");
 static int validate(const GsFwdArgs* a) {
     if (!a) return GS_E_BAD_ARG;
     if (a->P < 0 || a->W <= 0 || a->H <= 0) return GS_E_BAD_ARG;
@@ -202,6 +204,20 @@
     ql.cw_flag = own.cw_flag;
     ql.cw_done = own.cw_done;
     ql.cw_rec = own.cw_rec;
+}
+static bool order_travels(const GsFwdArgs* a) {
+    return a->fwd_order && !a->forward_only && gs_tune_get(GS_TUNE_POST_RENDER) && gs_tune_get(GS_TUNE_BWD_ORDER) &&
+           gs_tune_get(GS_TUNE_FWD_MARKS);
+}
+static int forward_post_render(const GsFwdArgs* a, const ImgView& im, bool l1, hipStream_t s) {
+    float* const loss = l1 ? a->l1_loss : nullptr;
+    const int nparts = im.ntiles * 4;
+    const float inv_n = 1.0f / (3.0f * (float)a->W * (float)a->H);
+    if (!gs_tune_get(GS_TUNE_POST_RENDER)) return loss ? launch_loss_final(im.l1_part, nparts, inv_n, loss, s) : GS_OK;
+    uint32_t* const order = order_travels(a) ? im.bwd_order : nullptr;
+    if (!loss && !order) return GS_OK;
+    StageScope sc_("post_render", s);
+    return launch_post_render(im.l1_part, nparts, inv_n, loss, im.qcount, im.ntiles, order, a->debug, s);
 }
 static int sync_if_debug(const GsFwdArgs* a, const char* stage, hipStream_t s) {
     if (!a->debug) return GS_OK;
@@ -350,10 +366,12 @@
     }
     ql.l1_target = a->l1_target;
     ql.l1_part = im.l1_part;
-    ql.l1_loss = a->l1_loss;
+    const bool post = gs_tune_get(GS_TUNE_POST_RENDER) != 0;
     { StageScope sc_("render_fwd", s);
     rc = launch_render_forward(g.rec, a->P > 0 ? b.point_list : nullptr, im.ranges, im.order, a->bg, a->W, a->H, out_color,
-                               im.final_T, im.n_contrib, ql, s); }
+                               im.final_T, im.n_contrib, ql, s);
+    if (rc == GS_OK && !post) rc = forward_post_render(a, im, a->l1_target != nullptr, s); }
+    if (rc == GS_OK && post) rc = forward_post_render(a, im, a->l1_target != nullptr, s);
     if (rc != GS_OK) return rc;
     return sync_if_debug(a, "render_forward", s);
 }
@@ -456,6 +474,7 @@
     ql.all_ones = im.all_ones;
     { StageScope sc_("render_fwd", s);
     rc = launch_render_forward(g.rec, b.point_list, im.ranges, im.order, a->bg, a->W, a->H, out_color, im.final_T, im.n_contrib, ql, s); }
+    if (rc == GS_OK) rc = forward_post_render(a, im, false, s);
     if (rc != GS_OK) return rc;
     return sync_if_debug(a, "render_forward", s);
 }
@@ -503,13 +522,24 @@
         uint32_t* const q8 = reinterpret_cast<uint32_t*>(b.marks);
         uint32_t* const own_order = (uint32_t*)((char*)sums + scratch_sums_bytes(a->P));
         const bool order_here = gs_tune_get(GS_TUNE_BWD_ORDER) != 0;
-        { StageScope sc_("tile_order", s);
-        rc = launch_tile_order(im.ranges, ql.qcount, order_here ? 1 : -1, im.ntiles, own_order, PairCount{nullptr, 0},
-                               FillJob{b.marks, (size_t)D, gs_tune_get(GS_TUNE_NT_STORES) & 1, b.marks_flag},
-                               LongLists{0, nullptr}, a->debug, s); }
-        if (rc != GS_OK) return rc;
+        bool ordered = order_travels(a);
+        if (ordered && a->debug) {
+            uint32_t flag = 0u;
+            hipError_t e = hipMemcpyAsync(&flag, b.marks_flag, 4, hipMemcpyDeviceToHost, s);
+            if (e == hipSuccess) e = hipStreamSynchronize(s);
+            if (e != hipSuccess) { gs_set_error((int)e, "marks_flag.copy"); return GS_E_HIP; }
+            ordered = flag == MARKS_CLEAN;
+        }
+        if (!ordered) {
+            StageScope sc_("tile_order", s);
+            rc = launch_tile_order(im.ranges, ql.qcount, order_here ? 1 : -1, im.ntiles, own_order, PairCount{nullptr, 0},
+                                   FillJob{b.marks, (size_t)D, gs_tune_get(GS_TUNE_NT_STORES) & 1, b.marks_flag},
+                                   LongLists{0, nullptr}, a->debug, s);
+            if (rc != GS_OK) return rc;
+        }
+        const uint32_t* const order = ordered ? im.bwd_order : (order_here ? own_order : im.order);
         { StageScope sc_("render_bwd", s);
-        rc = launch_render_backward(g.rec, im.ranges, order_here ? own_order : im.order, a->W, a->H, ql, out_color, dL_dpix,
+        rc = launch_render_backward(g.rec, im.ranges, order, a->W, a->H, ql, out_color, dL_dpix,
                                     dL_dopacity_img, im.final_T, a->bg, (float*)scratch, q8, second ? &si : nullptr,
                                     L1Grad{a->l1_target, a->l1_grad}, s); }
         if (rc != GS_OK) return rc;
diff --git a/3dgs-avatar-release_amd/csrc/common.h b/3dgs-avatar-release_amd/csrc/common.h
--- a/3dgs-avatar-release_amd/csrc/common.h
+++ b/3dgs-avatar-release_amd/csrc/common.h
@@ -116,7 +116,7 @@
     return s < G.nseg_max ? s : G.nseg_max;
 }
 
-enum { GS_TUNE_XCD_MAP = 0, GS_TUNE_DEPTH_SORT = 1, GS_TUNE_NT_STORES = 2, GS_TUNE_BWD_CHUNKS = 3, GS_TUNE_FWD4 = 4, GS_TUNE_SMALL_TILES = 5, GS_TUNE_SHARED_QLIST = 6, GS_TUNE_ONES_FAST = 7, GS_TUNE_BWD_ORDER = 8, GS_TUNE_FWD_MARKS = 9, GS_TUNE_FWDC_CH = 10, GS_TUNE_FWDC_DIV = 11, GS_TUNE_COUNT = 12 };
+enum { GS_TUNE_XCD_MAP = 0, GS_TUNE_DEPTH_SORT = 1, GS_TUNE_NT_STORES = 2, GS_TUNE_BWD_CHUNKS = 3, GS_TUNE_FWD4 = 4, GS_TUNE_SMALL_TILES = 5, GS_TUNE_SHARED_QLIST = 6, GS_TUNE_ONES_FAST = 7, GS_TUNE_BWD_ORDER = 8, GS_TUNE_FWD_MARKS = 9, GS_TUNE_FWDC_CH = 10, GS_TUNE_FWDC_DIV = 11, GS_TUNE_POST_RENDER = 12, GS_TUNE_COUNT = 13 };
 int gs_tune_get(int key);
 
 #define BWD_CH 128
@@ -142,7 +142,7 @@
 #define FWDC_DEAD 0x80000000u
 #define FWDC_SPIN_MAX (1 << 16)
 struct ImgLayout {
-    size_t ranges, n_contrib, final_T, ncon_c, tile_nmax, order, seg_cnt, tile_tot, all_ones, cw_flag, cw_done, cw_q, tile_zero_bytes, l1_part, ckpt, ck_start, cw_hdr, cw_units, cw_items, cw_rec, total;
+    size_t ranges, n_contrib, final_T, ncon_c, tile_nmax, order, seg_cnt, tile_tot, all_ones, cw_flag, cw_done, cw_q, tile_zero_bytes, l1_part, ckpt, ck_start, cw_hdr, cw_units, cw_items, cw_rec, bwd_order, total;
     int gx, gy, bwd_chunks;
 };
 static inline bool few_long_lists_mode(int ntiles, int long_lists) {
@@ -185,6 +185,7 @@
         L.cw_items = take((size_t)FWDC_Q_WORDS * 4);
         L.cw_rec = take((size_t)FWDC_MAX_UNITS * 4 * FWDC_SLOTS * 64 * 4);
     }
+    L.bwd_order = take(nt * 4);
     L.total = o;
     return L;
 }
@@ -232,6 +233,7 @@
     ptr<uint2> cw_units;
     ptr<uint32_t> cw_items;
     ptr<float> cw_rec;
+    ptr<uint32_t> bwd_order;
     size_t tile_zero_bytes;
     int cw_clear_words;
     size_t total;
@@ -284,6 +286,7 @@
     at(v.cw_xcc_mask, L.cw_q + (size_t)FWDC_Q_WORDS * 4, cw);
     at(v.l1_part, L.l1_part); at(v.ckpt, L.ckpt); at(v.ck_start, L.ck_start);
     at(v.cw_hdr, L.cw_hdr, cw); at(v.cw_units, L.cw_units, cw); at(v.cw_items, L.cw_items, cw); at(v.cw_rec, L.cw_rec, cw);
+    at(v.bwd_order, L.bwd_order);
     v.tile_zero_bytes = L.tile_zero_bytes;
     v.cw_clear_words = cw ? (int)((L.cw_q + FWDC_Q_BYTES - L.cw_flag) / 4) : 0;
     v.total = L.total; v.gx = L.gx; v.gy = L.gy; v.ntiles = L.gx * L.gy; v.bwd_chunks = L.bwd_chunks;
@@ -611,6 +614,26 @@
 size_t l1_ws_bytes(int64_t n);
 int launch_l1_loss(const float* x, const float* y, int64_t n, float* loss, float* grad, float* partial, hipStream_t s);
 int launch_loss_final(const float* partial, int nparts, float inv_n, float* loss, hipStream_t s);
+__device__ __forceinline__ void loss_final_wide_body(const float* __restrict__ partial, int nparts, float inv_n,
+                                                     float* __restrict__ loss, float* ws ) {
+    const int tid = threadIdx.x, lane = tid & 63, wid = tid >> 6;
+    float acc = 0.f;
+    for (int i0 = tid; i0 < nparts; i0 += 8 * 1024) {
+        float v[8];
+#pragma unroll
+        for (int u = 0; u < 8; u++) v[u] = (i0 + u * 1024 < nparts) ? partial[i0 + u * 1024] : 0.f;
+#pragma unroll
+        for (int u = 0; u < 8; u++) acc += v[u];
+    }
+    acc = wave_sum(acc);
+    if (lane == 0) ws[wid] = acc;
+    __syncthreads();
+    if (tid == 0) {
+        float t = 0.f;
+        for (int w = 0; w < 16; w++) t += ws[w];
+        loss[0] = t * inv_n;
+    }
+}
 int launch_bce_loss(const float* x, const float* y, int64_t n, float* loss, float* grad, float* partial, hipStream_t s);
 size_t ssim_ws_bytes(int C, int H, int W);
 int launch_ssim_forward(int C, int H, int W, const float* img1, const float* img2, float* ssim_out, float* dm_dmu1,
@@ -629,6 +652,8 @@
 }
 int launch_tile_order(const uint32_t* ranges, const uint32_t* keys, int mode, int ntiles, uint32_t* order, PairCount pc,
                       FillJob fill, LongLists ll, int debug, hipStream_t s);
+int launch_post_render(const float* l1_part, int nparts, float inv_n, float* l1_loss, const uint32_t* qcount, int ntiles,
+                       uint32_t* bwd_order, int debug, hipStream_t s);
 struct QuadLists {
     uint32_t* qlist;
     uint32_t* ncon_c;
@@ -657,7 +682,6 @@
     uint32_t* all_ones = nullptr;
     const float* l1_target = nullptr;
     float* l1_part = nullptr;
-    float* l1_loss = nullptr;
 };
 int launch_render_forward(const float* rec, const uint32_t* point_list, const uint32_t* ranges, const uint32_t* order,
                           const float* bg, int W, int H, float* out_color, float* final_T, uint32_t* n_contrib,
diff --git a/3dgs-avatar-release_amd/csrc/loss.hip b/3dgs-avatar-release_amd/csrc/loss.hip
--- a/3dgs-avatar-release_amd/csrc/loss.hip
+++ b/3dgs-avatar-release_amd/csrc/loss.hip
@@ -88,23 +88,7 @@
 __global__ __launch_bounds__(1024) void loss_final_wide_kernel(const float* __restrict__ partial, int nparts, float inv_n,
                                                                float* __restrict__ loss) {
     __shared__ float ws[16];
-    const int tid = threadIdx.x, lane = tid & 63, wid = tid >> 6;
-    float acc = 0.f;
-    for (int i0 = tid; i0 < nparts; i0 += 8 * 1024) {
-        float v[8];
-#pragma unroll
-        for (int u = 0; u < 8; u++) v[u] = (i0 + u * 1024 < nparts) ? partial[i0 + u * 1024] : 0.f;
-#pragma unroll
-        for (int u = 0; u < 8; u++) acc += v[u];
-    }
-    acc = wave_sum(acc);
-    if (lane == 0) ws[wid] = acc;
-    __syncthreads();
-    if (tid == 0) {
-        float t = 0.f;
-        for (int w = 0; w < 16; w++) t += ws[w];
-        loss[0] = t * inv_n;
-    }
+    loss_final_wide_body(partial, nparts, inv_n, loss, ws);
 }
 
 int launch_loss_final(const float* partial, int nparts, float inv_n, float* loss, hipStream_t s) {
diff --git a/3dgs-avatar-release_amd/csrc/render_fwd.hip b/3dgs-avatar-release_amd/csrc/render_fwd.hip
--- a/3dgs-avatar-release_amd/csrc/render_fwd.hip
+++ b/3dgs-avatar-release_amd/csrc/render_fwd.hip
@@ -913,8 +913,6 @@
         }
     }
     GS_LAUNCH_CHECK("render_forward", 0, s);
-    if (ql.l1_target)
-        return launch_loss_final(ql.l1_part, gx * gy * 4, 1.0f / (3.0f * (float)W * (float)H), ql.l1_loss, s);
     return GS_OK;
 }
 
diff --git a/3dgs-avatar-release_amd/diff_gaussian_rasterization/__init__.py b/3dgs-avatar-release_amd/diff_gaussian_rasterization/__init__.py
--- a/3dgs-avatar-release_amd/diff_gaussian_rasterization/__init__.py
+++ b/3dgs-avatar-release_amd/diff_gaussian_rasterization/__init__.py
@@ -34,12 +34,13 @@
 
 class _GeomEntry(object):
     __slots__ = ("key", "geom", "binning", "img", "num_rendered", "capacity", "radii", "color_ref", "means2D_id",
-                 "allow_second", "second", "long_lists", "__weakref__")
+                 "allow_second", "second", "long_lists", "args", "__weakref__")
 
     def __init__(self, key, geom, binning, img, num_rendered, capacity, radii):
         self.key, self.geom, self.binning, self.img, self.radii = key, geom, binning, img, radii
         self.num_rendered, self.capacity = num_rendered, capacity
         self.color_ref, self.means2D_id, self.allow_second, self.second, self.long_lists = None, None, False, None, 0
+        self.args = None
 
     def release(self):
         self.key = self.geom = self.binning = self.img = self.radii = None
@@ -336,7 +337,10 @@
             if not share or l1_target is not None:
                 _geom_cache.offer.pop(dev.index, None)
             ctx.geom_entry = None
+            a.fwd_order = 1 if (not inference and not capturing and hit is None and any(ctx.needs_input_grad)) else 0
             if hit is not None:
+                if hit.args is not None:
+                    hit.args.fwd_order = 0
                 a.long_lists = int(hit.long_lists)
             geom_bytes = _size("gs_geom_bytes", P)
             ik = ("img", W, H, int(a.long_lists))
@@ -387,6 +391,7 @@
                 num_rendered = capacity
                 if share:
                     ctx.geom_entry = _GeomEntry(gkey, geom, binning, img, num_rendered, capacity, radii)
+                    ctx.geom_entry.args = a
                     ctx.geom_entry.color_ref = weakref.ref(color)
                     ctx.geom_entry.means2D_id = id(means2D_in)
                     ctx.geom_entry.allow_second = not ctx.with_opacity
@@ -417,6 +422,7 @@
             _last_count[(dev.index, P, W, H)] = num_rendered
             if share:
                 ctx.geom_entry = _GeomEntry(gkey, geom, binning, img, num_rendered, capacity, radii)
+                ctx.geom_entry.args = a
                 ctx.geom_entry.color_ref = weakref.ref(color)
                 ctx.geom_entry.means2D_id = id(means2D_in)
                 ctx.geom_entry.allow_second = not ctx.with_opacity
@@ -491,6 +497,7 @@
         g_op = _f32c(grad_out_opacity, "grad_out_opacity") if (ctx.with_opacity and grad_out_opacity is not None) else None
         with _lib.on_device(dev):
             a, _keep = ctx.fwd_args
+            order_ready, a.fwd_order = a.fwd_order, 0
             if (a.means3D != means3D.data_ptr() or a.opacities != opacities.data_ptr()
                     or (has_sh and a.shs != sh.data_ptr()) or (has_sr and a.scales != scales.data_ptr())):
                 _keep = []
@@ -499,6 +506,7 @@
                                cov3Ds_precomp if has_cov else None, _keep, long_lists=ctx.long_lists)
             a.l1_target = ctx.l1_target.data_ptr() if use_l1 else None
             a.l1_loss = None
+            a.fwd_order = order_ready if (a is ctx.fwd_args[0] and second is None) else 0
             a.l1_grad = g_l1.data_ptr() if use_l1 else None
             gp = g.data_ptr() if g is not None else None
             sptr = _lib.stream_ptr(dev)
@@ -533,6 +541,7 @@
                                                       binning.data_ptr(), binning.numel(), img.data_ptr(), img.numel(), D,
                                                       color.data_ptr(), gp, g_op.data_ptr(), scratch.data_ptr(),
                                                       scratch_bytes, ctypes.byref(gr), sptr))
+        a.fwd_order = 0
         return (d_means3D, d_means2D, d_sh, d_colors if has_col else None, d_opacity, d_scales, d_rot,
                 d_cov3D if has_cov else None, None, None, None, None)
 
diff --git a/3dgs-avatar-release_amd/gsplat_mi355/_lib.py b/3dgs-avatar-release_amd/gsplat_mi355/_lib.py
--- a/3dgs-avatar-release_amd/gsplat_mi355/_lib.py
+++ b/3dgs-avatar-release_amd/gsplat_mi355/_lib.py
@@ -16,7 +16,7 @@
         ("scale_modifier", c_float), ("tanfovx", c_float), ("tanfovy", c_float),
         ("prefiltered", c_int32), ("debug", c_int32), ("tile_rect", c_int32), ("long_lists", c_int32),
         ("frame_stats", c_void_p), ("l1_target", c_void_p), ("l1_loss", c_void_p), ("l1_grad", c_void_p),
-        ("forward_only", c_int32),
+        ("forward_only", c_int32), ("fwd_order", c_int32),
     ]
 
 
diff --git a/include/gsplat_mi355.h b/include/gsplat_mi355.h
--- a/include/gsplat_mi355.h
+++ b/include/gsplat_mi355.h
@@ -43,6 +43,7 @@
     float* l1_loss;
     const float* l1_grad;
     int32_t forward_only;
+    int32_t fwd_order;
 } GsFwdArgs;
 
 typedef struct GsGrads {
```

Result: no change. 1793 frames/s, median of 6 (+0.8%).
